# tlkvstepan/PracticalDeepStereo_NIPS2018

Hardware: AMD Instinct MI355X
Metric: stereo pairs/sec, 960x540 D=192, Matching+Regularization+SubpixelMap hot path (higher is better)
Workload: dtype f32; 1 GPU; configs[1]: 960x540 pair padded to 576x960, D=192 (48 matching planes, 96 cost planes), batch 1, eval mode, random-init weights seed 0; parallelism=single GPU, launch=eager, whole pairs round-robin over 3 HIP streams

## Files before the change

include/pds_hip.h:

```cpp
#ifndef PDS_HIP_H
#define PDS_HIP_H

#include <stddef.h>
#include <stdint.h>

#ifdef __cplusplus
extern "C" {
#endif

#define PDS_ABI_VERSION 6

typedef void* pds_stream_t;

int pds_abi_version(void);
const char* pds_last_error(void);

long long pds_nonfinite_statistics(int reset);

int pds_probe_begin(const char* kernel, int capacity);
int pds_probe_end(float* ms, int* workgroups, int capacity);

int pds_debug_chain_stamps(unsigned* ticks, int capacity);

typedef struct PdsConvBlockParams {
    const float* weight;
    const float* bias;
    const float* gamma;
    const float* beta;
} PdsConvBlockParams;

int pds_subpixel_map_fwd(const float* similarities, float* disparities,
                         int batch, int planes, int height, int width,
                         int half_support_window, int disparity_step,
                         pds_stream_t stream);

int pds_subpixel_map_confidence_fwd(const float* similarities, float* disparities, float* confidence,
                                    int batch, int planes, int height, int width,
                                    int half_support_window, int disparity_step,
                                    pds_stream_t stream);

int pds_shift_concat_fwd(const float* left, const float* right, float* out,
                         int batch, int channels, int h, int w,
                         int d_begin, int d_count, pds_stream_t stream);

typedef struct PdsMatchingParams {
    int features;
    int signature_features;
    int residual_blocks;
    PdsConvBlockParams first;
    const PdsConvBlockParams* blocks;
    PdsConvBlockParams last;
} PdsMatchingParams;

size_t pds_matching_workspace_bytes(const PdsMatchingParams* params, int batch, int h, int w,
                                    int d_count);
int pds_matching_fwd(const PdsMatchingParams* params,
                     const float* left, const float* right, float* signatures,
                     int batch, int h, int w, int d_begin, int d_count,
                     void* workspace, size_t workspace_bytes, int weights_resident,
                     pds_stream_t stream);

size_t pds_matching_operation_workspace_bytes(const PdsMatchingParams* params, int n, int h, int w);
int pds_matching_operation_fwd(const PdsMatchingParams* params,
                               const float* concatenated, float* signature,
                               int n, int h, int w,
                               void* workspace, size_t workspace_bytes, pds_stream_t stream);

typedef struct PdsRegularizationParams {
    int features;
    PdsConvBlockParams smoothing;
    PdsConvBlockParams contraction[4][2];
    PdsConvBlockParams expansion[4][2];
    PdsConvBlockParams upsample_half;
    PdsConvBlockParams upsample_full;
} PdsRegularizationParams;

size_t pds_regularization_workspace_bytes(const PdsRegularizationParams* params,
                                          int batch, int d, int h, int w);
int pds_regularization_fwd(const PdsRegularizationParams* params,
                           const float* signatures, const float* left_shortcut, float* cost,
                           int batch, int d, int h, int w,
                           void* workspace, size_t workspace_bytes, int weights_resident,
                           pds_stream_t stream);

int pds_regularization_subpixel_map_fwd(const PdsRegularizationParams* params,
                                        const float* signatures, const float* left_shortcut,
                                        float* disparities,
                                        int batch, int d, int h, int w,
                                        int half_support_window, int disparity_step,
                                        int crop_top, int crop_left,
                                        void* workspace, size_t workspace_bytes, int weights_resident,
                                        pds_stream_t stream);

int pds_regularization_subpixel_map_confidence_fwd(const PdsRegularizationParams* params,
                                                   const float* signatures, const float* left_shortcut,
                                                   float* disparities, float* confidence,
                                                   int batch, int d, int h, int w,
                                                   int half_support_window, int disparity_step,
                                                   int crop_top, int crop_left,
                                                   void* workspace, size_t workspace_bytes,
                                                   int weights_resident, pds_stream_t stream);

int pds_regularization_subpixel_map_mirrored_fwd(const PdsRegularizationParams* params,
                                                 const float* signatures, const float* left_shortcut,
                                                 float* disparities, float* confidence ,
                                                 int batch, int d, int h, int w,
                                                 int half_support_window, int disparity_step,
                                                 int crop_top, int crop_left,
                                                 void* workspace, size_t workspace_bytes,
                                                 int weights_resident, pds_stream_t stream);

size_t pds_contraction_block_workspace_bytes(int batch, int c, int d, int h, int w);
int pds_contraction_block_fwd(const PdsConvBlockParams* downsampling, const PdsConvBlockParams* smoothing,
                              const float* x, float* down, float* smooth,
                              int batch, int c, int d, int h, int w,
                              void* workspace, size_t workspace_bytes, pds_stream_t stream);

size_t pds_expansion_block_workspace_bytes(int batch, int c, int d, int h, int w);
int pds_expansion_block_fwd(const PdsConvBlockParams* upsampling, const PdsConvBlockParams* smoothing,
                            const float* x, const float* shortcut, float* out,
                            int batch, int c, int d, int h, int w,
                            void* workspace, size_t workspace_bytes, pds_stream_t stream);

size_t pds_conv_block_workspace_bytes(int n, int cin, int cout, int d, int h, int w, int kd, int stride,
                                      int per_plane);
int pds_conv_block_fwd(const PdsConvBlockParams* params, const float* x, float* raw, float* scale,
                       float* shift, int n, int cin, int cout, int d, int h, int w, int kd, int stride,
                       int per_plane, void* workspace, size_t workspace_bytes, pds_stream_t stream);
int pds_conv_block_chained_fwd(const PdsConvBlockParams* params, const float* x, const float* x_scale,
                               const float* x_shift, int x_per_plane, const float* x_bound, float* raw, float* scale,
                               float* shift, int n, int cin, int cout, int d, int h, int w, int kd, int stride,
                               int per_plane, void* workspace, size_t workspace_bytes, pds_stream_t stream);

size_t pds_regularization_bwd_workspace_bytes(const PdsRegularizationParams* params, int batch, int d, int h, int w);
int pds_regularization_bwd(const PdsRegularizationParams* params, const PdsRegularizationParams* grads,
                           const float* signatures, const float* left_shortcut, const float* grad_cost,
                           float* grad_signatures, float* grad_left_shortcut, int batch, int d, int h, int w,
                           void* fwd_workspace, size_t fwd_workspace_bytes, void* workspace, size_t workspace_bytes,
                           pds_stream_t stream);

size_t pds_matching_operation_bwd_workspace_bytes(const PdsMatchingParams* params, int n, int h, int w);
int pds_matching_operation_bwd(const PdsMatchingParams* params, const PdsMatchingParams* grads,
                               const float* concatenated, const float* grad_signature, float* grad_concatenated,
                               int n, int h, int w, void* fwd_workspace, size_t fwd_workspace_bytes,
                               void* workspace, size_t workspace_bytes, pds_stream_t stream);

size_t pds_matching_train_workspace_bytes(const PdsMatchingParams* params, int batch, int h, int w, int d_count);
int pds_matching_train_fwd(const PdsMatchingParams* params, const float* left, const float* right, float* signatures,
                           int batch, int h, int w, int d_begin, int d_count, void* workspace, size_t workspace_bytes,
                           pds_stream_t stream);
size_t pds_matching_bwd_workspace_bytes(const PdsMatchingParams* params, int batch, int h, int w, int d_count);
int pds_matching_bwd(const PdsMatchingParams* params, const PdsMatchingParams* grads, const float* left,
                     const float* right, const float* grad_signatures, float* grad_left, float* grad_right, int batch,
                     int h, int w, int d_begin, int d_count, void* fwd_workspace, size_t fwd_workspace_bytes,
                     void* workspace, size_t workspace_bytes, pds_stream_t stream);

typedef struct PdsEmbeddingParams {
    int input_features;
    int features;
    int shortcut_features;
    int residual_blocks;
    PdsConvBlockParams downsampling[2];
    const PdsConvBlockParams* blocks;
    PdsConvBlockParams shortcut;
} PdsEmbeddingParams;

size_t pds_embedding_workspace_bytes(const PdsEmbeddingParams* params, int batch, int h, int w, int pad_top,
                                     int pad_left);
int pds_embedding_fwd(const PdsEmbeddingParams* params, const float* image, float* descriptor, float* shortcut,
                      int batch, int h, int w, int pad_top, int pad_left, void* workspace, size_t workspace_bytes,
                      int weights_resident, pds_stream_t stream);
int pds_embedding_mirrored_fwd(const PdsEmbeddingParams* params, const float* image, float* descriptor,
                               float* shortcut, int batch, int h, int w, int pad_top, int pad_left, void* workspace,
                               size_t workspace_bytes, int weights_resident, pds_stream_t stream);
size_t pds_embedding_bwd_workspace_bytes(const PdsEmbeddingParams* params, int batch, int h, int w, int pad_top,
                                         int pad_left);
int pds_embedding_bwd(const PdsEmbeddingParams* params, const PdsEmbeddingParams* grads, const float* image,
                      const float* descriptor, float* grad_descriptor, const float* grad_shortcut, int batch, int h,
                      int w, int pad_top, int pad_left, void* fwd_workspace, size_t fwd_workspace_bytes, void* workspace,
                      size_t workspace_bytes, pds_stream_t stream);
size_t pds_embedding_image_bwd_workspace_bytes(const PdsEmbeddingParams* params, int batch, int h, int w, int pad_top,
                                               int pad_left);
int pds_embedding_image_bwd(const PdsEmbeddingParams* params, const PdsEmbeddingParams* grads, const float* image,
                            const float* descriptor, float* grad_descriptor, const float* grad_shortcut,
                            float* grad_image, int batch, int h, int w, int pad_top, int pad_left, void* fwd_workspace,
                            size_t fwd_workspace_bytes, void* workspace, size_t workspace_bytes, pds_stream_t stream);

size_t pds_contraction_block_bwd_workspace_bytes(int batch, int c, int d, int h, int w);
int pds_contraction_block_bwd(const PdsConvBlockParams* downsampling, const PdsConvBlockParams* smoothing,
                              const PdsConvBlockParams* grad_downsampling, const PdsConvBlockParams* grad_smoothing,
                              const float* x, const float* grad_down, const float* grad_smooth, float* grad_x,
                              int batch, int c, int d, int h, int w, void* fwd_workspace, size_t fwd_workspace_bytes,
                              void* workspace, size_t workspace_bytes, pds_stream_t stream);
size_t pds_expansion_block_bwd_workspace_bytes(int batch, int c, int d, int h, int w);
int pds_expansion_block_bwd(const PdsConvBlockParams* upsampling, const PdsConvBlockParams* smoothing,
                            const PdsConvBlockParams* grad_upsampling, const PdsConvBlockParams* grad_smoothing,
                            const float* x, const float* shortcut, const float* grad_out, float* grad_x,
                            float* grad_shortcut, int batch, int c, int d, int h, int w, void* fwd_workspace,
                            size_t fwd_workspace_bytes, void* workspace, size_t workspace_bytes, pds_stream_t stream);

int pds_shift_concat_bwd(const float* grad_out, float* grad_left, float* grad_right, int batch, int channels,
                         int h, int w, int d_begin, int d_count, pds_stream_t stream);

size_t pds_subpixel_cross_entropy_workspace_bytes(int n, int h, int w);
int pds_subpixel_cross_entropy_fwd(const float* similarities, const float* ground_truth, const float* weights,
                                   float* loss, float* lse, float* stats, int n, int planes, int h, int w,
                                   float diversity, int disparity_step, void* workspace, size_t workspace_bytes,
                                   pds_stream_t stream);
int pds_subpixel_cross_entropy_bwd(const float* similarities, const float* ground_truth, const float* weights,
                                   const float* lse, const float* stats, const float* grad_loss,
                                   float* grad_similarities, int n, int planes, int h, int w, float diversity,
                                   int disparity_step, pds_stream_t stream);
int pds_subpixel_cross_entropy_weights_bwd(const float* similarities, const float* ground_truth, const float* lse,
                                           const float* stats, const float* grad_loss, float* grad_weights, int n,
                                           int planes, int h, int w, float diversity, int disparity_step,
// ... 35 lines not shown
```

practicaldeepstereo_nips2018_amd/_lib.py:

```python
import ctypes
import os
import subprocess
import threading

import torch

_PKG_DIR = os.path.dirname(os.path.abspath(__file__))
_CSRC = os.path.join(_PKG_DIR, 'csrc')
LIB_PATH = os.environ.get('PDS_HIP_LIB') or os.path.join(_PKG_DIR, 'libpds_hip.so')
HEADER_PATH = os.path.join(os.path.dirname(_PKG_DIR), 'include', 'pds_hip.h')

_lock = threading.Lock()
_lib = None


class ConvBlockParams(ctypes.Structure):
    _fields_ = [('weight', ctypes.c_void_p), ('bias', ctypes.c_void_p),
                ('gamma', ctypes.c_void_p), ('beta', ctypes.c_void_p)]


class MatchingParams(ctypes.Structure):
    _fields_ = [('features', ctypes.c_int), ('signature_features', ctypes.c_int),
                ('residual_blocks', ctypes.c_int),
                ('first', ConvBlockParams),
# ... 30 lines not shown


BUILD_FLAGS = ['--offload-arch=gfx950', '-O3', '-std=c++17', '-fPIC']


def _source_digest():
    import hashlib
    h = hashlib.sha256(' '.join(BUILD_FLAGS).encode())
    deps = sources() + sorted(os.path.join(_CSRC, f) for f in os.listdir(_CSRC) if f.endswith('.hpp')) + [HEADER_PATH]
    for path in deps:
        h.update(os.path.basename(path).encode())
        with open(path, 'rb') as f:
            h.update(f.read())
    return h.hexdigest()


def build_library(force=False, verbose=False):
    from concurrent.futures import ThreadPoolExecutor
    if os.environ.get('PDS_HIP_LIB'):
        return LIB_PATH
    srcs = sources()
    stamp = LIB_PATH + '.sha256'
    digest = _source_digest()
    if not force and os.path.exists(LIB_PATH) and os.path.exists(stamp):
        with open(stamp) as f:
            if f.read().strip() == digest:
                return LIB_PATH
    objdir = os.path.join(os.path.dirname(_PKG_DIR), 'build', 'obj')
    os.makedirs(objdir, exist_ok=True)

    import hashlib
    headers = sorted(os.path.join(_CSRC, f) for f in os.listdir(_CSRC) if f.endswith('.hpp')) + [HEADER_PATH]
    base = hashlib.sha256(' '.join(BUILD_FLAGS).encode())
    for path in headers:
        with open(path, 'rb') as f:
            base.update(f.read())

    def compile_one(src):
        obj = os.path.join(objdir, os.path.basename(src)[:-4] + '.o')
        h = base.copy()
        with open(src, 'rb') as f:
            h.update(f.read())
        mark = obj + '.sha256'
        if not force and os.path.exists(obj) and os.path.exists(mark):
            with open(mark) as f:
                if f.read().strip() == h.hexdigest():
                    return obj
        cmd = ['hipcc'] + BUILD_FLAGS + ['-c', src, '-o', obj]
        if verbose:
            print(' '.join(cmd))
        subprocess.run(cmd, check=True)
        with open(mark, 'w') as f:
            f.write(h.hexdigest() + '\n')
        return obj

    with ThreadPoolExecutor(max_workers=min(8, os.cpu_count() or 1)) as pool:
        objs = list(pool.map(compile_one, srcs))
    cmd = ['hipcc', '--offload-arch=gfx950', '-shared', '-fPIC', '-o', LIB_PATH] + objs
    if verbose:
        print(' '.join(cmd))
    subprocess.run(cmd, check=True)
    with open(stamp, 'w') as f:
        f.write(digest + '\n')
    return LIB_PATH


_VP = ctypes.c_void_p
_I = ctypes.c_int
_SZ = ctypes.c_size_t

SIGNATURES = {
    'pds_abi_version': (_I, []),
    'pds_last_error': (ctypes.c_char_p, []),
    'pds_nonfinite_statistics': (ctypes.c_longlong, [_I]),
    'pds_probe_begin': (_I, [ctypes.c_char_p, _I]),
    'pds_probe_end': (_I, [_VP, _VP, _I]),
    'pds_debug_chain_stamps': (_I, [_VP, _I]),
    'pds_subpixel_map_fwd': (_I, [_VP, _VP, _I, _I, _I, _I, _I, _I, _VP]),
    'pds_subpixel_map_confidence_fwd': (_I, [_VP, _VP, _VP, _I, _I, _I, _I, _I, _I, _VP]),
    'pds_shift_concat_fwd': (_I, [_VP, _VP, _VP, _I, _I, _I, _I, _I, _I, _VP]),
    'pds_matching_workspace_bytes': (_SZ, [ctypes.POINTER(MatchingParams), _I, _I, _I, _I]),
    'pds_matching_fwd': (_I, [ctypes.POINTER(MatchingParams), _VP, _VP, _VP, _I, _I, _I, _I, _I,
                              _VP, _SZ, _I, _VP]),
    'pds_matching_train_workspace_bytes': (_SZ, [ctypes.POINTER(MatchingParams), _I, _I, _I, _I]),
    'pds_matching_train_fwd': (_I, [ctypes.POINTER(MatchingParams), _VP, _VP, _VP, _I, _I, _I, _I, _I, _VP, _SZ, _VP]),
    'pds_matching_bwd_workspace_bytes': (_SZ, [ctypes.POINTER(MatchingParams), _I, _I, _I, _I]),
    'pds_matching_bwd': (_I, [ctypes.POINTER(MatchingParams), ctypes.POINTER(MatchingParams), _VP, _VP, _VP, _VP, _VP,
                              _I, _I, _I, _I, _I, _VP, _SZ, _VP, _SZ, _VP]),
    'pds_matching_operation_workspace_bytes': (_SZ, [ctypes.POINTER(MatchingParams), _I, _I, _I]),
    'pds_matching_operation_fwd': (_I, [ctypes.POINTER(MatchingParams), _VP, _VP, _I, _I, _I,
                                        _VP, _SZ, _VP]),
    'pds_regularization_workspace_bytes': (_SZ, [ctypes.POINTER(RegularizationParams), _I, _I, _I, _I]),
    'pds_regularization_fwd': (_I, [ctypes.POINTER(RegularizationParams), _VP, _VP, _VP,
                                    _I, _I, _I, _I, _VP, _SZ, _I, _VP]),
    'pds_regularization_subpixel_map_fwd': (_I, [ctypes.POINTER(RegularizationParams), _VP, _VP, _VP,
                                                 _I, _I, _I, _I, _I, _I, _I, _I, _VP, _SZ, _I, _VP]),
    'pds_regularization_subpixel_map_confidence_fwd': (_I, [ctypes.POINTER(RegularizationParams), _VP, _VP, _VP,
                                                            _VP, _I, _I, _I, _I, _I, _I, _I, _I, _VP, _SZ, _I,
                                                            _VP]),
    'pds_regularization_subpixel_map_mirrored_fwd': (_I, [ctypes.POINTER(RegularizationParams), _VP, _VP, _VP,
                                                          _VP, _I, _I, _I, _I, _I, _I, _I, _I, _VP, _SZ, _I,
                                                          _VP]),
    'pds_conv_block_workspace_bytes': (_SZ, [_I] * 9),
    'pds_conv_block_fwd': (_I, [ctypes.POINTER(ConvBlockParams), _VP, _VP, _VP, _VP,
                                _I, _I, _I, _I, _I, _I, _I, _I, _I, _VP, _SZ, _VP]),
    'pds_conv_block_chained_fwd': (_I, [ctypes.POINTER(ConvBlockParams), _VP, _VP, _VP, _I, _VP, _VP, _VP, _VP,
                                        _I, _I, _I, _I, _I, _I, _I, _I, _I, _VP, _SZ, _VP]),
    'pds_regularization_bwd_workspace_bytes': (_SZ, [ctypes.POINTER(RegularizationParams), _I, _I, _I, _I]),
    'pds_regularization_bwd': (_I, [ctypes.POINTER(RegularizationParams), ctypes.POINTER(RegularizationParams),
                                    _VP, _VP, _VP, _VP, _VP, _I, _I, _I, _I, _VP, _SZ, _VP, _SZ, _VP]),
    'pds_matching_operation_bwd_workspace_bytes': (_SZ, [ctypes.POINTER(MatchingParams), _I, _I, _I]),
    'pds_matching_operation_bwd': (_I, [ctypes.POINTER(MatchingParams), ctypes.POINTER(MatchingParams),
                                        _VP, _VP, _VP, _I, _I, _I, _VP, _SZ, _VP, _SZ, _VP]),
    'pds_contraction_block_bwd_workspace_bytes': (_SZ, [_I, _I, _I, _I, _I]),
    'pds_contraction_block_bwd': (_I, [ctypes.POINTER(ConvBlockParams)] * 4 + [_VP, _VP, _VP, _VP, _I, _I, _I, _I, _I,
                                       _VP, _SZ, _VP, _SZ, _VP]),
    'pds_expansion_block_bwd_workspace_bytes': (_SZ, [_I, _I, _I, _I, _I]),
    'pds_expansion_block_bwd': (_I, [ctypes.POINTER(ConvBlockParams)] * 4 + [_VP, _VP, _VP, _VP, _VP, _I, _I, _I, _I,
                                     _I, _VP, _SZ, _VP, _SZ, _VP]),
    'pds_embedding_workspace_bytes': (_SZ, [ctypes.POINTER(EmbeddingParams), _I, _I, _I, _I, _I]),
    'pds_embedding_fwd': (_I, [ctypes.POINTER(EmbeddingParams), _VP, _VP, _VP, _I, _I, _I, _I, _I, _VP, _SZ, _I,
                               _VP]),
    'pds_embedding_mirrored_fwd': (_I, [ctypes.POINTER(EmbeddingParams), _VP, _VP, _VP, _I, _I, _I, _I, _I, _VP,
                                        _SZ, _I, _VP]),
    'pds_embedding_bwd_workspace_bytes': (_SZ, [ctypes.POINTER(EmbeddingParams), _I, _I, _I, _I, _I]),
    'pds_embedding_bwd': (_I, [ctypes.POINTER(EmbeddingParams)] * 2 + [_VP, _VP, _VP, _VP, _I, _I, _I, _I, _I,
                               _VP, _SZ, _VP, _SZ, _VP]),
    'pds_embedding_image_bwd_workspace_bytes': (_SZ, [ctypes.POINTER(EmbeddingParams), _I, _I, _I, _I, _I]),
    'pds_embedding_image_bwd': (_I, [ctypes.POINTER(EmbeddingParams)] * 2 + [_VP, _VP, _VP, _VP, _VP, _I, _I, _I, _I, _I,
                                     _VP, _SZ, _VP, _SZ, _VP]),
    'pds_disparity_errors_workspace_bytes': (_SZ, [_SZ]),
    'pds_disparity_errors_fwd': (_I, [_VP, _VP, _SZ, ctypes.c_float, _VP, _VP, _VP, _VP, _SZ, _VP]),
    'pds_left_right_check_fwd': (_I, [_VP, _VP, _VP, _VP, _VP, _VP, _I, _I, _I, ctypes.c_float, _VP]),
    'pds_rectify_maps_fwd': (_I, [_VP, _VP, _VP, _VP, _VP, _I, _I, _VP]),
    'pds_remap_fwd': (_I, [_VP, _I, _VP, _VP, _VP, _I, _I, _I, _I, _I, ctypes.c_float, _I, _VP]),
    'pds_reproject_fwd': (_I, [_VP, _VP, _VP, ctypes.c_float, _VP, _VP, _VP, _I, _I, _I, _VP]),
    'pds_speckle_filter_workspace_bytes': (_SZ, [_I, _I, _I]),
    'pds_speckle_filter_fwd': (_I, [_VP, _VP, _VP, _VP, _VP, _I, _I, _I, ctypes.c_float, _I, ctypes.c_float,
                                    _VP, _SZ, _VP]),
    'pds_median_filter_fwd': (_I, [_VP, _VP, _VP, _VP, _I, _I, _I, _I, _I, _I, ctypes.c_float, _VP]),
    'pds_subpixel_cross_entropy_workspace_bytes': (_SZ, [_I, _I, _I]),
    'pds_subpixel_cross_entropy_fwd': (_I, [_VP, _VP, _VP, _VP, _VP, _VP, _I, _I, _I, _I, ctypes.c_float, _I,
                                            _VP, _SZ, _VP]),
    'pds_subpixel_cross_entropy_bwd': (_I, [_VP, _VP, _VP, _VP, _VP, _VP, _VP, _I, _I, _I, _I, ctypes.c_float, _I,
                                            _VP]),
    'pds_subpixel_cross_entropy_weights_bwd': (_I, [_VP, _VP, _VP, _VP, _VP, _VP, _I, _I, _I, _I, ctypes.c_float, _I,
                                                    _VP]),
    'pds_shift_concat_bwd': (_I, [_VP, _VP, _VP, _I, _I, _I, _I, _I, _I, _VP]),
    'pds_contraction_block_workspace_bytes': (_SZ, [_I, _I, _I, _I, _I]),
    'pds_contraction_block_fwd': (_I, [ctypes.POINTER(ConvBlockParams), ctypes.POINTER(ConvBlockParams),
                                       _VP, _VP, _VP, _I, _I, _I, _I, _I, _VP, _SZ, _VP]),
    'pds_expansion_block_workspace_bytes': (_SZ, [_I, _I, _I, _I, _I]),
    'pds_expansion_block_fwd': (_I, [ctypes.POINTER(ConvBlockParams), ctypes.POINTER(ConvBlockParams),
                                     _VP, _VP, _VP, _I, _I, _I, _I, _I, _VP, _SZ, _VP]),
}


ABI_VERSION = 6


def load():
    global _lib
    with _lock:
        if _lib is None:
            if not os.path.exists(LIB_PATH):
                raise RuntimeError(
                    'libpds_hip.so is missing (%s). Build it with '
                    '`python -c "import __graft_entry__ as g; g.build()"`; there is no CPU fallback.'
                    % LIB_PATH)
            lib = ctypes.CDLL(LIB_PATH)
            lib.pds_abi_version.restype = ctypes.c_int
            lib.pds_abi_version.argtypes = []
            found = lib.pds_abi_version()
            if found != ABI_VERSION:
                raise RuntimeError(
                    '%s implements ABI version %d, this package binds version %d: rebuild it with '
                    '`python -c "import __graft_entry__ as g; g.build()"`' % (LIB_PATH, found, ABI_VERSION))
            for name, (res, args) in SIGNATURES.items():
                fn = getattr(lib, name)
                fn.restype = res
                fn.argtypes = args
            _lib = lib
    return _lib


def check(rc, what):
    if rc != 0:
        raise RuntimeError('%s failed (%d): %s' % (what, rc, load().pds_last_error().decode()))


def require_gpu_tensor(t, name, dims=None):
    if not isinstance(t, torch.Tensor):
        raise TypeError('%s must be a torch.Tensor' % name)
    if not t.is_cuda:
        raise RuntimeError('%s must live on an MI355X (cuda) device: the HIP path has no CPU fallback' % name)
    if t.dtype != torch.float32:
        raise TypeError('%s must be float32, got %s' % (name, t.dtype))
    if dims is not None and t.dim() != dims:
        raise ValueError('%s must have %d dimensions, got %d' % (name, dims, t.dim()))
    return t.contiguous()


def ptr(t):
    return ctypes.c_void_p(t.data_ptr())


def stream_handle(device):
    return ctypes.c_void_p(torch.cuda.current_stream(device).cuda_stream)


def conv_block_params(conv, norm=None, tensor_of=None):
    f = tensor_of if tensor_of is not None else (lambda t: t)
    p = ConvBlockParams()
    p.weight = f(conv.weight).data_ptr()
    p.bias = f(conv.bias).data_ptr()
    p.gamma = f(norm.weight).data_ptr() if norm is not None else None
    p.beta = f(norm.bias).data_ptr() if norm is not None else None
    return p


def gradient_buffers(module):
    grads = {id(p): torch.empty_like(p) for p in module.parameters()}
    return grads, (lambda p: grads[id(p)])


def parameter_signature(module):
    signature = []
    for p in module.parameters():
        if p.is_inference():
            return None
        signature.append((p.data_ptr(), p._version))
    return tuple(signature)


def resident_key(module, parameter_owner, geometry):
    if not getattr(module, '_weights_frozen', False):
        return None
    signature = parameter_signature(parameter_owner)
    if signature is None:
        return None
    return (geometry, signature)


class FrozenWeightsMixin(object):

    _weights_frozen = False

    def freeze_weights(self):
        self._weights_frozen = True
        return self

    def thaw_weights(self):
        self._weights_frozen = False
        self._workspace.invalidate()
        return self

    def invalidate_weights(self):
        self._workspace.invalidate()
        return self

    def _apply(self, fn, *args, **kwargs):
        result = super(FrozenWeightsMixin, self)._apply(fn, *args, **kwargs)
        self._workspace.invalidate()
        return result

    def _load_from_state_dict(self, *args, **kwargs):
        self._workspace.invalidate()
        return super(FrozenWeightsMixin, self)._load_from_state_dict(*args, **kwargs)

    def train(self, mode=True):
        if mode and self._weights_frozen:
            self.thaw_weights()
        return super(FrozenWeightsMixin, self).train(mode)


class Workspace(object):

    MAX_STREAMS = 8

    def __init__(self):
        self._buffers = {}
        self._keys = {}

    def _buffer(self, nbytes, device):
        slot = (device.index, torch.cuda.current_stream(device).cuda_stream)
        buf = self._buffers.pop(slot, None)
        if buf is None or buf.numel() < nbytes:
            buf = None
            self._keys.pop(slot, None)
            buf = torch.empty(max(int(nbytes), 256), dtype=torch.uint8, device=device)
        self._buffers[slot] = buf
        while len(self._buffers) > self.MAX_STREAMS:
            old = next(iter(self._buffers))
# ... 50 lines not shown
```

practicaldeepstereo_nips2018_amd/csrc/api.hip:

```cpp
#include <cmath>

#include "api_internal.hpp"

namespace pds {

static thread_local char g_error[512] = "";

int set_error(int code, const char* fmt, ...) {
    va_list ap;
    va_start(ap, fmt);
    vsnprintf(g_error, sizeof(g_error), fmt, ap);
    va_end(ap);
    return code;
}

int check_launch(const char* what) {
    const hipError_t e = hipGetLastError();
    if (e != hipSuccess) return set_error((int)e, "%s: %s", what, hipGetErrorString(e));
    static const bool debug_sync = getenv("PDS_DEBUG_SYNC") != nullptr;
    if (debug_sync) {
        fprintf(stderr, "[pds] %s ...", what);
        fflush(stderr);
        const hipError_t es = hipDeviceSynchronize();
        fprintf(stderr, " %s\n", es == hipSuccess ? "ok" : hipGetErrorString(es));
// ... 63 lines not shown
    L.type = type;
    L.kd = kd;
    L.stride = stride;
    L.a = a.id;
    L.b = b.p ? b.id : -1;
    L.out = o.id;
    L.in_g = in_g;
    L.out_g = o.g;
    L.P = P;
    L.norm = norm;
    c.tape->layers.push_back(L);
}

Geom conv_out_geom(const Geom& in, int cout, int kd, int stride) {
    Geom o = in;
    o.c = cout;
    if (stride == 2) {
        if (kd == 3) o.d = (in.d + 1) / 2;
        o.h = (in.h + 1) / 2;
        o.w = (in.w + 1) / 2;
    }
    return o;
}


DT conv_block(Ctx& c, const Src& a, const Src& b, const Geom& in, const PdsConvBlockParams& P, int cout, int kd, int stride,
              int per_plane, float* out_raw, bool allow_mfma, float* scale_out, float* shift_out, const ConvExtra* extra) {
    DT o;
    o.g = conv_out_geom(in, cout, kd, stride);
    o.per_plane = per_plane;
    o.raw = out_raw ? out_raw : c.get<float>(o.g.numel());
    const bool norm = P.gamma != nullptr;
    ConvLayer L;
    L.a = a;
    L.b = b;
    L.in = in;
    L.weight = (extra && extra->s2d_cin) ? extra->weight_used : P.weight;
    L.bias = P.bias;
    L.out = o.raw;
    L.out_g = o.g;
    L.kd = kd;
    L.stride = stride;
    L.lrelu = norm ? 1 : 0;
    L.stat_per_plane = per_plane;
    L.partials = nullptr;
    L.packed = nullptr;
    L.sink = c.sink;
    if (extra) {
        L.l0A = extra->l0A;
        L.l0G = extra->l0G;
        L.l0G2 = extra->l0G2;
        L.l0_cstride = extra->l0_cstride;
        L.l0_rs = extra->l0_rs;
        L.out_batch_channels = extra->out_batch_channels;
        L.d_begin = extra->d_begin;
        L.side_out = extra->side_out;
        L.plane_weight_sets = extra->plane_weight_sets;
        L.out_cb8 = extra->out_cb8 ? 1 : 0;
        L.l1B = extra->l1B;
        L.l1H = extra->l1H;
        L.l1_bstride = extra->l1_bstride;
        L.l1_hstride = extra->l1_hstride;
        L.l1_edge = extra->l1_edge;
        L.l1_P = extra->l1_P;
        L.l1_d0 = extra->l1_d0;
    }
    o.cb8 = L.out_cb8 != 0;
    int kind = 0;
    if (allow_mfma && !norm && !c.tape && conv2d_t8_supported(L)) kind = 8;
    else if (allow_mfma && !(extra && extra->matching_extras()) && conv2d_x3_supported(L)) kind = 9;
    else if (allow_mfma && conv2d_mfma_supported(L)) kind = conv2d_wino_eligible(L) ? 4 : 2;
    else if (allow_mfma && conv3d_t8_supported(L)) kind = 6;
    else if (allow_mfma && conv3d_ks_supported(L)) kind = 7;
    else if (allow_mfma && conv3d_nx_supported(L)) kind = 10;
    else if (allow_mfma && conv3d_mfma_supported(L)) kind = 3;
    if (kind == 2)
        L.packed = c.get<float>(conv2d_mfma_packed_floats(in.c, cout) * (L.plane_weight_sets > 0 ? L.plane_weight_sets : 1));
    if (kind == 4)
        L.packed = c.get<float>(conv2d_wino_packed_floats(in.c, cout) * (L.plane_weight_sets > 0 ? L.plane_weight_sets : 1));
    if (kind == 3) L.packed = c.get<float>(conv3d_mfma_packed_floats(o.g, in.c, stride));
    if (kind == 7) L.packed = c.get<float>(conv3d_ks_packed_floats(in.c, cout, 27));
    if (kind == 10) L.packed = c.get<float>(conv3d_nx_packed_floats(in.c, cout));
    if (kind == 9) L.packed = c.get<float>(conv2d_x3_packed_floats(in.c));
    if ((a.cb8 || b.cb8 || L.out_cb8) && !(kind == 9 && !b.p && conv2d_x3_cb8_ok(L, a.cb8 != 0, L.out_cb8 != 0))) {
        c.run(set_error(-1, "conv_block: a channel-blocked tensor reached a kernel that does not take it"));
        return o;
    }
    if (L.l1B && kind != 9) {
        c.run(set_error(-1, "conv_block: the on-the-fly layer-1 source needs conv2d_x3"));
        return o;
    }
    if (L.out_batch_channels && kind != 4 && kind != 9) {
        c.run(set_error(-1, "conv_block: a channel-slice output needs the Winograd kernel"));
        return o;
    }
    if (extra && extra->matching_extras() && kind != 2 && kind != 4 && kind != 8) {
        c.run(set_error(-1, "conv_block: fused Matching extras need the conv2d MFMA kernel"));
        return o;
    }
    auto launch = [&]() {
        return kind == 2 ? launch_conv2d_mfma(L, c.s)
                         : kind == 4 ? launch_conv2d_wino(L, c.s)
                                     : kind == 3 ? launch_conv3d_mfma(L, c.s)
                                                 : kind == 6 ? launch_conv3d_t8(L, c.s)
                                                             : kind == 7 ? launch_conv3d_ks(L, c.s)
                                                             : kind == 10 ? launch_conv3d_nx(L, c.s)
                                                                         : kind == 8 ? launch_conv2d_t8(L, c.s)
                                                                                     : kind == 9 ? launch_conv2d_x3(L, c.s) : launch_conv_direct(L, c.s);
    };
    const bool collecting = c.sink && c.sink->phase == kPackCollect && c.base != nullptr;
    if (collecting && kind != 0 && kind != 6 && kind != 8) c.run(launch());
    if (norm) {
        const int tiles = kind == 2 ? conv2d_mfma_tiles(o.g)
                                    : kind == 4 ? conv2d_wino_tiles(o.g)
                                    : kind == 9 ? conv2d_x3_tiles(L)
                                    : kind == 3 ? conv3d_mfma_tiles(o.g, in.c, stride)
                                    : kind == 6 ? conv3d_t8_records(o.g)
                                    : kind == 7 ? conv3d_ks_tiles(o.g)
                                    : kind == 10 ? conv3d_nx_tiles(o.g) : conv_direct_tiles_for(o.g, stride);
        const bool volume_records = kind == 3 || kind == 6 || kind == 7 || kind == 10;
        const size_t records = (size_t)o.g.n * o.g.c * (volume_records ? 1 : o.g.d) * tiles;
        L.partials = c.get<double>(records * 2);
        const int groups = o.g.n * o.g.c * (per_plane ? o.g.d : 1);
        o.normed = true;
        o.scale = scale_out ? scale_out : c.get<float>(groups);
        o.shift = shift_out ? shift_out : c.get<float>(groups);
        o.mean = c.get<float>(groups);
        o.rstd = c.get<float>(groups);
        o.bound = c.get<float>(1);
        o.bound_n = 1;
        o.bounded = true;
        if (!c.plan) {
            const int per_group = volume_records ? tiles : tiles * (per_plane ? 1 : o.g.d);
            const double count = (double)o.g.h * o.g.w * (per_plane ? 1 : o.g.d);
            bool chained = false;
            if (c.chain && kind == 7 && !per_plane) {
                const KsChainFold fold{P.gamma, P.beta, o.scale, o.shift, o.mean, o.rstd, o.bound, groups, per_group, o.g.c, count};
                c.run(conv3d_ks_chain_add(*c.chain, L, fold, &chained));
            }
            if (!chained) {
                c.flush_chain();
                c.run(launch());
                c.run(launch_in_finalize(L.partials, groups, per_group, count, P.gamma, P.beta, o.g.c,
                                         per_plane ? o.g.d : 1, o.scale, o.shift, o.mean, o.rstd, c.s, o.bound));
            }
        }
    } else if (!c.plan) {
        c.flush_chain();
        c.run(launch());
    }
    tape_layer(c, 0, kd, stride, a, b, in, o, &P, norm);
    if (c.tape && extra && extra->s2d_cin) {
        c.tape->layers.back().weight_used = extra->weight_used;
        c.tape->layers.back().s2d_cin = extra->s2d_cin;
    }
    return o;
}

DT deconv_block(Ctx& c, const Src& a, const Src& b, const Geom& in, const PdsConvBlockParams& P, int cout, int kd,
                float* out_raw) {
    DT o;
    o.g = in;
    o.g.c = cout;
    o.g.d = (kd == 4) ? in.d * 2 : in.d;
    o.g.h = in.h * 2;
    o.g.w = in.w * 2;
// ... 98 lines not shown
    for (int i = 0; i < n; ++i) {
        if (hipEventSynchronize(g_probe_stop[i]) != hipSuccess) return set_error(-1, "probe: hipEventSynchronize failed");
        float t = 0.f;
        if (hipEventElapsedTime(&t, g_probe_start[i], g_probe_stop[i]) != hipSuccess)
            return set_error(-1, "probe: hipEventElapsedTime failed");
        if (ms) ms[i] = t;
        if (workgroups) workgroups[i] = g_probe_wgs[i];
    }
    return n;
}
const char* pds_last_error(void) { return g_error; }

int pds_debug_chain_stamps(unsigned* ticks, int capacity) {
    PDS_REQUIRE(ticks && capacity > 0, "chain stamps: bad arguments");
    return ks_chain_debug_stamps(ticks, capacity);
}

int pds_subpixel_map_fwd(const float* similarities, float* disparities, int batch, int planes, int height,
                         int width, int half_support_window, int disparity_step, pds_stream_t stream) {
    PDS_REQUIRE(similarities && disparities, "subpixel_map: null pointer");
    PDS_REQUIRE(batch > 0 && planes > 0 && height > 0 && width > 0, "subpixel_map: bad shape");
    PDS_REQUIRE(disparity_step >= 1 && half_support_window >= 1 && half_support_window % disparity_step == 0,
                "subpixel_map: bad window/step");
    const int hi = half_support_window / disparity_step;
    const int lo = -((half_support_window + disparity_step - 1) / disparity_step);
    return launch_subpixel_map(similarities, disparities, batch, planes, height, width, lo, hi, disparity_step,
                               (hipStream_t)stream);
}

int pds_subpixel_map_confidence_fwd(const float* similarities, float* disparities, float* confidence, int batch,
                                    int planes, int height, int width, int half_support_window, int disparity_step,
                                    pds_stream_t stream) {
    PDS_REQUIRE(similarities && disparities && confidence, "subpixel_map_confidence: null pointer");
    PDS_REQUIRE(batch > 0 && planes > 0 && height > 0 && width > 0, "subpixel_map_confidence: bad shape");
    PDS_REQUIRE(disparity_step >= 1 && half_support_window >= 1 && half_support_window % disparity_step == 0,
                "subpixel_map_confidence: bad window/step");
    const int hi = half_support_window / disparity_step;
    const int lo = -((half_support_window + disparity_step - 1) / disparity_step);
    return launch_subpixel_map(similarities, disparities, batch, planes, height, width, lo, hi, disparity_step,
                               (hipStream_t)stream, confidence);
}

int pds_shift_concat_fwd(const float* left, const float* right, float* out, int batch, int channels, int h, int w,
                         int d_begin, int d_count, pds_stream_t stream) {
    PDS_REQUIRE(left && right && out, "shift_concat: null pointer");
    PDS_REQUIRE(batch > 0 && channels > 0 && h > 0 && w > 0 && d_begin >= 0 && d_count > 0,
                "shift_concat: bad shape");
    return launch_shift_concat(left, right, out, batch, channels, h, w, d_begin, d_count, (hipStream_t)stream);
}

size_t pds_conv_block_workspace_bytes(int n, int cin, int cout, int d, int h, int w, int kd, int stride,
                                      int per_plane) {
    PdsConvBlockParams dummy{nullptr, nullptr, (const float*)1, (const float*)1};
    size_t need = 0;
    for (int bounded = 0; bounded < 2; ++bounded) {
        Ctx c{nullptr, 0, true, nullptr};
        Src src = plain_src(nullptr);
        src.normed = 1;
        src.bounded = bounded;
        conv_block(c, src, no_src(), Geom{n, cin, d, h, w}, dummy, cout, kd, stride, per_plane, (float*)1, true,
                   (float*)1, (float*)1);
        if (c.off > need) need = c.off;
    }
    return need + 256;
}

int pds_conv_block_fwd(const PdsConvBlockParams* params, const float* x, float* raw, float* scale, float* shift,
                       int n, int cin, int cout, int d, int h, int w, int kd, int stride, int per_plane,
                       void* workspace, size_t workspace_bytes, pds_stream_t stream) {
    PDS_REQUIRE(params && x && raw && workspace, "conv_block: null pointer");
    PDS_REQUIRE(params->weight && params->bias, "conv_block: null weight/bias");
    PDS_REQUIRE(n > 0 && cin > 0 && cout > 0 && d > 0 && h > 0 && w > 0, "conv_block: bad shape");
    PDS_REQUIRE((kd == 1 || kd == 3) && (stride == 1 || stride == 2) && !(kd == 1 && stride == 2),
                "conv_block: unsupported kd=%d stride=%d", kd, stride);
    if (params->gamma) PDS_REQUIRE(params->beta && scale && shift, "conv_block: null InstanceNorm outputs");
    const size_t need = pds_conv_block_workspace_bytes(n, cin, cout, d, h, w, kd, stride, per_plane);
    PDS_REQUIRE(workspace_bytes >= need, "conv_block: workspace too small (%zu < %zu)", workspace_bytes, need);
    Ctx c{(char*)workspace, 0, false, (hipStream_t)stream};
    conv_block(c, plain_src(x), no_src(), Geom{n, cin, d, h, w}, *params, cout, kd, stride, per_plane, raw, true,
               scale, shift);
    return c.err;
}

int pds_conv_block_chained_fwd(const PdsConvBlockParams* params, const float* x, const float* x_scale,
                               const float* x_shift, int x_per_plane, const float* x_bound, float* raw, float* scale,
                               float* shift, int n, int cin, int cout, int d, int h, int w, int kd, int stride,
                               int per_plane, void* workspace, size_t workspace_bytes, pds_stream_t stream) {
    PDS_REQUIRE(params && x && x_scale && x_shift && raw && workspace, "conv_block_chained: null pointer");
    PDS_REQUIRE(params->weight && params->bias, "conv_block_chained: null weight/bias");
    PDS_REQUIRE(n > 0 && cin > 0 && cout > 0 && d > 0 && h > 0 && w > 0, "conv_block_chained: bad shape");
    PDS_REQUIRE((kd == 1 || kd == 3) && (stride == 1 || stride == 2) && !(kd == 1 && stride == 2),
                "conv_block_chained: unsupported kd=%d stride=%d", kd, stride);
    if (params->gamma) PDS_REQUIRE(params->beta && scale && shift, "conv_block_chained: null InstanceNorm outputs");
    const size_t need = pds_conv_block_workspace_bytes(n, cin, cout, d, h, w, kd, stride, per_plane);
    PDS_REQUIRE(workspace_bytes >= need, "conv_block_chained: workspace too small (%zu < %zu)", workspace_bytes, need);
    Ctx c{(char*)workspace, 0, false, (hipStream_t)stream};
    Src src{x, x_scale, x_shift, x_per_plane ? 1 : 0, 0};
    src.normed = 1;
    if (x_bound) {
        src.bound = x_bound;
        src.bound_n = 1;
        src.bounded = 1;
    }
    conv_block(c, src, no_src(), Geom{n, cin, d, h, w}, *params, cout, kd, stride, per_plane, raw, true, scale, shift);
    return c.err;
}

size_t pds_disparity_errors_workspace_bytes(size_t count) {
    return disparity_errors_partial_doubles(count) * sizeof(double) + 256;
}

int pds_disparity_errors_fwd(const float* estimated, const float* ground_truth, size_t count, float n,
                             float* pixelwise_absolute_error, float* pixelwise_n_pixels_error, double* stats,
                             void* workspace, size_t workspace_bytes, pds_stream_t stream) {
    PDS_REQUIRE(estimated && ground_truth && stats && workspace, "disparity_errors: null pointer");
    PDS_REQUIRE(count > 0, "disparity_errors: empty input");
    PDS_REQUIRE(workspace_bytes >= pds_disparity_errors_workspace_bytes(count), "disparity_errors: workspace too small");
    return launch_disparity_errors(estimated, ground_truth, count, n, pixelwise_absolute_error,
                                   pixelwise_n_pixels_error, stats, reinterpret_cast<double*>(workspace),
                                   (hipStream_t)stream);
}

int pds_left_right_check_fwd(const float* left_disparity, const float* right_disparity, unsigned char* left_valid,
                             unsigned char* right_valid, float* left_filled, float* right_filled, int batch, int h,
                             int w, float max_difference, pds_stream_t stream) {
    PDS_REQUIRE(left_disparity && right_disparity && left_valid && right_valid, "left_right_check: null pointer");
    PDS_REQUIRE(batch > 0 && h > 0 && w > 0 && w < (1 << 24) && (size_t)batch * h <= 0x7fffffffu,
                "left_right_check: bad shape (%d, %d, %d)", batch, h, w);
    PDS_REQUIRE(max_difference >= 0.f && max_difference <= 3.402823466e+38f,
                "left_right_check: max_difference must be finite and >= 0 (got %g)", (double)max_difference);
    PDS_REQUIRE(left_filled != left_disparity && left_filled != right_disparity && right_filled != left_disparity &&
                    right_filled != right_disparity && (!left_filled || left_filled != right_filled),
                "left_right_check: a filled output aliases an input");
    return launch_left_right_check(left_disparity, right_disparity, left_valid, right_valid, left_filled, right_filled,
                                   batch * h, w, max_difference, (hipStream_t)stream);
}

static size_t speckle_checked_bytes(int batch, int h, int w) {
    if (!(batch > 0 && h > 0 && w > 0)) {
        set_error(-1, "speckle_filter: bad shape (%d, %d, %d)", batch, h, w);
        return 0;
    }
    if ((size_t)h * w > 0x7fffffffu) {
        set_error(-1, "speckle_filter: an image of %d x %d pixels does not fit 32-bit labels", h, w);
        return 0;
    }
    if ((size_t)batch * h * w > speckle_max_pixels()) {
        set_error(-1, "speckle_filter: batch * h * w = %zu does not fit 32-bit indices (at most %zu)",
                  (size_t)batch * h * w, speckle_max_pixels());
        return 0;
    }
    return speckle_workspace_bytes(batch, h, w);
}

size_t pds_speckle_filter_workspace_bytes(int batch, int h, int w) { return speckle_checked_bytes(batch, h, w); }

int pds_speckle_filter_fwd(const float* disparity, const unsigned char* valid, unsigned char* keep, float* filtered,
                           int* sizes, int batch, int h, int w, float max_difference, int max_size, float fill_value,
                           void* workspace, size_t workspace_bytes, pds_stream_t stream) {
    PDS_REQUIRE(disparity && keep && workspace, "speckle_filter: null pointer");
    const size_t need = speckle_checked_bytes(batch, h, w);
    if (need == 0) return -1;
    PDS_REQUIRE(max_difference >= 0.f && max_difference <= 3.402823466e+38f,
                "speckle_filter: max_difference must be finite and >= 0 (got %g)", (double)max_difference);
    PDS_REQUIRE(max_size >= 0, "speckle_filter: max_size must be >= 0 (got %d)", max_size);
    PDS_REQUIRE(workspace_bytes >= need, "speckle_filter: workspace too small (%zu < %zu)", workspace_bytes, need);
// ... 144 lines not shown
```

practicaldeepstereo_nips2018_amd/csrc/api_internal.hpp:

```cpp
#pragma once
#include <cstdlib>
#include <cstring>
#include <vector>

#include "common.hpp"

namespace pds {

int launch_conv2d_mfma(const ConvLayer& L, hipStream_t s);
bool conv2d_mfma_supported(const ConvLayer& L);
int conv2d_mfma_tiles(const Geom& out_g);
size_t conv2d_mfma_packed_floats(int cin, int cout);
int launch_conv2d_wino(const ConvLayer& L, hipStream_t s);
bool conv2d_wino_eligible(const ConvLayer& L);
int conv2d_wino_tiles(const Geom& out_g);
size_t conv2d_wino_packed_floats(int cin, int cout);
int launch_conv2d_x3(const ConvLayer& L, hipStream_t s);
bool conv2d_x3_supported(const ConvLayer& L);
bool conv2d_x3_cb8_ok(const ConvLayer& L, bool in_cb8, bool out_cb8);
int conv2d_x3_tiles(const ConvLayer& L);
size_t conv2d_x3_packed_floats(int cin);
int launch_conv2d_t8(const ConvLayer& L, hipStream_t s);
bool conv2d_t8_supported(const ConvLayer& L);
int launch_conv3d_mfma(const ConvLayer& L, hipStream_t s);
// ... 100 lines not shown
    }
    void run(int rc) {
        if (!err && rc) err = rc;
    }
    bool before_packing() const {
        if (sink) return base != nullptr && sink->phase == kPackCollect;
        return !plan;
    }
};

template <class Pipeline>
static int run_with_batched_packing(void* workspace, hipStream_t stream, Pipeline&& pipeline,
                                    bool weights_resident = false) {
    PackJob table[64];
    PackSink sink;
    sink.jobs = table;
    sink.capacity = 64;
    if (!weights_resident) {
        sink.phase = kPackCollect;
        Ctx collect{(char*)workspace, 0, true, stream};
        collect.sink = &sink;
        pipeline(collect);
        if (collect.err) return collect.err;
        if (sink.count > 0)
            if (int rc = launch_multi_pack(table, sink.count, stream)) return rc;
    }
    sink.phase = kPackDone;
    Ctx run{(char*)workspace, 0, false, stream};
    run.sink = &sink;
    pipeline(run);
    return run.err;
}

struct DT {
    float* raw = nullptr;
    float* scale = nullptr;
    float* shift = nullptr;
    float* mean = nullptr;
    float* rstd = nullptr;
    Geom g{0, 0, 0, 0, 0};
    int per_plane = 0;
    int id = -1;
    bool normed = false;
    float* bound = nullptr;
    int bound_n = 0;
    bool bounded = false;
    bool cb8 = false;
    Src src() const {
        Src s{raw, scale, shift, per_plane, 0};
        s.cb8 = cb8 ? 1 : 0;
        s.id = id;
        s.normed = normed ? 1 : 0;
        s.bound = bound;
        s.bound_n = bound_n;
        s.bounded = bounded ? 1 : 0;
        return s;
    }
};


void carve_amax(Ctx& c, DT& t, int records);
Src external_src(Ctx& c, const float* p, const Geom& g, int bcast_d = 0, bool needs_grad = true);
void tape_layer(Ctx& c, int type, int kd, int stride, const Src& a, const Src& b, const Geom& in_g, DT& o,
                const PdsConvBlockParams* P, bool norm);
Geom conv_out_geom(const Geom& in, int cout, int kd, int stride);

struct ConvExtra {
    const float* l0A = nullptr;
    const float* l0G = nullptr;
    const float* l0G2 = nullptr;
    size_t l0_cstride = 0;
    int l0_rs = 0;
    int out_batch_channels = 0;
    int d_begin = 0;
    float* side_out = nullptr;
    int plane_weight_sets = 0;
    const float* weight_used = nullptr;
    int s2d_cin = 0;
    bool out_cb8 = false;
    const float* l1B = nullptr;
    const float* l1H = nullptr;
    unsigned l1_bstride = 0, l1_hstride = 0, l1_edge = 0;
    int l1_P = 0, l1_d0 = 0;
    bool matching_extras() const { return l0A || side_out || plane_weight_sets > 0; }
};


DT conv_block(Ctx& c, const Src& a, const Src& b, const Geom& in, const PdsConvBlockParams& P, int cout, int kd, int stride,
              int per_plane, float* out_raw = nullptr, bool allow_mfma = true, float* scale_out = nullptr,
              float* shift_out = nullptr, const ConvExtra* extra = nullptr);
DT deconv_block(Ctx& c, const Src& a, const Src& b, const Geom& in, const PdsConvBlockParams& P, int cout, int kd,
                float* out_raw = nullptr);
int check_block(const PdsConvBlockParams& b, bool norm, const char* name);

struct GradMap {
    const char* params_base;
    const char* grads_base;
    size_t struct_bytes;
    const PdsConvBlockParams* blocks_params = nullptr;
    const PdsConvBlockParams* blocks_grads = nullptr;
    int blocks_count = 0;
    const PdsConvBlockParams* find(const PdsConvBlockParams* p) const {
        if (blocks_params && p >= blocks_params && p < blocks_params + blocks_count) return blocks_grads + (p - blocks_params);
        const char* q = reinterpret_cast<const char*>(p);
        if (q >= params_base && q < params_base + struct_bytes)
            return reinterpret_cast<const PdsConvBlockParams*>(grads_base + (q - params_base));
        return nullptr;
    }
};


extern thread_local size_t g_backward_arena_bytes;
struct ArenaLimit {
    explicit ArenaLimit(size_t bytes) { g_backward_arena_bytes = bytes; }
    ~ArenaLimit() { g_backward_arena_bytes = ~(size_t)0; }
};

void backward_walk(Ctx& c, const Tape& T, const GradMap& M, std::vector<float*>& dhat, std::vector<char>& written);

}
```

practicaldeepstereo_nips2018_amd/csrc/api_matching.hip:

```cpp
#include "api_internal.hpp"

namespace pds {

static void operation_tail(Ctx& c, const PdsMatchingParams& P, const Src& x0, const Geom& g, float* signature) {
    const int F = P.features;
    Src cur = x0;
    DT t2;
    for (int r = 0; r < P.residual_blocks; ++r) {
        DT t1 = conv_block(c, cur, no_src(), g, P.blocks[2 * r], F, 1, 1, 1);
        t2 = conv_block(c, t1.src(), no_src(), g, P.blocks[2 * r + 1], F, 1, 1, 1);
        if (r + 1 < P.residual_blocks) {
            DT nxt;
            nxt.raw = c.get<float>(g.numel());
            nxt.g = g;
            carve_amax(c, nxt, materialize_records(g));
            if (!c.plan) c.run(launch_materialize(t2.src(), cur, g, nxt.raw, c.s, nxt.bound));
            tape_layer(c, 2, 0, 0, t2.src(), cur, g, nxt, nullptr, false);
            cur = nxt.src();
        }
    }
    if (P.residual_blocks > 0)
        conv_block(c, t2.src(), cur, g, P.last, P.signature_features, 1, 1, 1, signature);
    else
        conv_block(c, cur, no_src(), g, P.last, P.signature_features, 1, 1, 1, signature);
}

static bool fused_matching_supported(const PdsMatchingParams& P, int batch, int h, int w, int d_count) {
    ConvLayer L{};
    L.a = plain_src(nullptr);
    L.b = no_src();
    L.in = Geom{batch, P.features, d_count, h, w};
    L.out_g = L.in;
    L.kd = 1;
    L.stride = 1;
    ConvLayer T = L;
    T.out_g.c = P.signature_features;
    return conv2d_mfma_supported(L) && conv2d_mfma_supported(T);
}

struct MatchingL0 {
    const float* w3 = nullptr;
};

static void matching_pipeline(Ctx& c, const PdsMatchingParams& P, const float* left, const float* right,
                              float* signatures, int batch, int h, int w, int d_begin, int d_count, bool train = false,
                              MatchingL0* l0_out = nullptr) {
    const int F = P.features;
    const size_t wn = (size_t)F * F * 9;
    float* w3 = c.get<float>(3 * wn);
    float* bias3 = c.get<float>(3 * F);
    if (l0_out) l0_out->w3 = w3;
    const Geom g{batch, F, d_count, h, w};
    const bool fused = [&]() {
        static const bool enabled = []() {
            const char* e = debug_switch("PDS_MATCHING_FUSED");
            return !(e && e[0] == '0');
        }();
        return enabled && fused_matching_supported(P, batch, h, w, d_count);
    }();
    const bool columns = [&]() {
        static const bool enabled = []() {
            const char* e = debug_switch("PDS_MATCHING_COLUMNS");
            return !(e && e[0] == '0');
        }();
        return enabled && fused && !train && P.residual_blocks >= 1 && F % 8 == 0;
    }();
    const int l0_planes = columns ? 2 : 3;
    const int l0_pad = columns ? 2 : 1;
    const int l0_rs = w + l0_pad;
    const Geom g3{batch, F, l0_planes, h, l0_rs};
    float* x3 = c.get<float>(g3.numel());
    float* wcol0 = columns ? c.get<float>(9 * (size_t)F * F) : nullptr;
    float* wcol1 = columns ? c.get<float>(9 * (size_t)F * F) : nullptr;
    if (c.before_packing()) {
        c.run(launch_split_first_weights(P.first.weight, P.first.bias, w3, w3 + wn, w3 + 2 * wn, bias3, F, F, c.s));
        if (columns) {
            c.run(launch_column_weights(P.first.weight, 2 * F, F, F, F, wcol0, c.s));
            c.run(launch_column_weights(P.blocks[0].weight, F, 0, F, F, wcol1, c.s));
        }
    }
    if (!c.plan) c.run(launch_l0_stack_inputs(left, right, x3, (size_t)batch * F, h, w, l0_planes, l0_pad, c.s));
    float* y3;
    if (fused) {
        PdsConvBlockParams p3{w3, bias3, nullptr, nullptr};
        ConvExtra e3;
        e3.plane_weight_sets = l0_planes;
        Tape* tape = c.tape;
        c.tape = nullptr;
        y3 = conv_block(c, plain_src(x3), no_src(), g3, p3, F, 1, 1, 1, nullptr, true, nullptr, nullptr, &e3).raw;
        c.tape = tape;
    } else {
        y3 = c.get<float>(g3.numel());
        float* tmp_in = c.get<float>((size_t)batch * F * h * (w + 1));
        float* tmp_out = c.get<float>((size_t)batch * F * h * (w + 1));
        const Geom g1{batch, F, 1, h, w + 1};
        Tape* tape = c.tape;
        c.tape = nullptr;
        for (int p = 0; p < 3; ++p) {
            if (!c.plan) c.run(launch_pad_left1(p == 0 ? left : right, tmp_in, (size_t)batch * F * h, w, c.s));
            PdsConvBlockParams pp{w3 + p * wn, bias3 + p * F, nullptr, nullptr};
            conv_block(c, plain_src(tmp_in), no_src(), g1, pp, F, 1, 1, 1, tmp_out);
            if (!c.plan)
                c.run((int)hipMemcpy2DAsync(y3 + (size_t)p * h * (w + 1), (size_t)3 * h * (w + 1) * sizeof(float), tmp_out,
                                        (size_t)h * (w + 1) * sizeof(float), (size_t)h * (w + 1) * sizeof(float),
                                        (size_t)batch * F, hipMemcpyDeviceToDevice, c.s));
        }
        c.tape = tape;
    }
    const size_t l0_cstride = (size_t)l0_planes * h * l0_rs;
    const float* l0A = y3 + l0_pad;
    const float* l0G = y3 + (size_t)h * l0_rs + (l0_pad - 1);
    const float* l0G2 = y3 + (size_t)2 * h * l0_rs + (l0_pad - 1);
    float* g2buf = nullptr;
    if (columns) {
        g2buf = c.get<float>(g3.numel());
        if (!c.plan)
            c.run(launch_l0_column_fix(y3 + (size_t)h * l0_rs, right, wcol0, g2buf + (size_t)h * l0_rs, y3, l0_pad,
                                       l0_cstride, l0_rs, l0_pad, batch, F, F, h, w, d_begin, d_count, c.s));
        l0G2 = g2buf + (size_t)h * l0_rs + (l0_pad - 1);
    }
    if (!fused || train) {
        DT x0;
        x0.g = g;
        x0.raw = c.get<float>(g.numel());
        carve_amax(c, x0, l0_combine_records(batch, F, d_count));
        if (!c.plan)
            c.run(launch_l0_combine(l0A, l0G, l0G2, l0_cstride, x0.raw, batch, F, h, w, d_begin, d_count, c.s, x0.bound));
        Src x0s = x0.src();
        if (c.tape) {
            TapeTensor t;
            t.raw = x0.raw;
            t.g = g;
            t.bound = x0.bound;
            t.bound_n = x0.bound_n;
            t.bounded = true;
            x0s.id = c.tape->add(t);
        }
        operation_tail(c, P, x0s, g, signatures);
        return;
    }
    ConvExtra l0;
    l0.l0A = l0A;
    l0.l0G = l0G;
    l0.l0G2 = l0G2;
    l0.l0_cstride = l0_cstride;
    l0.l0_rs = l0_rs;
    l0.d_begin = d_begin;
    const Src none = no_src();
    if (P.residual_blocks == 0) {
        conv_block(c, none, none, g, P.last, P.signature_features, 1, 1, 1, signatures, true, nullptr, nullptr, &l0);
        return;
    }
    const int cb8_level = [&]() {
        static const int level = []() {
            const char* e = debug_switch("PDS_MATCHING_CB8");
            return e ? atoi(e) : 2;
        }();
        if (!(F == 64 && h % 16 == 0 && w % 16 == 0)) return 0;
        ConvLayer probe;
        probe.a = plain_src(nullptr);
        probe.a.bounded = 1;
        probe.b = no_src();
        probe.in = g;
        probe.out_g = g;
        probe.kd = 1;
        probe.stride = 1;
        return conv2d_x3_cb8_ok(probe, true, true) ? level : 0;
    }();
    DT t1;
    ConvExtra fly;
    bool on_the_fly = false;
    {
        DT y4;
        const float* corr = nullptr;
        const float* corr0 = nullptr;
        if (columns) {
            float* w2 = c.get<float>(2 * wn);
            float* bias2 = c.get<float>(2 * F);
            const Geom g2{batch, F, 2, h, w + 2};
            float* cr = c.get<float>((size_t)batch * F * h * d_count * 2);
            float* cr0 = c.get<float>((size_t)batch * F * h);
            if (c.before_packing())
                c.run(launch_l1_weights2(P.blocks[0].weight, P.blocks[0].bias, w2, bias2, F, F, c.s));
            if (!c.plan)
                c.run(launch_l1_column_terms(y3 + (size_t)h * l0_rs, g2buf + (size_t)h * l0_rs, wcol1, cr, cr0,
                                             l0_cstride, l0_rs, l0_pad, batch, F, F, h, w, d_begin, d_count, c.s));
            float* x2 = y3;
            PdsConvBlockParams p2{w2, bias2, nullptr, nullptr};
            ConvExtra e2;
            e2.plane_weight_sets = 2;
            y4 = conv_block(c, plain_src(x2), none, g2, p2, F, 1, 1, 1, nullptr, true, nullptr, nullptr, &e2);
            corr = cr;
            corr0 = cr0;
        } else {
            const size_t wn4 = (size_t)kL1Planes * F * 2 * F * 9;
            float* w4 = c.get<float>(wn4);
            float* bias4 = c.get<float>(kL1Planes * F);
            const Geom g4{batch, 2 * F, kL1Planes, h, w + 2};
            float* x4 = c.get<float>(g4.numel());
            if (c.before_packing())
                c.run(launch_l1_weights(P.blocks[0].weight, P.blocks[0].bias, w4, bias4, F, F, c.s));
            if (!c.plan) c.run(launch_l1_stack_inputs(y3, x4, batch, F, h, w, c.s));
            PdsConvBlockParams p4{w4, bias4, nullptr, nullptr};
            ConvExtra e4;
            e4.plane_weight_sets = kL1Planes;
            y4 = conv_block(c, plain_src(x4), none, g4, p4, F, 1, 1, 1, nullptr, true, nullptr, nullptr, &e4);
        }
        t1.g = g;
        t1.per_plane = 1;
        t1.raw = c.get<float>(g.numel());
        const int tiles = l1_combine_tiles(h, w);
        double* partials = c.get<double>((size_t)batch * F * d_count * tiles * 2);
        const int groups = batch * F * d_count;
        t1.normed = true;
        t1.scale = c.get<float>(groups);
        t1.shift = c.get<float>(groups);
        t1.mean = c.get<float>(groups);
        t1.rstd = c.get<float>(groups);
        t1.bound = c.get<float>(1);
        t1.bound_n = 1;
        t1.bounded = true;
        if (columns && cb8_level >= 2) {
            const int pad = d_begin + d_count;
            fly.l1_bstride = (unsigned)(l1_blocked_b_floats(h, w) * sizeof(float));
            fly.l1_hstride = (unsigned)(l1_blocked_h_floats(h, w, pad, d_count) * sizeof(float));
            fly.l1_edge = (unsigned)(l1_blocked_edge_offset_floats(h, w, pad) * sizeof(float));
            fly.l1_P = pad;
            fly.l1_d0 = d_begin;
            float* Bc = c.get<float>((size_t)batch * (F / 8) * l1_blocked_b_floats(h, w));
            float* Hx = c.get<float>((size_t)batch * (F / 8) * l1_blocked_h_floats(h, w, pad, d_count));
            fly.l1B = Bc;
            fly.l1H = Hx;
            on_the_fly = true;
            if (!c.plan)
                c.run(launch_l1_blocked(y4.raw, corr, corr0, Bc, Hx, batch, F, h, w, pad, d_begin, d_count, c.s));
        }
        if (!c.plan) {
            c.run(launch_l1_combine(y4.raw, corr, corr0, on_the_fly ? nullptr : t1.raw, partials, batch, F, h, w, d_begin,
                                    d_count, c.s));
            c.run(launch_in_finalize(partials, groups, tiles, (double)h * w, P.blocks[0].gamma, P.blocks[0].beta, F,
                                     d_count, t1.scale, t1.shift, t1.mean, t1.rstd, c.s, t1.bound));
        }
    }
    DT t2 = on_the_fly ? conv_block(c, t1.src(), none, g, P.blocks[1], F, 1, 1, 1, nullptr, true, nullptr, nullptr, &fly)
                       : conv_block(c, t1.src(), none, g, P.blocks[1], F, 1, 1, 1);
    if (P.residual_blocks == 1) {
        conv_block(c, t2.src(), none, g, P.last, P.signature_features, 1, 1, 1, signatures, true, nullptr, nullptr,
                   &l0);
        return;
    }
    DT cur;
    cur.g = g;
    cur.raw = t1.raw;
    carve_amax(c, cur, materialize_l0_records(g));
    if (!c.plan)
        c.run(launch_materialize_l0(t2.src(), g, l0A, l0G, l0G2, l0_cstride, l0_rs, d_begin, cur.raw, c.s, cur.bound));
    float* spare_a = t2.raw;
    float* spare_b = c.get<float>(g.numel());
    for (int r = 1; r < P.residual_blocks; ++r) {
        ConvExtra blocked;
        blocked.out_cb8 = cb8_level >= 1;
        t1 = conv_block(c, cur.src(), none, g, P.blocks[2 * r], F, 1, 1, 1, spare_a, true, nullptr, nullptr, &blocked);
        t2 = conv_block(c, t1.src(), none, g, P.blocks[2 * r + 1], F, 1, 1, 1, spare_b);
        if (r + 1 < P.residual_blocks) {
            DT nxt;
            nxt.g = g;
            nxt.raw = spare_a;
            carve_amax(c, nxt, materialize_records(g));
            if (!c.plan) c.run(launch_materialize(t2.src(), cur.src(), g, nxt.raw, c.s, nxt.bound));
            spare_a = cur.raw;
            cur = nxt;
        }
    }
    conv_block(c, t2.src(), cur.src(), g, P.last, P.signature_features, 1, 1, 1, signatures);
}

static void operation_pipeline(Ctx& c, const PdsMatchingParams& P, const float* concatenated, float* signature,
                               int n, int h, int w) {
    const Geom gin{n, 2 * P.features, 1, h, w};
    DT x0 = conv_block(c, external_src(c, concatenated, gin), no_src(), gin, P.first, P.features, 1, 1, 1);
    operation_tail(c, P, x0.src(), x0.g, signature);
}

}

using namespace pds;

extern "C" {

static int check_matching_params(const PdsMatchingParams* P) {
    PDS_REQUIRE(P, "matching: null params");
    PDS_REQUIRE(P->features > 0 && P->signature_features > 0 && P->residual_blocks >= 0, "matching: bad params");
    PDS_REQUIRE(P->first.weight && P->first.bias && P->last.weight && P->last.bias, "matching: null weights");
    for (int i = 0; i < 2 * P->residual_blocks; ++i)
        PDS_REQUIRE(P->blocks && P->blocks[i].weight && P->blocks[i].bias && P->blocks[i].gamma && P->blocks[i].beta,
                    "matching: null residual-block weights");
    return 0;
}

size_t pds_matching_workspace_bytes(const PdsMatchingParams* params, int batch, int h, int w, int d_count) {
    if (check_matching_params(params)) return 0;
    Ctx c{nullptr, 0, true, nullptr};
    matching_pipeline(c, *params, nullptr, nullptr, nullptr, batch, h, w, 0, d_count);
    return c.off;
}

int pds_matching_fwd(const PdsMatchingParams* params, const float* left, const float* right, float* signatures,
                     int batch, int h, int w, int d_begin, int d_count, void* workspace, size_t workspace_bytes,
                     int weights_resident, pds_stream_t stream) {
    if (int rc = check_matching_params(params)) return rc;
    PDS_REQUIRE(left && right && signatures && workspace, "matching: null pointer");
    PDS_REQUIRE(batch > 0 && h > 0 && w > 0 && d_begin >= 0 && d_count > 0, "matching: bad shape");
    const size_t need = pds_matching_workspace_bytes(params, batch, h, w, d_count);
    PDS_REQUIRE(workspace_bytes >= need, "matching: workspace too small (%zu < %zu)", workspace_bytes, need);
    return run_with_batched_packing(workspace, (hipStream_t)stream, [&](Ctx& c) {
        matching_pipeline(c, *params, left, right, signatures, batch, h, w, d_begin, d_count);
    }, weights_resident != 0);
}

static int matching_backward(bool plan, size_t* bytes, const PdsMatchingParams* params, const PdsMatchingParams* grads,
                             const float* left, const float* right, const float* grad_signatures, float* grad_left,
                             float* grad_right, int batch, int h, int w, int d_begin, int d_count, void* fwd_workspace,
                             void* workspace, hipStream_t stream);

size_t pds_matching_train_workspace_bytes(const PdsMatchingParams* params, int batch, int h, int w, int d_count) {
    if (check_matching_params(params)) return 0;
    Ctx c{nullptr, 0, true, nullptr};
    matching_pipeline(c, *params, nullptr, nullptr, nullptr, batch, h, w, 0, d_count, true);
    return c.off;
}

int pds_matching_train_fwd(const PdsMatchingParams* params, const float* left, const float* right, float* signatures,
                           int batch, int h, int w, int d_begin, int d_count, void* workspace, size_t workspace_bytes,
                           pds_stream_t stream) {
    if (int rc = check_matching_params(params)) return rc;
    PDS_REQUIRE(left && right && signatures && workspace, "matching_train: null pointer");
    PDS_REQUIRE(batch > 0 && h > 0 && w > 0 && d_begin >= 0 && d_count > 0, "matching_train: bad shape");
    PDS_REQUIRE(params->residual_blocks >= 0, "matching_train: bad block count");
    const size_t need = pds_matching_train_workspace_bytes(params, batch, h, w, d_count);
    PDS_REQUIRE(workspace_bytes >= need, "matching_train: workspace too small (%zu < %zu)", workspace_bytes, need);
    return run_with_batched_packing(workspace, (hipStream_t)stream, [&](Ctx& c) {
        matching_pipeline(c, *params, left, right, signatures, batch, h, w, d_begin, d_count, true);
    });
}

size_t pds_matching_bwd_workspace_bytes(const PdsMatchingParams* params, int batch, int h, int w, int d_count) {
    if (check_matching_params(params)) return 0;
    size_t bytes = 0;
    if (matching_backward(true, &bytes, params, params, nullptr, nullptr, nullptr, nullptr, nullptr, batch, h, w, 0,
                          d_count, nullptr, nullptr, nullptr))
        return 0;
    return bytes + 256;
}

int pds_matching_bwd(const PdsMatchingParams* params, const PdsMatchingParams* grads, const float* left,
                     const float* right, const float* grad_signatures, float* grad_left, float* grad_right, int batch,
                     int h, int w, int d_begin, int d_count, void* fwd_workspace, size_t fwd_workspace_bytes,
                     void* workspace, size_t workspace_bytes, pds_stream_t stream) {
    if (int rc = check_matching_params(params)) return rc;
    if (int rc = check_matching_params(grads)) return rc;
    PDS_REQUIRE(left && right && grad_signatures && grad_left && grad_right && fwd_workspace && workspace,
                "matching_bwd: null pointer");
    PDS_REQUIRE(batch > 0 && h > 0 && w > 0 && d_begin >= 0 && d_count > 0, "matching_bwd: bad shape");
    PDS_REQUIRE(fwd_workspace_bytes >= pds_matching_train_workspace_bytes(params, batch, h, w, d_count),
                "matching_bwd: forward workspace too small");
    const size_t need = pds_matching_bwd_workspace_bytes(params, batch, h, w, d_count);
    PDS_REQUIRE(workspace_bytes >= need, "matching_bwd: workspace too small (%zu < %zu)", workspace_bytes, need);
    ArenaLimit limit(workspace_bytes);
    return matching_backward(false, nullptr, params, grads, left, right, grad_signatures, grad_left, grad_right, batch, h,
                             w, d_begin, d_count, fwd_workspace, workspace, (hipStream_t)stream);
}

size_t pds_matching_operation_workspace_bytes(const PdsMatchingParams* params, int n, int h, int w) {
    if (check_matching_params(params)) return 0;
    Ctx c{nullptr, 0, true, nullptr};
    operation_pipeline(c, *params, nullptr, nullptr, n, h, w);
    return c.off;
}

int pds_matching_operation_fwd(const PdsMatchingParams* params, const float* concatenated, float* signature, int n,
                               int h, int w, void* workspace, size_t workspace_bytes, pds_stream_t stream) {
    if (int rc = check_matching_params(params)) return rc;
    PDS_REQUIRE(concatenated && signature && workspace, "matching_operation: null pointer");
    PDS_REQUIRE(n > 0 && h > 0 && w > 0, "matching_operation: bad shape");
    const size_t need = pds_matching_operation_workspace_bytes(params, n, h, w);
    PDS_REQUIRE(workspace_bytes >= need, "matching_operation: workspace too small (%zu < %zu)", workspace_bytes,
                need);
    return run_with_batched_packing(workspace, (hipStream_t)stream, [&](Ctx& c) {
        operation_pipeline(c, *params, concatenated, signature, n, h, w);
    });
}

static int operation_backward(bool plan, size_t* bytes, const PdsMatchingParams* params, const PdsMatchingParams* grads,
                              const float* concatenated, const float* grad_signature, float* grad_concatenated, int n,
                              int h, int w, void* fwd_workspace, void* workspace, hipStream_t stream) {
    Tape tape;
    Ctx re{plan ? nullptr : (char*)fwd_workspace, 0, true, stream};
    re.tape = &tape;
    operation_pipeline(re, *params, concatenated, const_cast<float*>(grad_signature) , n, h, w);
// ... 118 lines not shown
```

practicaldeepstereo_nips2018_amd/csrc/api_regularization.hip:

```cpp
#include "api_internal.hpp"

namespace pds {

static DT regularization_trunk(Ctx& c, const PdsRegularizationParams& P, const float* ms, const float* left,
                               int batch, int d, int h, int w) {
    const int F = P.features;
    const Geom g0{batch, F, d, h, w};
    const Src ms_src = external_src(c, ms, g0);
    Src shortcut = external_src(c, left, g0, 1);
    KsChain chain;
    c.chain_sync = c.get<unsigned>(kKsChainStateWords);
    c.chain = (!c.plan && conv3d_ks_chain_enabled()) ? &chain : nullptr;
    DT out = conv_block(c, ms_src, no_src(), g0, P.smoothing, F, 3, 1, 0);
    DT pushed[4];
    for (int i = 0; i < 4; ++i) {
        pushed[i] = out;
        const int cin = out.g.c;
        DT down = conv_block(c, out.src(), shortcut, out.g, P.contraction[i][0], 2 * cin, 3, 2, 0);
        DT smooth = conv_block(c, down.src(), no_src(), down.g, P.contraction[i][1], 2 * cin, 3, 1, 0);
        shortcut = down.src();
        out = smooth;
    }
    for (int i = 0; i < 4; ++i) {
        const int cin = out.g.c;
        DT up = deconv_block(c, out.src(), no_src(), out.g, P.expansion[i][0], cin / 2, 4);
        out = conv_block(c, up.src(), pushed[3 - i].src(), up.g, P.expansion[i][1], cin / 2, 3, 1, 0);
    }
    DT half = deconv_block(c, out.src(), no_src(), out.g, P.upsample_half, F / 2, 4);
    c.flush_chain();
    c.chain = nullptr;
    return half;
}

bool upsample_full_valu_supported(int cin);
int launch_upsample_full(const float* in, const float* scale, const float* shift, const float* w, const float* bias,
                         float* cost, int batch, int cin, int d, int hi_, int wi, hipStream_t s);

static void regularization_pipeline(Ctx& c, const PdsRegularizationParams& P, const float* ms, const float* left,
                                    float* cost, int batch, int d, int h, int w) {
    DT half = regularization_trunk(c, P, ms, left, batch, d, h, w);
    if (upsample_full_valu_supported(half.g.c)) {
        float* w_pairs = c.get<float>((size_t)half.g.c * 48);
        if (c.before_packing()) c.run(launch_upsample_weight_pairs(P.upsample_full.weight, w_pairs, half.g.c, c.s));
        if (!c.plan)
            c.run(launch_upsample_full(half.raw, half.scale, half.shift, w_pairs, P.upsample_full.bias,
                                       cost, batch, half.g.c, half.g.d, half.g.h, half.g.w, c.s));
        DT full;
        full.raw = cost;
        full.g = Geom{batch, 1, half.g.d, 2 * half.g.h, 2 * half.g.w};
        tape_layer(c, 1, 3, 1, half.src(), no_src(), half.g, full, &P.upsample_full, false);
        return;
    }
    deconv_block(c, half.src(), no_src(), half.g, P.upsample_full, 1, 3, cost);
}


static void contraction_pipeline(Ctx& c, const PdsConvBlockParams* pp, const float* x, float* down_out,
                                 float* smooth_out, const Geom& g, int* id_down_out = nullptr,
                                 int* id_smooth_out = nullptr) {
    const Src xs = external_src(c, x, g);
    DT down = conv_block(c, xs, no_src(), g, pp[0], 2 * g.c, 3, 2, 0);
    DT smooth = conv_block(c, down.src(), no_src(), down.g, pp[1], 2 * g.c, 3, 1, 0);
    if (!c.plan) {
        c.run(launch_materialize(down.src(), no_src(), down.g, down_out, c.s));
        c.run(launch_materialize(smooth.src(), no_src(), smooth.g, smooth_out, c.s));
    }
    DT od, os;
    od.raw = down_out;
    od.g = down.g;
    os.raw = smooth_out;
    os.g = smooth.g;
    tape_layer(c, 2, 0, 0, down.src(), no_src(), down.g, od, nullptr, false);
    tape_layer(c, 2, 0, 0, smooth.src(), no_src(), smooth.g, os, nullptr, false);
    if (id_down_out) *id_down_out = od.id;
    if (id_smooth_out) *id_smooth_out = os.id;
}

static void expansion_pipeline(Ctx& c, const PdsConvBlockParams* pp, const float* x, const float* shortcut,
                               float* out, const Geom& g) {
    const Src xs = external_src(c, x, g);
    const Geom gs{g.n, g.c / 2, 2 * g.d, 2 * g.h, 2 * g.w};
    const Src ss = external_src(c, shortcut, gs);
    DT up = deconv_block(c, xs, no_src(), g, pp[0], g.c / 2, 4);
    DT sm = conv_block(c, up.src(), ss, up.g, pp[1], g.c / 2, 3, 1, 0);
    if (!c.plan) c.run(launch_materialize(sm.src(), no_src(), sm.g, out, c.s));
    DT o;
    o.raw = out;
    o.g = sm.g;
    tape_layer(c, 2, 0, 0, sm.src(), no_src(), sm.g, o, nullptr, false);
}

}

using namespace pds;

extern "C" {

static int check_regularization(const PdsRegularizationParams* P, int batch, int d, int h, int w) {
    PDS_REQUIRE(P, "regularization: null params");
    PDS_REQUIRE(P->features >= 2 && P->features % 2 == 0, "regularization: features must be even");
    PDS_REQUIRE(batch > 0 && d > 0 && h > 0 && w > 0, "regularization: bad shape");
    PDS_REQUIRE(d % 16 == 0 && h % 16 == 0 && w % 16 == 0,
                "regularization: D, h, w must be multiples of 16 (got %d, %d, %d)", d, h, w);
    PDS_REQUIRE((d / 16) * (h / 16) * (w / 16) > 1,
                "regularization: InstanceNorm needs more than one element at 1/16 scale");
    if (int rc = check_block(P->smoothing, true, "regularization._smoothing")) return rc;
    for (int i = 0; i < 4; ++i)
        for (int j = 0; j < 2; ++j) {
            if (int rc = check_block(P->contraction[i][j], true, "regularization._contraction_blocks")) return rc;
            if (int rc = check_block(P->expansion[i][j], true, "regularization._expansion_blocks")) return rc;
        }
    if (int rc = check_block(P->upsample_half, true, "regularization._upsample_to_halfsize")) return rc;
    return check_block(P->upsample_full, false, "regularization._upsample_to_fullsize");
}

size_t pds_regularization_workspace_bytes(const PdsRegularizationParams* params, int batch, int d, int h, int w) {
    if (check_regularization(params, batch, d, h, w)) return 0;
    Ctx c{nullptr, 0, true, nullptr};
    regularization_pipeline(c, *params, nullptr, nullptr, nullptr, batch, d, h, w);
    c.get<float>((size_t)batch * 2 * d * 4 * h * 4 * w);
    return c.off;
}

int pds_regularization_fwd(const PdsRegularizationParams* params, const float* signatures,
                           const float* left_shortcut, float* cost, int batch, int d, int h, int w, void* workspace,
                           size_t workspace_bytes, int weights_resident, pds_stream_t stream) {
    if (int rc = check_regularization(params, batch, d, h, w)) return rc;
    PDS_REQUIRE(signatures && left_shortcut && cost && workspace, "regularization: null pointer");
    const size_t need = pds_regularization_workspace_bytes(params, batch, d, h, w);
    PDS_REQUIRE(workspace_bytes >= need, "regularization: workspace too small (%zu < %zu)", workspace_bytes, need);
    return run_with_batched_packing(workspace, (hipStream_t)stream, [&](Ctx& c) {
        regularization_pipeline(c, *params, signatures, left_shortcut, cost, batch, d, h, w);
    }, weights_resident != 0);
}

static int regularization_estimator(const PdsRegularizationParams* params, const float* signatures,
                                    const float* left_shortcut, float* disparities, float* confidence, int batch, int d,
                                    int h, int w, int half_support_window, int disparity_step, int crop_top,
                                    int crop_left, void* workspace, size_t workspace_bytes, int weights_resident,
                                    pds_stream_t stream, const char* what, bool mirror = false) {
    if (int rc = check_regularization(params, batch, d, h, w)) return rc;
    PDS_REQUIRE(signatures && left_shortcut && disparities && workspace, "%s: null pointer", what);
    PDS_REQUIRE(disparity_step >= 1 && half_support_window >= 1 && half_support_window % disparity_step == 0,
                "%s: bad window/step", what);
    PDS_REQUIRE(crop_top >= 0 && crop_top < 4 * h && crop_left >= 0 && crop_left < 4 * w,
                "%s: bad crop (%d, %d)", what, crop_top, crop_left);
    const size_t need = pds_regularization_workspace_bytes(params, batch, d, h, w);
    PDS_REQUIRE(workspace_bytes >= need, "%s: workspace too small (%zu < %zu)", what, workspace_bytes, need);
    Ctx c{(char*)workspace, 0, false, (hipStream_t)stream};
    const int hi = half_support_window / disparity_step;
    const int lo = -((half_support_window + disparity_step - 1) / disparity_step);
    if (upsample_estimator_supported(params->features / 2, lo, hi)) {
        DT half;
        float* w_pairs = nullptr;
        if (int rc = run_with_batched_packing(workspace, (hipStream_t)stream, [&](Ctx& cc) {
                half = regularization_trunk(cc, *params, signatures, left_shortcut, batch, d, h, w);
                w_pairs = cc.get<float>((size_t)half.g.c * 48);
                if (cc.before_packing())
                    cc.run(launch_upsample_weight_pairs(params->upsample_full.weight, w_pairs, half.g.c, cc.s));
            }, weights_resident != 0))
            return rc;
        return launch_upsample_estimator(half.raw, half.scale, half.shift, w_pairs,
                                         params->upsample_full.bias, disparities, batch, half.g.c, half.g.d, half.g.h,
                                         half.g.w, lo, hi, disparity_step, crop_top, crop_left, (hipStream_t)stream,
                                         confidence, mirror);
    }
    PDS_REQUIRE(crop_top == 0 && crop_left == 0,
                "%s: the crop is only folded into the fused kernel (4 features, window <= 4 taps)", what);
    PDS_REQUIRE(!mirror, "%s: the mirror is only folded into the fused kernel (4 features, window <= 4 taps)", what);
    float* cost = c.get<float>((size_t)batch * 2 * d * 4 * h * 4 * w);
    if (int rc = run_with_batched_packing((char*)workspace + c.off, (hipStream_t)stream, [&](Ctx& cc) {
            regularization_pipeline(cc, *params, signatures, left_shortcut, cost, batch, d, h, w);
        }, weights_resident != 0))
        return rc;
    if (confidence)
        return pds_subpixel_map_confidence_fwd(cost, disparities, confidence, batch, 2 * d, 4 * h, 4 * w,
                                               half_support_window, disparity_step, stream);
    return pds_subpixel_map_fwd(cost, disparities, batch, 2 * d, 4 * h, 4 * w, half_support_window, disparity_step,
                                stream);
}

int pds_regularization_subpixel_map_fwd(const PdsRegularizationParams* params, const float* signatures,
                                        const float* left_shortcut, float* disparities, int batch, int d, int h,
                                        int w, int half_support_window, int disparity_step, int crop_top,
                                        int crop_left, void* workspace, size_t workspace_bytes, int weights_resident,
                                        pds_stream_t stream) {
    return regularization_estimator(params, signatures, left_shortcut, disparities, nullptr, batch, d, h, w,
                                    half_support_window, disparity_step, crop_top, crop_left, workspace,
                                    workspace_bytes, weights_resident, stream, "regularization_subpixel_map");
}

int pds_regularization_subpixel_map_confidence_fwd(const PdsRegularizationParams* params, const float* signatures,
                                                   const float* left_shortcut, float* disparities, float* confidence,
                                                   int batch, int d, int h, int w, int half_support_window,
                                                   int disparity_step, int crop_top, int crop_left, void* workspace,
                                                   size_t workspace_bytes, int weights_resident, pds_stream_t stream) {
    PDS_REQUIRE(confidence, "regularization_subpixel_map_confidence: null pointer");
    return regularization_estimator(params, signatures, left_shortcut, disparities, confidence, batch, d, h, w,
                                    half_support_window, disparity_step, crop_top, crop_left, workspace,
                                    workspace_bytes, weights_resident, stream, "regularization_subpixel_map_confidence");
}

int pds_regularization_subpixel_map_mirrored_fwd(const PdsRegularizationParams* params, const float* signatures,
                                                 const float* left_shortcut, float* disparities, float* confidence,
                                                 int batch, int d, int h, int w, int half_support_window,
                                                 int disparity_step, int crop_top, int crop_left, void* workspace,
                                                 size_t workspace_bytes, int weights_resident, pds_stream_t stream) {
    return regularization_estimator(params, signatures, left_shortcut, disparities, confidence, batch, d, h, w,
                                    half_support_window, disparity_step, crop_top, crop_left, workspace,
                                    workspace_bytes, weights_resident, stream, "regularization_subpixel_map_mirrored",
                                    true);
}


#define PDS_MARK reinterpret_cast<const float*>(8)
static const PdsConvBlockParams kDummyBlocks[2] = {{PDS_MARK, PDS_MARK, PDS_MARK, PDS_MARK},
                                                   {PDS_MARK, PDS_MARK, PDS_MARK, PDS_MARK}};

size_t pds_contraction_block_workspace_bytes(int batch, int c_, int d, int h, int w) {
    Ctx c{nullptr, 0, true, nullptr};
    contraction_pipeline(c, kDummyBlocks, nullptr, nullptr, nullptr, Geom{batch, c_, d, h, w});
    return c.off + 256;
}

int pds_contraction_block_fwd(const PdsConvBlockParams* downsampling, const PdsConvBlockParams* smoothing,
                              const float* x, float* down_out, float* smooth_out, int batch, int c_, int d, int h,
                              int w, void* workspace, size_t workspace_bytes, pds_stream_t stream) {
    PDS_REQUIRE(downsampling && smoothing && x && down_out && smooth_out && workspace, "contraction: null pointer");
    PDS_REQUIRE(batch > 0 && c_ > 0 && d > 0 && h > 0 && w > 0, "contraction: bad shape");
    if (int rc = check_block(*downsampling, true, "contraction._downsampling_2x")) return rc;
    if (int rc = check_block(*smoothing, true, "contraction._smoothing")) return rc;
    const size_t need = pds_contraction_block_workspace_bytes(batch, c_, d, h, w);
    PDS_REQUIRE(workspace_bytes >= need, "contraction: workspace too small (%zu < %zu)", workspace_bytes, need);
    const PdsConvBlockParams pp[2] = {*downsampling, *smoothing};
    Ctx c{(char*)workspace, 0, false, (hipStream_t)stream};
    contraction_pipeline(c, pp, x, down_out, smooth_out, Geom{batch, c_, d, h, w});
    return c.err;
}

size_t pds_expansion_block_workspace_bytes(int batch, int c_, int d, int h, int w) {
    Ctx c{nullptr, 0, true, nullptr};
    expansion_pipeline(c, kDummyBlocks, nullptr, nullptr, nullptr, Geom{batch, c_, d, h, w});
    return c.off + 256;
}

int pds_expansion_block_fwd(const PdsConvBlockParams* upsampling, const PdsConvBlockParams* smoothing, const float* x,
                            const float* shortcut, float* out, int batch, int c_, int d, int h, int w,
                            void* workspace, size_t workspace_bytes, pds_stream_t stream) {
    PDS_REQUIRE(upsampling && smoothing && x && shortcut && out && workspace, "expansion: null pointer");
    PDS_REQUIRE(batch > 0 && c_ >= 2 && c_ % 2 == 0 && d > 0 && h > 0 && w > 0, "expansion: bad shape");
    if (int rc = check_block(*upsampling, true, "expansion._upsampling_2x")) return rc;
    if (int rc = check_block(*smoothing, true, "expansion._smoothing")) return rc;
    const size_t need = pds_expansion_block_workspace_bytes(batch, c_, d, h, w);
    PDS_REQUIRE(workspace_bytes >= need, "expansion: workspace too small (%zu < %zu)", workspace_bytes, need);
    const PdsConvBlockParams pp[2] = {*upsampling, *smoothing};
    Ctx c{(char*)workspace, 0, false, (hipStream_t)stream};
    expansion_pipeline(c, pp, x, shortcut, out, Geom{batch, c_, d, h, w});
    return c.err;
}

static size_t regularization_fwd_bytes(const PdsRegularizationParams* params, int batch, int d, int h, int w) {
    Ctx c{nullptr, 0, true, nullptr};
    regularization_pipeline(c, *params, nullptr, nullptr, nullptr, batch, d, h, w);
    return c.off;
}

static int regularization_backward(bool plan, size_t* bytes, const PdsRegularizationParams* params,
                                   const PdsRegularizationParams* grads, const float* signatures,
                                   const float* left_shortcut, const float* grad_cost, float* grad_signatures,
                                   float* grad_left_shortcut, int batch, int d, int h, int w, void* fwd_workspace,
                                   void* workspace, hipStream_t stream) {
    Tape tape;
    Ctx re{plan ? nullptr : (char*)fwd_workspace, 0, true, stream};
    re.tape = &tape;
    regularization_pipeline(re, *params, signatures, left_shortcut, const_cast<float*>(grad_cost) ,
                            batch, d, h, w);
    if (re.err) return re.err;
    std::vector<float*> dhat(tape.tensors.size(), nullptr);
    std::vector<char> written(tape.tensors.size(), 0);
    dhat[0] = grad_signatures;
    dhat[1] = grad_left_shortcut;
    dhat[tape.tensors.size() - 1] = const_cast<float*>(grad_cost);
    written[tape.tensors.size() - 1] = 1;
    GradMap M{reinterpret_cast<const char*>(params), reinterpret_cast<const char*>(grads), sizeof(PdsRegularizationParams)};
    Ctx c{plan ? nullptr : (char*)workspace, 0, plan, stream};
    if (!plan) c.limit = g_backward_arena_bytes;
    if (plan) {
        dhat[0] = dhat[1] = dhat[tape.tensors.size() - 1] = reinterpret_cast<float*>(8);
    }
    backward_walk(c, tape, M, dhat, written);
    if (bytes) *bytes = c.off;
    return c.err;
}

size_t pds_regularization_bwd_workspace_bytes(const PdsRegularizationParams* params, int batch, int d, int h, int w) {
    if (check_regularization(params, batch, d, h, w)) return 0;
// ... 119 lines not shown
```

practicaldeepstereo_nips2018_amd/csrc/common.hpp:

```cpp
#pragma once
#include <hip/hip_runtime.h>
#include <atomic>
#include <mutex>
#include <cstdarg>
#include <cstddef>
#include <cstdint>
#include <cstdio>
#include <cstdlib>

#include "../../include/pds_hip.h"

namespace pds {

inline const char* debug_switch(const char* name) {
    static const bool armed = []() {
        const char* e = std::getenv("PDS_DEBUG_SWITCHES");
        return e && e[0] == '1';
    }();
    return armed ? std::getenv(name) : nullptr;
}
inline bool debug_switch_off(const char* name) {
    const char* e = debug_switch(name);
    return e && e[0] == '0';
}
// ... 38 lines not shown
        return m;
    }
};

#define PDS_REQUIRE(cond, ...)                       \
    do {                                             \
        if (!(cond)) return pds::set_error(-1, __VA_ARGS__); \
    } while (0)

struct Src {
    const float* p;
    const float* scale;
    const float* shift;
    int per_plane;
    int bcast_d;
    int id = -1;
    int normed = 0;
    const float* bound = nullptr;
    int bound_n = 0;
    int bounded = 0;
    int cb8 = 0;
};

inline Src plain_src(const float* p) { return Src{p, nullptr, nullptr, 0, 0}; }
inline Src no_src() { return Src{nullptr, nullptr, nullptr, 0, 0}; }

struct Geom {
    int n, c, d, h, w;
    __host__ __device__ size_t plane() const { return (size_t)h * w; }
    __host__ __device__ size_t volume() const { return (size_t)d * h * w; }
    __host__ __device__ size_t numel() const { return (size_t)n * c * d * h * w; }
};

struct PackJob {
    const float* src = nullptr;
    float* dst = nullptr;
    unsigned* mask = nullptr;
    int cout = 0, cin = 0, mblocks = 0, kc = 4, taps = 9;
    int mode = 0;
    int total = 0;
};
int launch_multi_pack(const PackJob* jobs, int count, hipStream_t s);

enum PackPhase { kPackInline = 0, kPackCollect = 1, kPackDone = 2 };
struct PackSink {
    PackPhase phase = kPackInline;
    PackJob* jobs = nullptr;
    int count = 0, capacity = 0;
    bool push(const PackJob& j) {
        if (count >= capacity) return false;
        jobs[count++] = j;
        return true;
    }
};

struct ConvLayer {
    Src a, b;
    Geom in;
    const float* weight;
    const float* bias;
    float* out;
    Geom out_g;
    int kd;
    int stride;
    int lrelu;
    int stat_per_plane;
    double* partials;
    float* packed;
    const float* l0A = nullptr;
    const float* l0G = nullptr;
    const float* l0G2 = nullptr;
    size_t l0_cstride = 0;
    int l0_rs = 0;
    int out_batch_channels = 0;
    int d_begin = 0;
    float* side_out = nullptr;
    int plane_weight_sets = 0;
    PackSink* sink = nullptr;
    int out_cb8 = 0;
    const float* l1B = nullptr;
    const float* l1H = nullptr;
    unsigned l1_bstride = 0, l1_hstride = 0, l1_edge = 0;
    int l1_P = 0, l1_d0 = 0;
};

int launch_conv_direct(const ConvLayer& L, hipStream_t s);
int conv_direct_tiles_for(const Geom& out_g, int stride);

struct DeconvLayer {
    Src a, b;
    Geom in;
    const float* weight;
    const float* bias;
    float* out;
    Geom out_g;
    int kd;
    int lrelu;
    double* partials;
    float* packed;
    PackSink* sink = nullptr;
};
int launch_deconv_direct(const DeconvLayer& L, hipStream_t s);
int deconv_direct_tiles(const Geom& out_g);

struct KsChainFold {
    const float* gamma;
    const float* beta;
    float* scale;
    float* shift;
    float* mean;
    float* rstd;
    float* bound;
    int groups, per_group, channels;
    double count;
};
struct KsChain {
    int count = 0;
    struct alignas(8) Slot {
        unsigned char bytes[384];
    } storage[12];
};
constexpr int kKsChainSyncWords = 64;
constexpr int kKsChainStateWords = 2048;
bool conv3d_ks_chain_enabled();
int conv3d_ks_chain_add(KsChain& chain, const ConvLayer& L, const KsChainFold& fold, bool* taken);
int deconv3d_ks_chain_add(KsChain& chain, const DeconvLayer& L, const KsChainFold& fold, bool* taken);
int conv3d_ks_chain_launch(KsChain& chain, unsigned* sync_words, hipStream_t s);

int launch_in_finalize(const double* partials, int groups, int per_group, double count,
                       const float* gamma, const float* beta, int channels, int groups_per_channel_block,
                       float* scale, float* shift, float* mean, float* rstd, hipStream_t s, float* bound = nullptr);

size_t in_bwd_scratch_doubles(const Geom& g);
int launch_in_bwd(const float* g, const float* t, const Geom& geom, int per_plane, const float* mean,
                  const float* rstd, const float* gamma, double* scratch, float* m1, float* m2, float* dz,
                  float* dgamma, float* dbeta, float* dbias, int accumulate_params, hipStream_t s,
                  float* dz_amax = nullptr);
constexpr int kDzAmaxSlots = 1024;
int channel_sum_splits(const Geom& g);
int launch_channel_sum(const float* dz, const Geom& g, float* db, int accumulate, double* scratch, hipStream_t s,
                       float* amax = nullptr);
int launch_flip_weights(const float* w, float* wf, int cout, int cin, int taps, hipStream_t s);
int launch_bwd_data(int transposed, int kd, int stride, const float* dz, const float* w, float* dx, const Geom& in,
                    const Geom& out, hipStream_t s);
size_t bwd_weight_scratch_doubles(int transposed, int kd, const Geom& in, const Geom& out);
int launch_bwd_weight(int transposed, int kd, int stride, const Src& a, const Src& b, const float* dz, float* dw,
                      const Geom& in, const Geom& out, int accumulate, double* scratch, hipStream_t s);
bool wgrad_up_full_mfma_supported(int transposed, int kd, const Src& b, const Geom& in, const Geom& out);
size_t wgrad_up_full_mfma_scratch_floats(const Geom& in);
int launch_wgrad_up_full_mfma(const Src& a, const float* dz, float* dw, const Geom& in, int accumulate, float* scratch,
                              hipStream_t s);
bool wgrad3d_s2_mfma_supported(int transposed, int kd, int stride, const Geom& in, const Geom& out);
size_t wgrad3d_s2_mfma_scratch_floats(int transposed, const Geom& in, const Geom& out);
int launch_wgrad3d_s2_mfma(int transposed, const Src& a, const Src& b, const float* dz, float* dw, const Geom& in,
                           const Geom& out, int accumulate, float* scratch, hipStream_t s);
bool wgrad3d_mfma_supported(int transposed, int kd, int stride, const Geom& in, const Geom& out);
size_t wgrad3d_mfma_scratch_floats(const Geom& in, const Geom& out);
int launch_wgrad3d_mfma(const Src& a, const Src& b, const float* dz, float* dw, const Geom& in, const Geom& out,
                        int accumulate, float* scratch, hipStream_t s);
bool wgrad2d_mfma_supported(int transposed, int kd, int stride, const Src& b, const Geom& in, const Geom& out);
size_t wgrad2d_mfma_scratch_floats(const Geom& in, const Geom& out);
int launch_wgrad2d_mfma(const Src& a, const Src& b, const Src& dz, float* dw, const Geom& in, const Geom& out,
                        int accumulate, float* scratch, hipStream_t s);
bool wgrad2d_x3_supported(const Src& a, const Src& b, const Src& dz, const Geom& in, const Geom& out);
int launch_wgrad2d_x3(const Src& a, const Src& b, const Src& dz, float* partial, int workgroups, const Geom& in,
                      const Geom& out, hipStream_t s);
int launch_wgrad_reduce_f32(const float* partial, size_t wcount, int parts, float* dw, int accumulate, hipStream_t s);
int launch_grad_add(float* dst, const float* src, size_t count, int accumulate, hipStream_t s);
int launch_grad_reduce_d(float* dst, const float* src, const Geom& g, int accumulate, hipStream_t s);
int launch_shift_concat_bwd(const float* g, float* dleft, float* dright, int batch, int channels, int h, int w,
                            int d_begin, int d_count, hipStream_t s);

int launch_materialize(const Src& a, const Src& b, const Geom& g, float* out, hipStream_t s, float* amax = nullptr);
int materialize_records(const Geom& g);
int launch_materialize_l0(const Src& a, const Geom& g, const float* A, const float* G, const float* G2,
                          size_t l0_cstride, int l0_rs, int d_begin, float* out, hipStream_t s, float* amax = nullptr);
int materialize_l0_records(const Geom& g);

int launch_left_right_check(const float* dl, const float* dr, unsigned char* lv, unsigned char* rv, float* lf,
                            float* rf, int rows, int w, float max_difference, hipStream_t s);

size_t speckle_workspace_bytes(int batch, int h, int w);
size_t speckle_max_pixels();
int launch_speckle_filter(const float* disparity, const unsigned char* valid, unsigned char* keep, float* filtered,
                          int* sizes, int batch, int h, int w, float max_difference, int max_size, float fill,
                          void* workspace, hipStream_t s);

int launch_median_filter(const float* disparity, const unsigned char* valid, float* filtered, unsigned char* ok,
                         int batch, int h, int w, int kernel_size, int fill_holes, int min_valid, float fill,
                         hipStream_t s);

struct RectifyMapsArgs {
    double inverse_projection[9];
    double camera[5];
    double distortion[5];
};
struct ReprojectArgs {
    float matrix[16];
    float min_confidence;
    int first;
};
int launch_rectify_maps(const RectifyMapsArgs& a, float* map_x, float* map_y, int h, int w, hipStream_t s);
int launch_remap(const void* image, int layout, const float* map_x, const float* map_y, float* out, int batch, int h_in,
                 int w_in, int h_out, int w_out, float border, int reverse_channels, hipStream_t s);
int launch_reproject(const ReprojectArgs& a, const float* disparity, const unsigned char* valid, const float* confidence,
                     float* points, float* depth, int total, int h, int w, hipStream_t s);

int launch_subpixel_map(const float* sim, float* disp, int batch, int planes, int height, int width,
                        int taps_lo, int taps_hi, int step, hipStream_t s, float* conf = nullptr);

template <bool NEG_INF>
__device__ __forceinline__ float softmax_mass_update(float S, float v, float best) {
    const float d = v - best;
    const float e = __builtin_amdgcn_exp2f(-fabsf(d) * 1.44269504088896341f);
    if constexpr (NEG_INF) return d > 0.f ? fmaf(S, e, 1.f) : (d == d ? S + e : S);
    return d > 0.f ? fmaf(S, e, 1.f) : S + e;
}

int launch_shift_concat(const float* left, const float* right, float* out, int batch, int channels,
                        int h, int w, int d_begin, int d_count, hipStream_t s);

int launch_l0_combine(const float* A, const float* G, const float* G2, size_t cstride, float* x0, int batch,
                      int channels, int h, int w, int d_begin, int d_count, hipStream_t s, float* amax = nullptr);
int l0_combine_records(int batch, int channels, int d_count);
int launch_l0_combine_bwd(const float* g, float* gy_a, float* gy_gs, float* gy_g, float* gy_g2, int batch,
                          int channels, int h, int w, int d_begin, int d_count, hipStream_t s);
int launch_first_weight_grads(const float* dwl, const float* dws, const float* dwg, float* dw0, int cout, int cin_half,
                              hipStream_t s);
int launch_crop_left1_add(const float* a, const float* b, float* out, size_t rows, int w, hipStream_t s);
int launch_l0_stack_inputs(const float* left, const float* right, float* out, size_t bc_count, int h, int w,
                           int planes, int pad, hipStream_t s);

constexpr int kL1Planes = 5;
int launch_l1_stack_inputs(const float* y3, float* x4, int batch, int channels, int h, int w, hipStream_t s);
int launch_l1_weights(const float* w1, const float* b1, float* w4, float* bias4, int cout, int channels, hipStream_t s);
int l1_combine_tiles(int h, int w);
int launch_l1_combine(const float* y4, const float* corr, const float* corr0, float* t1, double* partials,
                      int batch, int channels, int h, int w, int d_begin, int d_count, hipStream_t s);
int launch_column_weights(const float* wt, int cin_total, int cin_off, int channels, int cout, float* out,
                          hipStream_t s);
int launch_l0_column_fix(const float* G, const float* R, const float* wcol, float* G2, float* A, int zero_cols,
                         size_t cstride, int rs, int co, int batch, int channels, int cout, int h, int w, int d_begin,
                         int d_count, hipStream_t s);
int launch_l1_column_terms(const float* G, const float* G2, const float* wcol, float* corr, float* corr0,
                           size_t cstride, int rs, int co, int batch, int channels, int cout, int h, int w, int d_begin,
                           int d_count, hipStream_t s);
int launch_l1_weights2(const float* w1, const float* b1, float* w2, float* bias2, int cout, int channels,
                       hipStream_t s);
__host__ __device__ size_t l1_blocked_b_floats(int h, int w);
__host__ __device__ size_t l1_blocked_h_floats(int h, int w, int pad, int d_count);
__host__ __device__ size_t l1_blocked_edge_offset_floats(int h, int w, int pad);
int launch_l1_blocked(const float* y4, const float* corr, const float* corr0, float* Bc, float* Hx, int batch, int channels,
                      int h, int w, int pad, int d_begin, int d_count, hipStream_t s);

int launch_pad_left1(const float* in, float* out, size_t rows, int w, hipStream_t s);
int launch_split_first_weights(const float* w0, const float* b0, float* wl, float* wr, float* wr2, float* bias3,
                               int cout, int cin_half, hipStream_t s);

int image_stats_chunks(int h, int w);
int launch_image_stats(const float* img, int nc, int h, int w, double* partials, hipStream_t s);
// ... 158 lines not shown
```

practicaldeepstereo_nips2018_amd/csrc/conv2d_t8.hip:

```cpp
#include <atomic>
#include <type_traits>

#include "common.hpp"

namespace pds {

namespace {

constexpr int C2_THREADS = 256;
constexpr int C2_CIN = 64, C2_COUT = 8, C2_KC = 4, C2_CHUNKS = C2_CIN / C2_KC;
constexpr int C2_TY = 16, C2_NB = 2, C2_TX = 16 * C2_NB, C2_RP = C2_TY / 8;
constexpr int C2_YT = C2_TY + 2, C2_XT = C2_TX + 2, C2_RS = 36;
constexpr int C2_PART = C2_YT * C2_RS * 8;
constexpr int C2_BUF = 2 * C2_PART;
constexpr int C2_AFRAGS = C2_CHUNKS * 3 * 2;
constexpr int C2_ABYTES = C2_AFRAGS * 64 * 8;
constexpr int C2_NPOS = C2_YT * C2_XT;
constexpr int C2_POS = (C2_NPOS + C2_THREADS - 1) / C2_THREADS;
static_assert(C2_RS >= C2_XT, "LDS row");
typedef float f32x4 __attribute__((ext_vector_type(4)));
typedef _Float16 f16x4 __attribute__((ext_vector_type(4)));

struct C2Args {
    Src a, b;
    const float* __restrict__ w;
    const float* __restrict__ bias;
    float* __restrict__ out;
    int N, D, H, W;
    int lrelu;
    int tiles_x, tiles_y, tiles;
};

__device__ __forceinline__ void c2_split(const float (&v)[4], f16x4& hi, f16x4& lo) {
    pds_u32x2 h, l;
    split_quad_f16(v, h, l);
    hi = __builtin_bit_cast(f16x4, h);
    lo = __builtin_bit_cast(f16x4, l);
}

struct C2Scales {
    float ws, as, unscale;
};
__device__ __forceinline__ float c2_uniform(float v) {
    return __builtin_bit_cast(float, __builtin_amdgcn_readfirstlane(__builtin_bit_cast(int, v)));
}
__device__ __forceinline__ C2Scales c2_scales(const C2Args& A, bool two, float* red) {
    float m[3] = {0.f, 0.f, 0.f};
    for (int i = threadIdx.x; i < C2_COUT * C2_CIN * 9; i += blockDim.x) m[0] = fmaxf(m[0], fabsf(A.w[i]));
    for (int i = threadIdx.x; i < A.a.bound_n; i += blockDim.x) {
        const float v = fabsf(A.a.bound[i]);
        m[1] = fmaxf(m[1], v == v ? v : __builtin_inff());
    }
    if (two)
        for (int i = threadIdx.x; i < A.b.bound_n; i += blockDim.x) {
            const float v = fabsf(A.b.bound[i]);
            m[2] = fmaxf(m[2], v == v ? v : __builtin_inff());
        }
    const int wave = threadIdx.x >> 6, waves = (blockDim.x + 63) >> 6;
#pragma unroll
    for (int k = 0; k < 3; ++k) {
        m[k] = wave_max(m[k]);
        if ((threadIdx.x & 63) == 0) red[wave * 3 + k] = m[k];
    }
    __syncthreads();
    float r[3] = {0.f, 0.f, 0.f};
    for (int w = 0; w < waves; ++w)
#pragma unroll
        for (int k = 0; k < 3; ++k) r[k] = fmaxf(r[k], red[w * 3 + k]);
    __syncthreads();
    C2Scales S;
    S.ws = c2_uniform(pow2_scale(r[0], kHalfTarget));
    S.as = c2_uniform(pow2_scale(r[1] + r[2], kHalfTarget));
    S.unscale = c2_uniform((1.f / S.ws) * (1.f / S.as));
    return S;
}

}

template <bool TWO, bool NA, bool NB2>
__global__ __launch_bounds__(C2_THREADS, 2) void conv2d_t8_kernel(const C2Args A) {
    extern __shared__ __attribute__((aligned(16))) unsigned char lds[];
    unsigned char* abuf = lds;
    unsigned char* ibuf = lds + C2_ABYTES;

    const int tid = threadIdx.x;
    const int lane = tid & 63;
    const int wave = __builtin_amdgcn_readfirstlane(tid >> 6);
    const int n16 = lane & 15, q = lane >> 4;
    const size_t plane = (size_t)A.H * A.W;
    const size_t cstride = (size_t)A.D * plane;
    const int cbytes = (int)(cstride * sizeof(float));
    const __amdgpu_buffer_rsrc_t ra = __builtin_amdgcn_make_buffer_rsrc(
        const_cast<float*>(A.a.p), 0, (int)((size_t)A.N * C2_CIN * cstride * sizeof(float)), 0x00020000);
    const __amdgpu_buffer_rsrc_t rb = __builtin_amdgcn_make_buffer_rsrc(
        const_cast<float*>(TWO ? A.b.p : A.a.p), 0, (int)((size_t)A.N * C2_CIN * cstride * sizeof(float)), 0x00020000);
    const __amdgpu_buffer_rsrc_t ro = __builtin_amdgcn_make_buffer_rsrc(
        A.out, 0, (int)((size_t)A.N * C2_COUT * cstride * sizeof(float)), 0x00020000);

    const C2Scales SC = c2_scales(A, TWO, reinterpret_cast<float*>(ibuf));
    for (int e = tid; e < C2_CHUNKS * 3 * 64; e += C2_THREADS) {
        const int l = e & 63, f = e >> 6;
        const int m = l & 15, oc = m >> 1, py = m & 1, yi = l >> 4, dy = yi - py;
        const int chunk = f / 3, dx = f % 3;
        float wv[4];
#pragma unroll
        for (int i = 0; i < 4; ++i)
            wv[i] = (dy >= 0 && dy <= 2)
                        ? A.w[((size_t)oc * C2_CIN + chunk * C2_KC + i) * 9 + dy * 3 + dx] * SC.ws
                        : 0.f;
        f16x4 hi, lo;
        c2_split(wv, hi, lo);
        *reinterpret_cast<f16x4*>(abuf + ((size_t)(f * 2 + 0) * 64 + l) * 8) = hi;
        *reinterpret_cast<f16x4*>(abuf + ((size_t)(f * 2 + 1) * 64 + l) * 8) = lo;
    }
// ... 55 lines not shown
        const int c0 = (g % C2_CHUNKS) * C2_KC;
        const int soff = __builtin_amdgcn_readfirstlane(sbase + c0 * cbytes);
#pragma unroll
        for (int k = 0; k < C2_POS; ++k) {
#pragma unroll
            for (int ch = 0; ch < C2_KC; ++ch) {
                va[SET][k][ch] =
                    __builtin_bit_cast(float, __builtin_amdgcn_raw_buffer_load_b32(ra, goff[k], soff + ch * cbytes, 0));
                if (TWO)
                    vb[SET][k][ch] = __builtin_bit_cast(
                        float, __builtin_amdgcn_raw_buffer_load_b32(rb, goff[k], soff + ch * cbytes, 0));
            }
            inside_regs[SET][k] = inside[k];
        }
#pragma unroll
        for (int ch = 0; ch < C2_KC; ++ch) {
            if (NA) {
                const int gi = __builtin_amdgcn_readfirstlane(gidx + (c0 + ch) * stride_a);
                vs[SET][ch] = A.a.scale[gi];
                vh[SET][ch] = A.a.shift[gi];
            }
            if (TWO && NB2) {
                const int gi = __builtin_amdgcn_readfirstlane(gch + (c0 + ch) * stride_b);
                vs2[SET][ch] = A.b.scale[gi];
                vh2[SET][ch] = A.b.shift[gi];
            }
        }
    };
    auto stash = [&](unsigned char* buf, auto set_c) {
        constexpr int SET = decltype(set_c)::value;
        float cs[C2_KC], cs2[C2_KC], chs[C2_KC];
#pragma unroll
        for (int ch = 0; ch < C2_KC; ++ch) {
            cs[ch] = NA ? vs[SET][ch] * SC.as : SC.as;
            cs2[ch] = (TWO && NB2) ? vs2[SET][ch] * SC.as : SC.as;
            chs[ch] = ((NA ? vh[SET][ch] : 0.f) + ((TWO && NB2) ? vh2[SET][ch] : 0.f)) * SC.as;
        }
#pragma unroll
        for (int k = 0; k < C2_POS; ++k) {
            float v[4];
#pragma unroll
            for (int ch = 0; ch < C2_KC; ++ch) {
                float t = cs[ch] * va[SET][k][ch];
                if (TWO) t = fmaf(cs2[ch], vb[SET][k][ch], t);
                if (NA || (TWO && NB2)) t = fmaf(chs[ch], inside_regs[SET][k], t);
                v[ch] = t;
            }
            f16x4 hi, lo;
            c2_split(v, hi, lo);
            *reinterpret_cast<f16x4*>(buf + lo_off[k]) = hi;
            *reinterpret_cast<f16x4*>(buf + C2_PART + lo_off[k]) = lo;
        }
    };

    const float bscale = SC.ws * SC.as;
    const float bias0 = (A.bias ? A.bias[2 * q] : 0.f) * bscale, bias1 = (A.bias ? A.bias[2 * q + 1] : 0.f) * bscale;
    const int b_base = ((2 * C2_RP * wave + q) * C2_RS + n16) * 8;
    const unsigned out_lane = (unsigned)((size_t)(2 * q) * cstride + n16) * 4u;
    const unsigned out_c1 = (unsigned)cstride * 4u;

    using S0 = std::integral_constant<int, 0>;
    using S1 = std::integral_constant<int, 1>;
    using S2 = std::integral_constant<int, 2>;
    using S3 = std::integral_constant<int, 3>;
    int fetched_tile = -1;
    auto fetch_chunk = [&](int g, auto set_c) {
        const int gf = min(g, total_chunks - 1);
        if (gf / C2_CHUNKS != fetched_tile) {
            fetched_tile = gf / C2_CHUNKS;
            prepare(fetched_tile, goff, inside, sbase, gidx, gch);
        }
        fetch(gf, set_c);
    };
    if (total_chunks > 0) {
        fetch_chunk(0, S0());
        stash(ibuf, S0());
        fetch_chunk(1, S1());
        fetch_chunk(2, S2());
        fetch_chunk(3, S3());
    }
    __syncthreads();

    f32x4 acc[C2_RP][C2_NB];
    TilePos Pcur = tile_pos(0);
    auto step = [&](int g, auto set_stash, auto set_fetch) {
        const int c = g % C2_CHUNKS;
        if (c == 0) {
            Pcur = tile_pos(g / C2_CHUNKS);
#pragma unroll
            for (int p = 0; p < C2_RP; ++p)
#pragma unroll
                for (int j = 0; j < C2_NB; ++j) acc[p][j] = f32x4{bias0, bias0, bias1, bias1};
        }
        const int gf = min(g + DEPTH, total_chunks - 1);
        const bool new_tile = gf / C2_CHUNKS != fetched_tile;
        if (new_tile) prepare(gf / C2_CHUNKS, goff_n, inside_n, sbase_n, gidx_n, gch_n);
        fetched_tile = gf / C2_CHUNKS;

        const unsigned char* buf = ibuf + (g & 1) * C2_BUF + b_base;
        stash(ibuf + ((g + 1) & 1) * C2_BUF, set_stash);
#pragma unroll
        for (int k = 0; k < C2_POS; ++k) {
            inside[k] = new_tile ? inside_n[k] : inside[k];
            goff[k] = new_tile ? goff_n[k] : goff[k];
        }
        sbase = new_tile ? sbase_n : sbase;
        gidx = new_tile ? gidx_n : gidx;
        gch = new_tile ? gch_n : gch;
        fetch(gf, set_fetch);
        const unsigned char* af = abuf + ((size_t)c * 3 * 2 * 64 + lane) * 8;
#pragma unroll
        for (int dx = 0; dx < 3; ++dx) {
            const f16x4 a_hi = *reinterpret_cast<const f16x4*>(af + (dx * 2 + 0) * 512);
            const f16x4 a_lo = *reinterpret_cast<const f16x4*>(af + (dx * 2 + 1) * 512);
#pragma unroll
            for (int p = 0; p < C2_RP; ++p)
#pragma unroll
                for (int j = 0; j < C2_NB; ++j) {
                    const unsigned char* bp = buf + ((2 * p) * C2_RS + 16 * j + dx) * 8;
                    const f16x4 b_hi = *reinterpret_cast<const f16x4*>(bp);
                    const f16x4 b_lo = *reinterpret_cast<const f16x4*>(bp + C2_PART);
                    acc[p][j] = __builtin_amdgcn_mfma_f32_16x16x16f16(a_hi, b_lo, acc[p][j], 0, 0, 0);
                    acc[p][j] = __builtin_amdgcn_mfma_f32_16x16x16f16(a_lo, b_hi, acc[p][j], 0, 0, 0);
                    acc[p][j] = __builtin_amdgcn_mfma_f32_16x16x16f16(a_hi, b_hi, acc[p][j], 0, 0, 0);
                }
        }
#pragma unroll
        for (int i = 0; i < 3 * C2_RP * C2_NB * 3; ++i) {
            __builtin_amdgcn_sched_group_barrier(0x008, 1, 0);
            __builtin_amdgcn_sched_group_barrier(0x100, 1, 0);
            __builtin_amdgcn_sched_group_barrier(0x002, 4, 0);
            __builtin_amdgcn_sched_group_barrier(0x200, 1, 0);
            __builtin_amdgcn_sched_group_barrier(0x020, 1, 0);
        }
        if (c == C2_CHUNKS - 1) {
            const int out_base = (int)((size_t)Pcur.nb * C2_COUT * cstride * sizeof(float));
#pragma unroll
            for (int p = 0; p < C2_RP; ++p)
#pragma unroll
                for (int r = 0; r < 4; ++r) {
                    const int h = r >> 1, y = Pcur.y0 + 2 * (C2_RP * wave + p) + (r & 1);
                    const int row_bytes = __builtin_amdgcn_readfirstlane(
                        out_base + (int)(((size_t)Pcur.d * A.H + min(y, A.H - 1)) * A.W + Pcur.x0) * (int)sizeof(float));
#pragma unroll
                    for (int j = 0; j < C2_NB; ++j) {
                        float t = acc[p][j][r] * SC.unscale;
                        if (A.lrelu) t = fmaxf(t, t * kLeakySlope);
                        const bool ok = y < A.H && Pcur.x0 + 16 * j + n16 < A.W;
                        __builtin_amdgcn_raw_buffer_store_b32(__builtin_bit_cast(int, t), ro,
                                                              ok ? out_lane + (h ? out_c1 : 0u) + 64u * j : ~0u, row_bytes, 0);
                    }
                }
        }
        __syncthreads();
    };
    for (int g = 0; g < total_chunks; g += 4) {
        step(g, S1(), S0());
        step(g + 1, S2(), S1());
        step(g + 2, S3(), S2());
        step(g + 3, S0(), S3());
    }
}

constexpr int C2W_THREADS = 512;
constexpr int C2W_MAXW = 352;
typedef unsigned u32x4 __attribute__((ext_vector_type(4)));

template <bool TWO, int NBH, int C2W_TY, int C2W_ITEMS>
__global__ __launch_bounds__(C2W_THREADS, 2) void conv2d_t8w_kernel(const C2Args A) {
    constexpr int C2W_YT = C2W_TY + 2;
    extern __shared__ __attribute__((aligned(16))) unsigned char lds[];
    unsigned char* abuf = lds;
    unsigned char* ibuf = lds + C2_ABYTES;
    const int RSW = A.W + 4, QW = A.W >> 2;
    const int part_bytes = C2W_YT * RSW * 8, buf_bytes = 2 * part_bytes;

    const int tid = threadIdx.x;
    const int lane = tid & 63;
    const int wave = __builtin_amdgcn_readfirstlane(tid >> 6);
    const int pair = wave & 3, half = wave >> 2;
    const int n16 = lane & 15, q = lane >> 4;
    const size_t plane = (size_t)A.H * A.W;
    const size_t cstride = (size_t)A.D * plane;
    const int cbytes = (int)(cstride * sizeof(float));
    const __amdgpu_buffer_rsrc_t ra = __builtin_amdgcn_make_buffer_rsrc(
        const_cast<float*>(A.a.p), 0, (int)((size_t)A.N * C2_CIN * cstride * sizeof(float)), 0x00020000);
    const __amdgpu_buffer_rsrc_t rb = __builtin_amdgcn_make_buffer_rsrc(
        const_cast<float*>(TWO ? A.b.p : A.a.p), 0, (int)((size_t)A.N * C2_CIN * cstride * sizeof(float)), 0x00020000);
    const __amdgpu_buffer_rsrc_t ro = __builtin_amdgcn_make_buffer_rsrc(
        A.out, 0, (int)((size_t)A.N * C2_COUT * cstride * sizeof(float)), 0x00020000);

    const C2Scales SC = c2_scales(A, TWO, reinterpret_cast<float*>(ibuf));
    for (int e = tid; e < C2_CHUNKS * 3 * 64; e += C2W_THREADS) {
        const int l = e & 63, f = e >> 6;
        const int m = l & 15, oc = m >> 1, py = m & 1, yi = l >> 4, dy = yi - py;
        const int chunk = f / 3, dx = f % 3;
        float wv[4];
#pragma unroll
        for (int i = 0; i < 4; ++i)
            wv[i] = (dy >= 0 && dy <= 2)
                        ? A.w[((size_t)oc * C2_CIN + chunk * C2_KC + i) * 9 + dy * 3 + dx] * SC.ws
                        : 0.f;
        f16x4 hi, lo;
        c2_split(wv, hi, lo);
        *reinterpret_cast<f16x4*>(abuf + ((size_t)(f * 2 + 0) * 64 + l) * 8) = hi;
        *reinterpret_cast<f16x4*>(abuf + ((size_t)(f * 2 + 1) * 64 + l) * 8) = lo;
    }
    for (int e = tid; e < 2 * 2 * C2W_YT * 2; e += C2W_THREADS) {
        const int side = e & 1, row = e >> 1;
        *reinterpret_cast<unsigned long long*>(ibuf + ((size_t)row * RSW + (side ? A.W + 2 : 1)) * 8) = 0ull;
    }

    const int xcd = blockIdx.x & 7, slot = blockIdx.x >> 3, per_xcd = gridDim.x >> 3;
    const int t_end = (int)(((long long)(xcd + 1) * A.tiles) >> 3);
    const int t_first = (int)(((long long)xcd * A.tiles) >> 3) + slot;
    const int my_tiles = t_first < t_end ? (t_end - t_first + per_xcd - 1) / per_xcd : 0;
    const int total_chunks = my_tiles * C2_CHUNKS;

    int item_row[C2W_ITEMS], item_col[C2W_ITEMS], lo_off[C2W_ITEMS], lo_step[C2W_ITEMS];
    bool item_ok[C2W_ITEMS];
#pragma unroll
    for (int k = 0; k < C2W_ITEMS; ++k) {
        item_ok[k] = tid + C2W_THREADS * k < C2W_YT * QW;
        const int it = min(tid + C2W_THREADS * k, C2W_YT * QW - 1);
        item_row[k] = it / QW;
        item_col[k] = 4 * (it % QW);
        lo_off[k] = item_ok[k] ? (item_row[k] * RSW + 2 + item_col[k]) * 8 : 0;
        lo_step[k] = item_ok[k] ? 16 : 0;
    }

    struct TilePos {
        int nb, d, y0;
    };
    auto tile_pos = [&](int local) {
        const int t = t_first + min(local, my_tiles - 1) * per_xcd;
        TilePos p;
        p.y0 = (t % A.tiles_y) * C2W_TY;
        const int r = t / A.tiles_y;
        p.d = r % A.D;
        p.nb = r / A.D;
        return p;
    };

    unsigned goff[C2W_ITEMS], goff_n[C2W_ITEMS];
// ... 24 lines not shown
#pragma unroll
        for (int k = 0; k < C2W_ITEMS; ++k) {
#pragma unroll
            for (int ch = 0; ch < C2_KC; ++ch) {
                va[SET][k][ch] = __builtin_bit_cast(
                    f32x4, __builtin_amdgcn_raw_buffer_load_b128(ra, goff[k], soff + ch * cbytes, 0));
                if (TWO)
                    vb[SET][k][ch] = __builtin_bit_cast(
                        f32x4, __builtin_amdgcn_raw_buffer_load_b128(rb, goff[k], soff + ch * cbytes, 0));
            }
            inside_regs[SET][k] = inside[k];
        }
#pragma unroll
        for (int ch = 0; ch < C2_KC; ++ch) {
            const int gi = __builtin_amdgcn_readfirstlane(gidx + (c0 + ch) * stride_a);
            vs[SET][ch] = A.a.scale[gi];
            vh[SET][ch] = A.a.shift[gi];
        }
    };
    typedef _Float16 f16x8 __attribute__((ext_vector_type(8)));
    auto stash = [&](unsigned char* buf, auto set_c) {
        constexpr int SET = decltype(set_c)::value;
        float cs[C2_KC], chs[C2_KC];
#pragma unroll
        for (int ch = 0; ch < C2_KC; ++ch) {
            cs[ch] = vs[SET][ch] * SC.as;
            chs[ch] = vh[SET][ch] * SC.as;
        }
#pragma unroll
        for (int k = 0; k < C2W_ITEMS; ++k)
#pragma unroll
            for (int pp = 0; pp < 2; ++pp) {
                f16x8 hi2, lo2;
#pragma unroll
                for (int e = 0; e < 2; ++e) {
                    const int px = 2 * pp + e;
                    float v[4];
#pragma unroll
                    for (int ch = 0; ch < C2_KC; ++ch) {
                        float t = cs[ch] * va[SET][k][ch][px];
                        if (TWO) t = fmaf(SC.as, vb[SET][k][ch][px], t);
                        v[ch] = fmaf(chs[ch], inside_regs[SET][k], t);
                    }
                    f16x4 hi, lo;
                    c2_split(v, hi, lo);
#pragma unroll
                    for (int i = 0; i < 4; ++i) {
                        hi2[4 * e + i] = hi[i];
                        lo2[4 * e + i] = lo[i];
                    }
                }
                *reinterpret_cast<f16x8*>(buf + lo_off[k] + pp * lo_step[k]) = hi2;
                *reinterpret_cast<f16x8*>(buf + part_bytes + lo_off[k] + pp * lo_step[k]) = lo2;
            }
    };

    const float bscale = SC.ws * SC.as;
    const float bias0 = (A.bias ? A.bias[2 * q] : 0.f) * bscale, bias1 = (A.bias ? A.bias[2 * q + 1] : 0.f) * bscale;
    const int b_base = ((2 * pair + q) * RSW + 16 * half * NBH + n16 + 1) * 8;
    const unsigned out_lane = (unsigned)((size_t)(2 * q) * cstride + 16 * half * NBH + n16) * 4u;
    const unsigned out_c1 = (unsigned)cstride * 4u;

    using S0 = std::integral_constant<int, 0>;
    using S1 = std::integral_constant<int, 1>;
    int fetched_tile = -1;
    auto fetch_chunk = [&](int g, auto set_c) {
        const int gf = min(g, total_chunks - 1);
        if (gf / C2_CHUNKS != fetched_tile) {
            fetched_tile = gf / C2_CHUNKS;
            prepare(fetched_tile, goff, inside, sbase, gidx);
        }
        fetch(gf, set_c);
    };
    __syncthreads();
    if (total_chunks > 0) {
        fetch_chunk(0, S0());
        stash(ibuf, S0());
        fetch_chunk(1, S1());
        fetch_chunk(2, S0());
    }
    __syncthreads();

    f32x4 acc[NBH];
    TilePos Pcur = tile_pos(0);
#ifdef PDS_C2W_TIMING
    long long tmw[5] = {0, 0, 0, 0, 0};
#endif
    auto step = [&](int g, auto set_c) {
        const int c = g % C2_CHUNKS;
        if (c == 0) {
            Pcur = tile_pos(g / C2_CHUNKS);
#pragma unroll
            for (int j = 0; j < NBH; ++j) acc[j] = f32x4{bias0, bias0, bias1, bias1};
        }
        const int gf = min(g + 3, total_chunks - 1);
        const bool new_tile = gf / C2_CHUNKS != fetched_tile;
        if (new_tile) prepare(gf / C2_CHUNKS, goff_n, inside_n, sbase_n, gidx_n);
        fetched_tile = gf / C2_CHUNKS;

        const unsigned char* buf = ibuf + (g & 1) * buf_bytes + b_base;
#ifdef PDS_C2W_TIMING
        const long long tt0 = __builtin_readcyclecounter();
#endif
        stash(ibuf + ((g + 1) & 1) * buf_bytes, set_c);
#ifdef PDS_C2W_TIMING
        asm volatile("s_waitcnt lgkmcnt(0)" ::: "memory");
        const long long tt1 = __builtin_readcyclecounter();
#endif
#pragma unroll
        for (int k = 0; k < C2W_ITEMS; ++k) {
            inside[k] = new_tile ? inside_n[k] : inside[k];
            goff[k] = new_tile ? goff_n[k] : goff[k];
        }
        sbase = new_tile ? sbase_n : sbase;
        gidx = new_tile ? gidx_n : gidx;
        fetch(gf, set_c);
#ifdef PDS_C2W_TIMING
        const long long tt2 = __builtin_readcyclecounter();
#endif
        const unsigned char* af = abuf + ((size_t)c * 3 * 2 * 64 + lane) * 8;
#pragma unroll
        for (int dx = 0; dx < 3; ++dx) {
            const f16x4 a_hi = *reinterpret_cast<const f16x4*>(af + (dx * 2 + 0) * 512);
            const f16x4 a_lo = *reinterpret_cast<const f16x4*>(af + (dx * 2 + 1) * 512);
#pragma unroll
            for (int j = 0; j < NBH; ++j) {
                const unsigned char* bp = buf + (16 * j + dx) * 8;
                const f16x4 b_hi = *reinterpret_cast<const f16x4*>(bp);
                const f16x4 b_lo = *reinterpret_cast<const f16x4*>(bp + part_bytes);
                acc[j] = __builtin_amdgcn_mfma_f32_16x16x16f16(a_hi, b_lo, acc[j], 0, 0, 0);
                acc[j] = __builtin_amdgcn_mfma_f32_16x16x16f16(a_lo, b_hi, acc[j], 0, 0, 0);
                acc[j] = __builtin_amdgcn_mfma_f32_16x16x16f16(a_hi, b_hi, acc[j], 0, 0, 0);
            }
        }
#ifndef PDS_C2W_TIMING
#pragma unroll
        for (int i = 0; i < 3 * NBH * 3; ++i) {
            __builtin_amdgcn_sched_group_barrier(0x008, 1, 0);
            __builtin_amdgcn_sched_group_barrier(0x100, 1, 0);
            __builtin_amdgcn_sched_group_barrier(0x002, 4, 0);
            __builtin_amdgcn_sched_group_barrier(0x200, 1, 0);
            __builtin_amdgcn_sched_group_barrier(0x020, 1, 0);
        }
#else
        const long long tt3 = __builtin_readcyclecounter();
        tmw[0] += tt1 - tt0; tmw[1] += tt2 - tt1; tmw[2] += tt3 - tt2;
#endif
        if (c == C2_CHUNKS - 1) {
            const int out_base = (int)((size_t)Pcur.nb * C2_COUT * cstride * sizeof(float));
#pragma unroll
            for (int r = 0; r < 4; ++r) {
                const int h = r >> 1, y = Pcur.y0 + 2 * pair + (r & 1);
                const int row_bytes = __builtin_amdgcn_readfirstlane(
                    out_base + (int)(((size_t)Pcur.d * A.H + min(y, A.H - 1)) * A.W) * (int)sizeof(float));
#pragma unroll
                for (int j = 0; j < NBH; ++j) {
                    float t = acc[j][r] * SC.unscale;
                    if (A.lrelu) t = fmaxf(t, t * kLeakySlope);
                    const bool ok = 2 * pair < C2W_TY && y < A.H && 16 * (half * NBH + j) + n16 < A.W;
                    __builtin_amdgcn_raw_buffer_store_b32(__builtin_bit_cast(int, t), ro,
                                                          ok ? out_lane + (h ? out_c1 : 0u) + 64u * j : ~0u, row_bytes, 0);
                }
            }
        }
#ifdef PDS_C2W_TIMING
        const long long tt4 = __builtin_readcyclecounter();
#endif
        __syncthreads();
#ifdef PDS_C2W_TIMING
        tmw[3] += __builtin_readcyclecounter() - tt4;
        tmw[4] += 1;
#endif
    };
#ifdef PDS_C2W_TIMING
    const long long t_all = __builtin_readcyclecounter();
#endif
    for (int g = 0; g < total_chunks; g += 2) {
        step(g, S1());
        step(g + 1, S0());
    }
#ifdef PDS_C2W_TIMING
    if (lane == 0 && (blockIdx.x % 61) == 0 && (wave == 0 || wave == 5))
        printf("[t8w] wg %d wave %d: total %lld | stash(+wait) %lld fetch-issue %lld mfma %lld barrier %lld over %lld chunks (%d tiles)\n",
               (int)blockIdx.x, wave, (long long)__builtin_readcyclecounter() - t_all, tmw[0], tmw[1], tmw[2], tmw[3], tmw[4], my_tiles);
#endif
}

namespace {

bool c2t8_enabled() {
    static const bool on = []() {
        const char* e = debug_switch("PDS_CONV2D_T8");
        return !(e && e[0] == '0');
    }();
    return on;
}

template <bool TWO, bool NA, bool NB2>
int launch_c2t8(const C2Args& A, hipStream_t s) {
    constexpr size_t lds_bytes = (size_t)C2_ABYTES + 2 * C2_BUF;
    static std::atomic<unsigned> attr_done{0};
    if (DeviceOnce once{attr_done}) {
        (void)hipFuncSetAttribute(reinterpret_cast<const void*>(&conv2d_t8_kernel<TWO, NA, NB2>),
                                  hipFuncAttributeMaxDynamicSharedMemorySize, (int)(160 * 1024));
    }
    int wgs = 512;
    if (wgs > A.tiles) wgs = (A.tiles + 7) / 8 * 8;
    hipLaunchKernelGGL((conv2d_t8_kernel<TWO, NA, NB2>), dim3(wgs), dim3(C2_THREADS), lds_bytes, s, A);
    return check_launch("conv2d_t8");
}

}

bool c2t8_wide(const ConvLayer& L) {
    static const bool on = []() {
        const char* e = debug_switch("PDS_CONV2D_T8W");
        return !(e && e[0] == '0');
    }();
    if (!on) return false;
    if (!L.a.scale || (L.b.p && L.b.scale)) return false;
    return (L.in.w & 3) == 0 && L.in.w >= 64 && L.in.w <= C2W_MAXW && L.in.h >= 8;
}

template <bool TWO, int NBH, int TY, int ITEMS>
int launch_c2t8w(C2Args& A, hipStream_t s) {
    A.tiles_x = 1;
    A.tiles_y = (A.H + TY - 1) / TY;
    A.tiles = A.N * A.D * A.tiles_y;
    const size_t lds_bytes = (size_t)C2_ABYTES + 2 * 2 * (size_t)(TY + 2) * (A.W + 4) * 8 + 2 * (size_t)(A.W + 4) * 8 + 256;
    static std::atomic<unsigned> attr_done{0};
    static int cus[32] = {0};
    int dev = 0;
    (void)hipGetDevice(&dev);
    if (DeviceOnce once{attr_done}) {
        (void)hipFuncSetAttribute(reinterpret_cast<const void*>(&conv2d_t8w_kernel<TWO, NBH, TY, ITEMS>),
                                  hipFuncAttributeMaxDynamicSharedMemorySize, (int)(160 * 1024));
        int n = 0;
        (void)hipDeviceGetAttribute(&n, hipDeviceAttributeMultiprocessorCount, dev);
        cus[dev & 31] = n > 0 ? n : 256;
    }
    int wgs = cus[dev & 31] / 8 * 8;
    if (wgs > A.tiles) wgs = (A.tiles + 7) / 8 * 8;
    const int probe = probe_before("conv2d_t8w", s);
    hipLaunchKernelGGL((conv2d_t8w_kernel<TWO, NBH, TY, ITEMS>), dim3(wgs), dim3(C2W_THREADS), lds_bytes, s, A);
    probe_after(probe, A.tiles, s);
    return check_launch("conv2d_t8w");
}

int c2t8w_rows(int w) {
    static const int forced = []() {
        const char* e = debug_switch("PDS_CONV2D_T8W_ROWS");
        return e ? atoi(e) : 0;
    }();
    if (forced == 8 || forced == 6) return forced;
    return 8 * (w >> 2) <= C2W_THREADS ? 6 : 8;
}

bool conv2d_t8_supported(const ConvLayer& L) {
    if (!c2t8_enabled()) return false;
    if (L.kd != 1 || L.stride != 1 || L.in.c != C2_CIN || L.out_g.c != C2_COUT) return false;
    if (L.l0A || L.side_out || L.plane_weight_sets > 0) return false;
    if (!L.a.bounded) return false;
    if (L.b.p && !L.b.bounded) return false;
    if (L.b.p && L.b.bcast_d) return false;
    if ((size_t)L.in.n * C2_CIN * L.in.d * L.in.h * L.in.w >= ((size_t)1 << 29)) return false;
    const long tiles = (long)L.in.n * L.in.d * ((L.in.h + C2_TY - 1) / C2_TY) * ((L.in.w + C2_TX - 1) / C2_TX);
    return tiles < (1L << 30);
}

int launch_conv2d_t8(const ConvLayer& L, hipStream_t s) {
    C2Args A;
    A.a = L.a;
    A.b = L.b;
    A.w = L.weight;
    A.bias = L.bias;
    A.out = L.out;
    A.N = L.in.n;
    A.D = L.in.d;
    A.H = L.in.h;
    A.W = L.in.w;
    A.lrelu = L.lrelu;
    A.tiles_x = (A.W + C2_TX - 1) / C2_TX;
    A.tiles_y = (A.H + C2_TY - 1) / C2_TY;
    A.tiles = A.N * A.D * A.tiles_y * A.tiles_x;
    if (!A.a.bound || A.a.bound_n <= 0 || (L.b.p && (!A.b.bound || A.b.bound_n <= 0)))
        return set_error(-1, "conv2d_t8: a source without a range bound");
    if (c2t8_wide(L)) {
        const int blocks = (A.W + 15) / 16, nbh = (blocks + 1) / 2;
        const int rows = c2t8w_rows(A.W), items = ((rows + 2) * (A.W >> 2) + C2W_THREADS - 1) / C2W_THREADS;
        if (nbh <= 8 && rows == 6 && items == 1)
            return L.b.p ? launch_c2t8w<true, 8, 6, 1>(A, s) : launch_c2t8w<false, 8, 6, 1>(A, s);
        if (nbh <= 8) return L.b.p ? launch_c2t8w<true, 8, 8, 2>(A, s) : launch_c2t8w<false, 8, 8, 2>(A, s);
        return L.b.p ? launch_c2t8w<true, 11, 8, 2>(A, s) : launch_c2t8w<false, 11, 8, 2>(A, s);
    }
    const bool na = L.a.scale != nullptr, nb2 = L.b.p && L.b.scale;
    if (L.b.p) {
        if (na) return nb2 ? launch_c2t8<true, true, true>(A, s) : launch_c2t8<true, true, false>(A, s);
        return nb2 ? launch_c2t8<true, false, true>(A, s) : launch_c2t8<true, false, false>(A, s);
    }
    return na ? launch_c2t8<false, true, false>(A, s) : launch_c2t8<false, false, false>(A, s);
}

}
```

practicaldeepstereo_nips2018_amd/csrc/conv3d_t8x.hip:

```cpp
#include "persistent3d.hpp"

namespace pds {

namespace {

template <int NB, int P>
struct TXCfg {
    static constexpr int XT = 16 * NB + 2, YT = 6;
    static constexpr int YX = YT * XT;
    static constexpr int PART = T8_C * YX * 8;
    static constexpr int BUF = P * PART;
    static constexpr int SLOTS_HALF = 4 * YX;
    static constexpr int SPT = (SLOTS_HALF + P3D_THREADS - 1) / P3D_THREADS;
    static constexpr int PRODUCTS = P == 3 ? 6 : 3;
};

template <int P>
__device__ __forceinline__ void tx_split(const float (&v)[4], u32x2 (&part)[P]) {
    if constexpr (P == 2) {
        pds_u32x2 h, l;
        split_quad_f16(v, h, l);
        part[0] = __builtin_bit_cast(u32x2, h);
        part[1] = __builtin_bit_cast(u32x2, l);
    } else {
// ... 174 lines not shown
        walk.next(px, py, pz);
        prepare(px, py, pz);
        unsigned char* nxt = lds + (cur ^ 1) * C::BUF;
        const unsigned char* bp = lds + cur * C::BUF + b_base;

        f32x4 acc[NB];
#pragma unroll
        for (int j = 0; j < NB; ++j) acc[j] = f32x4{0.f, 0.f, 0.f, 0.f};
#pragma unroll
        for (int g = 0; g < 2; ++g) {
            fetch_half(g);
#pragma unroll
            for (int dy = 0; dy < 3; ++dy) {
#pragma unroll
                for (int dx = 0; dx < 3; ++dx) {
                    u32x2 bf[NB][P];
#pragma unroll
                    for (int j = 0; j < NB; ++j)
#pragma unroll
                        for (int p = 0; p < P; ++p)
                            bf[j][p] = *reinterpret_cast<const u32x2*>(
                                bp + p * C::PART + ((g * 4 * C::YT + dy) * C::XT + dx + 16 * j) * 8);
#pragma unroll
                    for (int c = 0; c < C::PRODUCTS; ++c) {
                        const int pa = P == 3 ? (c == 0 ? 0 : c == 1 ? 2 : c == 2 ? 1 : c == 3 ? 0 : c == 4 ? 1 : 0) : (c == 1 ? 1 : 0);
                        const int pb = P == 3 ? (c == 0 ? 2 : c == 1 ? 0 : c == 2 ? 1 : c == 3 ? 1 : c == 4 ? 0 : 0) : (c == 0 ? 1 : 0);
#pragma unroll
                        for (int j = 0; j < NB; ++j) acc[j] = tx_mma<P>(af[g][dy * 3 + dx][pa], bf[j][pb], acc[j]);
                    }
                }
            }
            stash_half(g, nxt);
        }

        {
            const int y = y0 + wave;
#pragma unroll
            for (int r = 0; r < 4; ++r) {
                const int h = r >> 1, z = z0 + (r & 1);
                const bool rowok = EXACT || (z < A.D && y < A.H);
                const int row_bytes = EXACT ? ((z * A.H + y) * A.W + x0) * (int)sizeof(float)
                                            : ((min(z, A.D - 1) * A.H + min(y, A.H - 1)) * A.W + x0) * (int)sizeof(float);
#pragma unroll
                for (int j = 0; j < NB; ++j) {
                    float t = fmaf(acc[j][r], unscale, h ? bias1 : bias0);
                    if (A.lrelu) t = fmaxf(t, t * kLeakySlope);
                    const bool ok = EXACT || (rowok && x0 + 16 * j + n16 < A.W);
                    const unsigned off = out_lane + (h ? out_c1 : 0u) + 64u * j;
                    __builtin_amdgcn_raw_buffer_store_b32(__builtin_bit_cast(int, t), ro, ok ? off : ~0u, row_bytes, 0);
                    t = ok ? t : 0.f;
                    ssum[h] += t;
                    ssq[h] = fmaf(t, t, ssq[h]);
                }
            }
        }
        __syncthreads();
        cur ^= 1;
    }

    if (A.partials) {
        double* red = reinterpret_cast<double*>(lds);
        red[tid * 4 + 0] = (double)ssum[0];
        red[tid * 4 + 1] = (double)ssq[0];
        red[tid * 4 + 2] = (double)ssum[1];
        red[tid * 4 + 3] = (double)ssq[1];
        __syncthreads();
        if (tid < T8_C * 2) {
            const int oc = tid >> 1, k = tid & 1, qq = oc >> 1, hh = oc & 1;
            double sum = 0.0;
            for (int wv = 0; wv < 4; ++wv)
                for (int n = 0; n < 16; ++n) sum += red[(wv * 64 + qq * 16 + n) * 4 + hh * 2 + k];
            A.partials[(((size_t)nb * T8_C + oc) * A.records + blockIdx.x) * 2 + k] = sum;
        }
    }
}

namespace {

template <int NB, int P, int SRC, bool EXACT>
int launch_t8x(const T8Args& A, int batch, hipStream_t s) {
    using C = TXCfg<NB, P>;
    constexpr size_t lds_bytes = (size_t)2 * C::BUF + 4 * T8_C * sizeof(float);
    static_assert(lds_bytes <= 160 * 1024, "LDS");
    return launch_persistent<&conv3d_t8x_kernel<NB, P, SRC, EXACT>>(EXACT ? "conv3d_t8x<exact>" : "conv3d_t8x<guarded>",
                                                                    "conv3d_t8x", A, A.records, batch, lds_bytes, s);
}

}

bool conv3d_t8x_enabled() {
    static const bool on = !debug_switch_off("PDS_CONV3D_T8X");
    return on;
}

int launch_conv3d_t8x(const ConvLayer& L, const T8Plan& plan, hipStream_t s) {
    const T8Args A = t8_args(L, plan);
    const int nb = plan.nb, src = plan.src;
    const bool exact = plan.exact, fp16 = plan.certified;
    if (!fp16 && src == 2) return set_error(-1, "conv3d_t8x: two sources need range certificates");
#define PDS_T8X_CASE(NB_, SRC_)                                                                                  \
    if (nb == NB_ && src == SRC_) {                                                                              \
        if (fp16) return exact ? launch_t8x<NB_, 2, SRC_, true>(A, L.in.n, s) : launch_t8x<NB_, 2, SRC_, false>(A, L.in.n, s); \
        if constexpr (SRC_ != 2)                                                                                 \
            return exact ? launch_t8x<NB_, 3, SRC_, true>(A, L.in.n, s) : launch_t8x<NB_, 3, SRC_, false>(A, L.in.n, s);       \
    }
    PDS_T8X_CASE(2, 0)
    PDS_T8X_CASE(2, 1)
    PDS_T8X_CASE(2, 2)
    PDS_T8X_CASE(3, 0)
    PDS_T8X_CASE(3, 1)
    PDS_T8X_CASE(3, 2)
#undef PDS_T8X_CASE
    return set_error(-1, "conv3d_t8x: no configuration");
}

}
```

practicaldeepstereo_nips2018_amd/csrc/misc.hip:

```cpp
#include "common.hpp"

namespace pds {

__global__ __launch_bounds__(256) void shift_concat_kernel(const float* __restrict__ left,
                                                           const float* __restrict__ right,
                                                           float* __restrict__ out, int batch, int C, int h,
                                                           int w, int d_begin, int d_count) {
    const size_t row_count = (size_t)d_count * batch * 2 * C * h;
    for (size_t row = blockIdx.x; row < row_count; row += gridDim.x) {
        size_t r = row;
        const int y = (int)(r % h);
        r /= h;
        const int c2 = (int)(r % (2 * C));
        r /= (2 * C);
        const int b = (int)(r % batch);
        const int d = d_begin + (int)(r / batch);
        float* dst = out + row * w;
        if (c2 < C) {
            const float* src = left + (((size_t)b * C + c2) * h + y) * w;
            for (int x = threadIdx.x; x < w; x += 256) dst[x] = src[x];
        } else {
            const float* src = right + (((size_t)b * C + (c2 - C)) * h + y) * w;
            for (int x = threadIdx.x; x < w; x += 256) dst[x] = (x >= d) ? src[x - d] : 0.f;
        }
// ... 653 lines not shown
    const float* Bp = y4 + ((size_t)(n * C + g * 8) * 2) * plane;
    const float* Hp = Bp + plane;
    float v[8];
    float* dst;
    if (item < nb) {
#pragma unroll
        for (int c = 0; c < 8; ++c) v[c] = Bp[(size_t)c * 2 * plane + item];
        dst = Bc + (size_t)ng * l1_blocked_b_floats(h, w) + (size_t)item * 8;
    } else if (item < nb + nh) {
        const int i = item - nb, y = i / HW, j = i % HW;
#pragma unroll
        for (int c = 0; c < 8; ++c) v[c] = j >= pad ? Hp[(size_t)c * 2 * plane + (size_t)y * W2 + (j - pad)] : 0.f;
        dst = Hx + (size_t)ng * l1_blocked_h_floats(h, w, pad, d_count) + (size_t)i * 8;
    } else {
        const int i = item - nb - nh, slot = i & 1, y = (i >> 1) % h, dl = (i >> 1) / h, d = d_begin + dl;
#pragma unroll
        for (int c = 0; c < 8; ++c) {
            const size_t nc = (size_t)n * C + g * 8 + c;
            const float* hrow = Hp + (size_t)c * 2 * plane + (size_t)y * W2;
            float t = 0.f;
            if (d == 0) {
                if (slot == 0) t = hrow[2] + corr0[nc * h + y];
            } else {
                const int u = w - 2 + slot - d;
                t = (u >= -2 ? hrow[u + 2] : 0.f) + corr[((nc * h + y) * d_count + dl) * 2 + slot];
            }
            v[c] = t;
        }
        dst = Hx + (size_t)ng * l1_blocked_h_floats(h, w, pad, d_count) + l1_blocked_edge_offset_floats(h, w, pad) +
              (size_t)i * 8;
    }
    typedef float f32x4 __attribute__((ext_vector_type(4)));
    reinterpret_cast<f32x4*>(dst)[0] = f32x4{v[0], v[1], v[2], v[3]};
    reinterpret_cast<f32x4*>(dst)[1] = f32x4{v[4], v[5], v[6], v[7]};
}

int launch_l1_blocked(const float* y4, const float* corr, const float* corr0, float* Bc, float* Hx, int batch, int channels,
                      int h, int w, int pad, int d_begin, int d_count, hipStream_t s) {
    const int items = h * (w + 2) + h * (pad + w + 2) + d_count * h * 2;
    hipLaunchKernelGGL(l1_blocked_kernel, dim3((items + 255) / 256, batch * (channels / 8)), dim3(256), 0, s, y4, corr, corr0,
                       Bc, Hx, channels, h, w, pad, d_begin, d_count);
    return check_launch("l1_blocked");
}

int launch_l1_stack_inputs(const float* y3, float* x4, int batch, int channels, int h, int w, hipStream_t s) {
    const size_t total = (size_t)batch * 2 * channels * kL1Planes * h * (w + 2);
    unsigned bx = (unsigned)((total + 255) / 256);
    if (bx > 8192) bx = 8192;
    hipLaunchKernelGGL(l1_stack_inputs_kernel, dim3(bx), dim3(256), 0, s, y3, x4, batch, channels, h, w);
    return check_launch("l1_stack_inputs");
}

int launch_l1_weights(const float* w1, const float* b1, float* w4, float* bias4, int cout, int channels,
                      hipStream_t s) {
    const int total = kL1Planes * cout * 2 * channels * 9;
    hipLaunchKernelGGL(l1_weights_kernel, dim3((total + 255) / 256), dim3(256), 0, s, w1, b1, w4, bias4, cout,
                       channels);
    return check_launch("l1_weights");
}

int l1_combine_tiles(int h, int w) {
    const size_t quads = (size_t)h * ((w + 3) / 4);
    return (int)((quads + 255) / 256);
}

int launch_l1_combine(const float* y4, const float* corr, const float* corr0, float* t1, double* partials,
                      int batch, int channels, int h, int w, int d_begin, int d_count, hipStream_t s) {
    for (int first = 0; first < d_count; first += kL1MaxPlanes) {
        const int n = d_count - first < kL1MaxPlanes ? d_count - first : kL1MaxPlanes;
        const dim3 grid(l1_combine_tiles(h, w), batch * channels);
        if (corr && !t1)
            hipLaunchKernelGGL((l1_combine_kernel<true, false>), grid, dim3(256), 0, s, y4, corr, corr0, t1, partials,
                               channels, h, w, d_begin, first, n, d_count);
        else if (corr)
            hipLaunchKernelGGL(l1_combine_kernel<true>, grid, dim3(256), 0, s, y4, corr, corr0, t1, partials, channels, h,
                               w, d_begin, first, n, d_count);
        else
            hipLaunchKernelGGL(l1_combine_kernel<false>, grid, dim3(256), 0, s, y4, corr, corr0, t1, partials, channels,
                               h, w, d_begin, first, n, d_count);
    }
    return check_launch("l1_combine");
}

}
```

practicaldeepstereo_nips2018_amd/matching.py:

```python
import ctypes

import torch
from torch import nn

from practicaldeepstereo_nips2018_amd import _lib
from practicaldeepstereo_nips2018_amd import network_blocks


class MatchingOperation(nn.Module):

    def __init__(self,
                 number_of_concatenated_descriptor_features=128,
                 number_of_features=64,
                 number_of_compact_matching_signature_features=8,
                 number_of_residual_blocks=2):
        super(MatchingOperation, self).__init__()
        if number_of_concatenated_descriptor_features % 2 != 0:
            raise ValueError('"number_of_concatenated_descriptor_features" should be even.')
        self._number_of_residual_blocks = number_of_residual_blocks
        layers = [network_blocks.convolution_3x3(number_of_concatenated_descriptor_features,
                                                 number_of_features)]
        for _ in range(number_of_residual_blocks):
            layers.append(network_blocks.ResidualBlock(number_of_features))
        layers.append(network_blocks.convolution_3x3(
# ... 79 lines not shown
        params, keep = module.native_params()
        grads, tensor_of = _lib.gradient_buffers(module)
        grad_params, keep_grads = module.native_params(tensor_of)
        grad_x = torch.empty_like(x)
        nbytes = lib.pds_matching_operation_bwd_workspace_bytes(ctypes.byref(params), n, h, w)
        ws = torch.empty(max(int(nbytes), 256), dtype=torch.uint8, device=x.device)
        fws = _lib.saved_workspace(ctx, 'matching')
        with torch.cuda.device(x.device):
            _lib.check(lib.pds_matching_operation_bwd(
                ctypes.byref(params), ctypes.byref(grad_params), _lib.ptr(x), _lib.ptr(grad_out),
                _lib.ptr(grad_x), n, h, w, _lib.ptr(fws), fws.numel(), _lib.ptr(ws), ws.numel(),
                _lib.stream_handle(x.device)), 'pds_matching_operation_bwd')
        del keep, keep_grads
        ctx.forward_workspace = None
        return (None, grad_x) + tuple(grads[id(p)] for p in module.parameters())


class _ShiftConcatFunction(torch.autograd.Function):

    @staticmethod
    def forward(ctx, left, right, begin, count):
        lib = _lib.load()
        batch, channels, h, w = left.shape
        out = torch.empty((count, batch, 2 * channels, h, w), dtype=torch.float32, device=left.device)
        with torch.cuda.device(left.device):
            _lib.check(lib.pds_shift_concat_fwd(
                _lib.ptr(left), _lib.ptr(right), _lib.ptr(out), batch, channels, h, w,
                begin, count, _lib.stream_handle(left.device)), 'pds_shift_concat_fwd')
        ctx.geometry = (batch, channels, h, w, begin, count)
        return out

    @staticmethod
    def backward(ctx, grad_out):
        lib = _lib.load()
        batch, channels, h, w, begin, count = ctx.geometry
        grad_out = grad_out.contiguous()
        grad_left = torch.empty((batch, channels, h, w), dtype=torch.float32, device=grad_out.device)
        grad_right = torch.empty_like(grad_left)
        with torch.cuda.device(grad_out.device):
            _lib.check(lib.pds_shift_concat_bwd(
                _lib.ptr(grad_out), _lib.ptr(grad_left), _lib.ptr(grad_right), batch, channels, h, w,
                begin, count, _lib.stream_handle(grad_out.device)), 'pds_shift_concat_bwd')
        return grad_left, grad_right, None, None


class Matching(_lib.FrozenWeightsMixin, nn.Module):

    def __init__(self, maximum_disparity, operation):
        super(Matching, self).__init__()
        self._maximum_disparity = maximum_disparity
        self._operation = operation
        self._workspace = _lib.Workspace()
        self._disparity_shard = None

    def set_maximum_disparity(self, maximum_disparity):
        self._maximum_disparity = maximum_disparity

    def set_disparity_shard(self, shard):
        self._disparity_shard = shard

    def _plane_range(self):
        if self._disparity_shard is None:
            return 0, self._maximum_disparity + 1
        begin, count = self._disparity_shard
        if begin < 0 or count < 1 or begin + count > self._maximum_disparity + 1:
            raise ValueError('disparity shard (%d, %d) outside [0, %d]' %
                             (begin, count, self._maximum_disparity))
        return begin, count

    def forward(self, left_embedding, right_embedding):
        left = _lib.require_gpu_tensor(left_embedding, 'left_embedding', 4)
        right = _lib.require_gpu_tensor(right_embedding, 'right_embedding', 4)
        if left.shape != right.shape:
            raise ValueError('left and right embeddings differ in shape: %s vs %s' %
                             (tuple(left.shape), tuple(right.shape)))
        begin, count = self._plane_range()
        operation = self._operation
        needs_grad = torch.is_grad_enabled() and (
            left.requires_grad or right.requires_grad or
            (isinstance(operation, nn.Module) and any(p.requires_grad for p in operation.parameters())))
        if (isinstance(operation, MatchingOperation) and operation.supports_fused_matching()
                and left.size(1) == operation.number_of_descriptor_features):
            if not needs_grad:
                return _FusedMatchingFunction.apply(self, left, right, begin, count,
                                                    *operation.parameters())
            _lib.warn_eval_with_grad(self)
            if operation.supports_native_training():
                return _TrainMatchingFunction.apply(self, left, right, begin, count, *operation.parameters())
        return self._forward_generic(left, right, begin, count)

    def _forward_generic(self, left, right, begin, count):
        concatenated = _ShiftConcatFunction.apply(left, right, begin, count)
        return torch.stack([self._operation(plane) for plane in concatenated.unbind(0)], dim=2)


class _TrainMatchingFunction(torch.autograd.Function):

    @staticmethod
    def forward(ctx, module, left, right, begin, count, *unused_parameters):
        lib = _lib.load()
        operation = module._operation
        left, right = left.contiguous(), right.contiguous()
        batch, _, h, w = left.shape
        params, keep = operation.native_params()
        out = torch.empty((batch, operation.number_of_signature_features, count, h, w),
                          dtype=torch.float32, device=left.device)
        nbytes = _lib.planned_bytes(lib.pds_matching_train_workspace_bytes(ctypes.byref(params), batch, h, w, count),
                                    'pds_matching_train_workspace_bytes')
        ws = torch.empty(nbytes, dtype=torch.uint8, device=left.device)
        with torch.cuda.device(left.device):
            _lib.check(lib.pds_matching_train_fwd(
                ctypes.byref(params), _lib.ptr(left), _lib.ptr(right), _lib.ptr(out), batch, h, w, begin, count,
                _lib.ptr(ws), ws.numel(), _lib.stream_handle(left.device)), 'pds_matching_train_fwd')
        del keep
        ctx.module = module
        ctx.geometry = (begin, count)
        ctx.forward_workspace = ws
        ctx.save_for_backward(left, right)
        return out

    @staticmethod
    def backward(ctx, grad_out):
        lib = _lib.load()
        operation = ctx.module._operation
        left, right = ctx.saved_tensors
        begin, count = ctx.geometry
        batch, _, h, w = left.shape
        grad_out = grad_out.contiguous()
        params, keep = operation.native_params()
        grads, tensor_of = _lib.gradient_buffers(operation)
        grad_params, keep_grads = operation.native_params(tensor_of)
        grad_left, grad_right = torch.empty_like(left), torch.empty_like(right)
        nbytes = _lib.planned_bytes(lib.pds_matching_bwd_workspace_bytes(ctypes.byref(params), batch, h, w, count),
                                    'pds_matching_bwd_workspace_bytes')
        ws = torch.empty(nbytes, dtype=torch.uint8, device=left.device)
        fws = _lib.saved_workspace(ctx, 'matching')
        with torch.cuda.device(left.device):
            _lib.check(lib.pds_matching_bwd(
                ctypes.byref(params), ctypes.byref(grad_params), _lib.ptr(left), _lib.ptr(right), _lib.ptr(grad_out),
                _lib.ptr(grad_left), _lib.ptr(grad_right), batch, h, w, begin, count, _lib.ptr(fws), fws.numel(),
                _lib.ptr(ws), ws.numel(), _lib.stream_handle(left.device)), 'pds_matching_bwd')
        del keep, keep_grads
        ctx.forward_workspace = None
        return (None, grad_left, grad_right, None, None) + tuple(grads[id(p)] for p in operation.parameters())


class _FusedMatchingFunction(torch.autograd.Function):
    @staticmethod
    def forward(ctx, module, left, right, begin, count, *unused_parameters):
        lib = _lib.load()
        operation = module._operation
        batch, _, h, w = left.shape
        params, keep = operation.native_params()
        out = torch.empty((batch, operation.number_of_signature_features, count, h, w),
                          dtype=torch.float32, device=left.device)
        nbytes = lib.pds_matching_workspace_bytes(ctypes.byref(params), batch, h, w, count)
        ws, resident, token = module._workspace.get_resident(
            nbytes, left.device, _lib.resident_key(module, operation, (batch, h, w, count)))
        with torch.cuda.device(left.device):
            _lib.check(lib.pds_matching_fwd(
                ctypes.byref(params), _lib.ptr(left), _lib.ptr(right), _lib.ptr(out),
                batch, h, w, begin, count, _lib.ptr(ws), ws.numel(), int(resident),
                _lib.stream_handle(left.device)), 'pds_matching_fwd')
        module._workspace.commit(token)
        del keep
        return out

    @staticmethod
    def backward(ctx, *grads):
        _lib.not_differentiable('Matching (fused inference path)')
```

practicaldeepstereo_nips2018_amd/regularization.py:

```python
import ctypes

import torch
from torch import nn

from practicaldeepstereo_nips2018_amd import _lib
from practicaldeepstereo_nips2018_amd import network_blocks


def _block_params(block, tensor_of=None):
    return _lib.conv_block_params(block.conv, block.norm, tensor_of)


class ContractionBlock3d(nn.Module):

    def __init__(self, number_of_features):
        super(ContractionBlock3d, self).__init__()
        self._downsampling_2x = network_blocks.convolutional_block_3x3x3_stride_2(
            number_of_features, 2 * number_of_features)
        self._smoothing = network_blocks.convolutional_block_3x3x3(
            2 * number_of_features, 2 * number_of_features)
        self._workspace = _lib.Workspace()

    def forward(self, block_input):
        x = _lib.require_gpu_tensor(block_input, 'block_input', 5)
# ... 94 lines not shown
            _lib.check(lib.pds_expansion_block_fwd(
                ctypes.byref(pu), ctypes.byref(ps), _lib.ptr(x), _lib.ptr(shortcut), _lib.ptr(out),
                batch, c, d, h, w, _lib.ptr(ws), ws.numel(), _lib.stream_handle(x.device)),
                'pds_expansion_block_fwd')
        if training:
            ctx.module = module
            ctx.forward_workspace = ws
            ctx.save_for_backward(x, shortcut)
        return out

    @staticmethod
    def backward(ctx, grad_out):
        lib = _lib.load()
        module = ctx.module
        x, shortcut = ctx.saved_tensors
        batch, c, d, h, w = x.shape
        grad_out = grad_out.contiguous()
        grads, tensor_of = _lib.gradient_buffers(module)
        pu, ps = _block_params(module._upsampling_2x), _block_params(module._smoothing)
        gu, gs = _block_params(module._upsampling_2x, tensor_of), _block_params(module._smoothing, tensor_of)
        grad_x, grad_shortcut = torch.empty_like(x), torch.empty_like(shortcut)
        ws = torch.empty(max(int(lib.pds_expansion_block_bwd_workspace_bytes(batch, c, d, h, w)), 256),
                         dtype=torch.uint8, device=x.device)
        fws = _lib.saved_workspace(ctx, 'regularization')
        with torch.cuda.device(x.device):
            _lib.check(lib.pds_expansion_block_bwd(
                ctypes.byref(pu), ctypes.byref(ps), ctypes.byref(gu), ctypes.byref(gs), _lib.ptr(x),
                _lib.ptr(shortcut), _lib.ptr(grad_out), _lib.ptr(grad_x), _lib.ptr(grad_shortcut),
                batch, c, d, h, w, _lib.ptr(fws), fws.numel(), _lib.ptr(ws), ws.numel(),
                _lib.stream_handle(x.device)), 'pds_expansion_block_bwd')
        ctx.forward_workspace = None
        return (None, grad_x, grad_shortcut) + tuple(grads[id(p)] for p in module.parameters())


class Regularization(_lib.FrozenWeightsMixin, nn.Module):

    def __init__(self, number_of_features=8):
        super(Regularization, self).__init__()
        self._smoothing = network_blocks.convolutional_block_3x3x3(
            number_of_features, number_of_features)
        self._contraction_blocks = nn.ModuleList(
            [ContractionBlock3d(number_of_features * scale) for scale in (1, 2, 4, 8)])
        self._expansion_blocks = nn.ModuleList(
            [ExpansionBlock3d(number_of_features * scale) for scale in (16, 8, 4, 2)])
        self._upsample_to_halfsize = network_blocks.transposed_convolutional_block_4x4x4_stride_2(
            number_of_features, number_of_features // 2)
        self._upsample_to_fullsize = network_blocks.transposed_convolution_3x4x4_stride_122(
            number_of_features // 2, 1)
        self._workspace = _lib.Workspace()

    @property
    def number_of_features(self):
        return self._smoothing.conv.in_channels

    def native_params(self, tensor_of=None):
        params = _lib.RegularizationParams()
        params.features = self.number_of_features
        params.smoothing = _block_params(self._smoothing, tensor_of)
        for level in range(4):
            contraction, expansion = self._contraction_blocks[level], self._expansion_blocks[level]
            params.contraction[level][0] = _block_params(contraction._downsampling_2x, tensor_of)
            params.contraction[level][1] = _block_params(contraction._smoothing, tensor_of)
            params.expansion[level][0] = _block_params(expansion._upsampling_2x, tensor_of)
            params.expansion[level][1] = _block_params(expansion._smoothing, tensor_of)
        params.upsample_half = _block_params(self._upsample_to_halfsize, tensor_of)
        params.upsample_full = _lib.conv_block_params(self._upsample_to_fullsize, None, tensor_of)
        return params

    def can_fold_crop(self, estimator):
        taps = -(-estimator._half_support_window // estimator._disparity_step)
        return self.number_of_features == 8 and 1 <= taps <= 4

    def _check_inputs(self, matching_signatures, shortcut_from_left_image):
        ms = _lib.require_gpu_tensor(matching_signatures, 'matching_signatures', 5)
        shortcut = _lib.require_gpu_tensor(shortcut_from_left_image, 'shortcut_from_left_image', 4)
        batch, c, d, h, w = ms.shape
        if c != self.number_of_features:
            raise ValueError('expected %d matching signature features, got %d' % (self.number_of_features, c))
        if tuple(shortcut.shape) != (batch, c, h, w):
            raise ValueError('shortcut of shape %s does not match signatures %s' %
                             (tuple(shortcut.shape), tuple(ms.shape)))
        return ms, shortcut

    def forward(self, matching_signatures, shortcut_from_left_image):
        ms, shortcut = self._check_inputs(matching_signatures, shortcut_from_left_image)
        return _RegularizationFunction.apply(self, ms, shortcut, None, *self.parameters())

    def forward_with_estimator(self, matching_signatures, shortcut_from_left_image, estimator, crop=(0, 0),
                               with_confidence=False, mirror=False):
        ms, shortcut = self._check_inputs(matching_signatures, shortcut_from_left_image)
        fold_mirror = bool(mirror) and self.can_fold_crop(estimator)
        window = (estimator._half_support_window, estimator._disparity_step, int(crop[0]), int(crop[1]),
                  bool(with_confidence), fold_mirror)
        out = _RegularizationFunction.apply(self, ms, shortcut, window, *self.parameters())
        if mirror and not fold_mirror:
            out = tuple(torch.flip(o, [-1]) for o in out) if with_confidence else torch.flip(out, [-1])
        return tuple(out) if with_confidence else out


class _RegularizationFunction(torch.autograd.Function):

    @staticmethod
    def forward(ctx, module, ms, shortcut, estimator_window, *unused_parameters):
        lib = _lib.load()
        batch, _, d, h, w = ms.shape
        params = module.native_params()
        nbytes = lib.pds_regularization_workspace_bytes(ctypes.byref(params), batch, d, h, w)
        if nbytes == 0:
            raise ValueError(lib.pds_last_error().decode())
        training = any(ctx.needs_input_grad) and estimator_window is None
        confidence = None
        if estimator_window is None:
            out = torch.empty((batch, 2 * d, 4 * h, 4 * w), dtype=torch.float32, device=ms.device)
        else:
            crop_top, crop_left = estimator_window[2], estimator_window[3]
            out = torch.empty((batch, 4 * h - crop_top, 4 * w - crop_left), dtype=torch.float32, device=ms.device)
            if estimator_window[4]:
                confidence = torch.empty_like(out)
        token = None
        if training:
            ws, resident = torch.empty(max(int(nbytes), 256), dtype=torch.uint8, device=ms.device), False
        else:
            window = None if estimator_window is None else (estimator_window[0], estimator_window[1])
            ws, resident, token = module._workspace.get_resident(
                nbytes, ms.device, _lib.resident_key(module, module, (batch, d, h, w, window)))
        with torch.cuda.device(ms.device):
            if estimator_window is None:
                _lib.check(lib.pds_regularization_fwd(
                    ctypes.byref(params), _lib.ptr(ms), _lib.ptr(shortcut), _lib.ptr(out),
                    batch, d, h, w, _lib.ptr(ws), ws.numel(), int(resident), _lib.stream_handle(ms.device)),
                    'pds_regularization_fwd')
            elif estimator_window[5]:
                _lib.check(lib.pds_regularization_subpixel_map_mirrored_fwd(
                    ctypes.byref(params), _lib.ptr(ms), _lib.ptr(shortcut), _lib.ptr(out),
                    None if confidence is None else _lib.ptr(confidence),
                    batch, d, h, w, estimator_window[0], estimator_window[1], crop_top, crop_left,
                    _lib.ptr(ws), ws.numel(), int(resident), _lib.stream_handle(ms.device)),
                    'pds_regularization_subpixel_map_mirrored_fwd')
            elif confidence is not None:
                _lib.check(lib.pds_regularization_subpixel_map_confidence_fwd(
                    ctypes.byref(params), _lib.ptr(ms), _lib.ptr(shortcut), _lib.ptr(out), _lib.ptr(confidence),
                    batch, d, h, w, estimator_window[0], estimator_window[1], crop_top, crop_left,
                    _lib.ptr(ws), ws.numel(), int(resident), _lib.stream_handle(ms.device)),
                    'pds_regularization_subpixel_map_confidence_fwd')
            else:
                _lib.check(lib.pds_regularization_subpixel_map_fwd(
                    ctypes.byref(params), _lib.ptr(ms), _lib.ptr(shortcut), _lib.ptr(out),
                    batch, d, h, w, estimator_window[0], estimator_window[1], crop_top, crop_left,
                    _lib.ptr(ws), ws.numel(), int(resident), _lib.stream_handle(ms.device)),
                    'pds_regularization_subpixel_map_fwd')
        if token is not None:
            module._workspace.commit(token)
        if training:
            ctx.module = module
            ctx.forward_workspace = ws
            ctx.save_for_backward(ms, shortcut)
        else:
            ctx.module = None
        if confidence is not None:
            return out, confidence
        return out

    @staticmethod
    def backward(ctx, grad_out, *unused_grad_confidence):
        module = ctx.module
        if module is None:
            _lib.not_differentiable('Regularization fused with SubpixelMap (inference only, estimator.py:19)')
        lib = _lib.load()
        ms, shortcut = ctx.saved_tensors
        batch, _, d, h, w = ms.shape
        grad_out = grad_out.contiguous()
        params = module.native_params()
        grads, tensor_of = _lib.gradient_buffers(module)
        grad_params = module.native_params(tensor_of)
        grad_ms = torch.empty_like(ms)
        grad_shortcut = torch.empty_like(shortcut)
        nbytes = lib.pds_regularization_bwd_workspace_bytes(ctypes.byref(params), batch, d, h, w)
        ws = torch.empty(max(int(nbytes), 256), dtype=torch.uint8, device=ms.device)
        fws = _lib.saved_workspace(ctx, 'regularization')
        with torch.cuda.device(ms.device):
            _lib.check(lib.pds_regularization_bwd(
                ctypes.byref(params), ctypes.byref(grad_params), _lib.ptr(ms), _lib.ptr(shortcut),
                _lib.ptr(grad_out), _lib.ptr(grad_ms), _lib.ptr(grad_shortcut), batch, d, h, w,
                _lib.ptr(fws), fws.numel(), _lib.ptr(ws), ws.numel(), _lib.stream_handle(ms.device)),
                'pds_regularization_bwd')
        ctx.forward_workspace = None
        return (None, grad_ms, grad_shortcut, None) + tuple(grads[id(p)] for p in module.parameters())
```

Baseline: 433.1 pairs/s.

## Propagate a signature amax bound from matching into regularization's first conv

The final matching conv now writes per-block absolute-max records of the signatures, or a standalone amax kernel derives them. These records are attached to the signatures tensor and handed to new bounded regularization entry points, so the first 3D conv can take a bounded input and skip its own range pass over the large signature volume. The cost is a new cross-module certificate path with tensor-version tracking, plus an extra reduction kernel whenever no bound is attached.

After: 434.0 pairs/s (median of 2 runs). About the same (+0.2%).

```diff
diff --git a/include/pds_hip.h b/include/pds_hip.h
--- a/include/pds_hip.h
+++ b/include/pds_hip.h
@@ -60,6 +60,15 @@
                      void* workspace, size_t workspace_bytes, int weights_resident,
                      pds_stream_t stream);
 
+int pds_matching_signatures_bound_records(const PdsMatchingParams* params, int batch, int h, int w, int d_count);
+int pds_matching_bounded_fwd(const PdsMatchingParams* params,
+                             const float* left, const float* right, float* signatures,
+                             float* signatures_bound , int signatures_bound_records,
+                             int batch, int h, int w, int d_begin, int d_count,
+                             void* workspace, size_t workspace_bytes, int weights_resident,
+                             pds_stream_t stream);
+int pds_signatures_bound_fwd(const float* signatures, size_t count, float* bound, int records, pds_stream_t stream);
+
 size_t pds_matching_operation_workspace_bytes(const PdsMatchingParams* params, int n, int h, int w);
 int pds_matching_operation_fwd(const PdsMatchingParams* params,
                                const float* concatenated, float* signature,
@@ -83,6 +92,13 @@
                            void* workspace, size_t workspace_bytes, int weights_resident,
                            pds_stream_t stream);
 
+int pds_regularization_bounded_fwd(const PdsRegularizationParams* params,
+                                   const float* signatures, const float* signatures_bound ,
+                                   int signatures_bound_records, const float* left_shortcut, float* cost,
+                                   int batch, int d, int h, int w,
+                                   void* workspace, size_t workspace_bytes, int weights_resident,
+                                   pds_stream_t stream);
+
 int pds_regularization_subpixel_map_fwd(const PdsRegularizationParams* params,
                                         const float* signatures, const float* left_shortcut,
                                         float* disparities,
@@ -109,6 +125,16 @@
                                                  int crop_top, int crop_left,
                                                  void* workspace, size_t workspace_bytes,
                                                  int weights_resident, pds_stream_t stream);
+
+int pds_regularization_subpixel_map_bounded_fwd(const PdsRegularizationParams* params,
+                                                const float* signatures, const float* signatures_bound ,
+                                                int signatures_bound_records, const float* left_shortcut,
+                                                float* disparities, float* confidence ,
+                                                int batch, int d, int h, int w,
+                                                int half_support_window, int disparity_step,
+                                                int crop_top, int crop_left, int mirror,
+                                                void* workspace, size_t workspace_bytes,
+                                                int weights_resident, pds_stream_t stream);
 
 size_t pds_contraction_block_workspace_bytes(int batch, int c, int d, int h, int w);
 int pds_contraction_block_fwd(const PdsConvBlockParams* downsampling, const PdsConvBlockParams* smoothing,
@@ -131,6 +157,10 @@
                                const float* x_shift, int x_per_plane, const float* x_bound, float* raw, float* scale,
                                float* shift, int n, int cin, int cout, int d, int h, int w, int kd, int stride,
                                int per_plane, void* workspace, size_t workspace_bytes, pds_stream_t stream);
+int pds_conv_block_bounded_fwd(const PdsConvBlockParams* params, const float* x, const float* x_bound,
+                               int x_bound_records, float* raw, float* scale, float* shift, int n, int cin, int cout,
+                               int d, int h, int w, int kd, int stride, int per_plane, void* workspace,
+                               size_t workspace_bytes, pds_stream_t stream);
 
 size_t pds_regularization_bwd_workspace_bytes(const PdsRegularizationParams* params, int batch, int d, int h, int w);
 int pds_regularization_bwd(const PdsRegularizationParams* params, const PdsRegularizationParams* grads,
diff --git a/practicaldeepstereo_nips2018_amd/_lib.py b/practicaldeepstereo_nips2018_amd/_lib.py
--- a/practicaldeepstereo_nips2018_amd/_lib.py
+++ b/practicaldeepstereo_nips2018_amd/_lib.py
@@ -136,6 +136,10 @@
     'pds_matching_workspace_bytes': (_SZ, [ctypes.POINTER(MatchingParams), _I, _I, _I, _I]),
     'pds_matching_fwd': (_I, [ctypes.POINTER(MatchingParams), _VP, _VP, _VP, _I, _I, _I, _I, _I,
                               _VP, _SZ, _I, _VP]),
+    'pds_matching_signatures_bound_records': (_I, [ctypes.POINTER(MatchingParams), _I, _I, _I, _I]),
+    'pds_matching_bounded_fwd': (_I, [ctypes.POINTER(MatchingParams), _VP, _VP, _VP, _VP, _I, _I, _I, _I, _I, _I,
+                                      _VP, _SZ, _I, _VP]),
+    'pds_signatures_bound_fwd': (_I, [_VP, _SZ, _VP, _I, _VP]),
     'pds_matching_train_workspace_bytes': (_SZ, [ctypes.POINTER(MatchingParams), _I, _I, _I, _I]),
     'pds_matching_train_fwd': (_I, [ctypes.POINTER(MatchingParams), _VP, _VP, _VP, _I, _I, _I, _I, _I, _VP, _SZ, _VP]),
     'pds_matching_bwd_workspace_bytes': (_SZ, [ctypes.POINTER(MatchingParams), _I, _I, _I, _I]),
@@ -147,6 +151,11 @@
     'pds_regularization_workspace_bytes': (_SZ, [ctypes.POINTER(RegularizationParams), _I, _I, _I, _I]),
     'pds_regularization_fwd': (_I, [ctypes.POINTER(RegularizationParams), _VP, _VP, _VP,
                                     _I, _I, _I, _I, _VP, _SZ, _I, _VP]),
+    'pds_regularization_bounded_fwd': (_I, [ctypes.POINTER(RegularizationParams), _VP, _VP, _I, _VP, _VP,
+                                            _I, _I, _I, _I, _VP, _SZ, _I, _VP]),
+    'pds_regularization_subpixel_map_bounded_fwd': (_I, [ctypes.POINTER(RegularizationParams), _VP, _VP, _I, _VP, _VP,
+                                                         _VP, _I, _I, _I, _I, _I, _I, _I, _I, _I, _VP, _SZ, _I,
+                                                         _VP]),
     'pds_regularization_subpixel_map_fwd': (_I, [ctypes.POINTER(RegularizationParams), _VP, _VP, _VP,
                                                  _I, _I, _I, _I, _I, _I, _I, _I, _VP, _SZ, _I, _VP]),
     'pds_regularization_subpixel_map_confidence_fwd': (_I, [ctypes.POINTER(RegularizationParams), _VP, _VP, _VP,
@@ -159,6 +168,8 @@
     'pds_conv_block_fwd': (_I, [ctypes.POINTER(ConvBlockParams), _VP, _VP, _VP, _VP,
                                 _I, _I, _I, _I, _I, _I, _I, _I, _I, _VP, _SZ, _VP]),
     'pds_conv_block_chained_fwd': (_I, [ctypes.POINTER(ConvBlockParams), _VP, _VP, _VP, _I, _VP, _VP, _VP, _VP,
+                                        _I, _I, _I, _I, _I, _I, _I, _I, _I, _VP, _SZ, _VP]),
+    'pds_conv_block_bounded_fwd': (_I, [ctypes.POINTER(ConvBlockParams), _VP, _VP, _I, _VP, _VP, _VP,
                                         _I, _I, _I, _I, _I, _I, _I, _I, _I, _VP, _SZ, _VP]),
     'pds_regularization_bwd_workspace_bytes': (_SZ, [ctypes.POINTER(RegularizationParams), _I, _I, _I, _I]),
     'pds_regularization_bwd': (_I, [ctypes.POINTER(RegularizationParams), ctypes.POINTER(RegularizationParams),
@@ -263,6 +274,42 @@
     return ctypes.c_void_p(torch.cuda.current_stream(device).cuda_stream)
 
 
+_SIGNATURES_BOUND = '_pds_signatures_bound'
+SIGNATURES_BOUND_RECORDS = 512
+
+
+def _version_of(tensor):
+    try:
+        return tensor._version
+    except RuntimeError:
+        return None
+
+
+def attach_signatures_bound(signatures, records):
+    version = _version_of(signatures)
+    if version is not None:
+        setattr(signatures, _SIGNATURES_BOUND, (records, version))
+    return signatures
+
+
+def attached_signatures_bound(signatures):
+    held = getattr(signatures, _SIGNATURES_BOUND, None)
+    if held is None:
+        return None
+    records, version = held
+    if version != _version_of(signatures) or records.device != signatures.device:
+        return None
+    return records
+
+
+def derive_signatures_bound(signatures):
+    records = torch.empty(SIGNATURES_BOUND_RECORDS, dtype=torch.float32, device=signatures.device)
+    with torch.cuda.device(signatures.device):
+        check(load().pds_signatures_bound_fwd(ptr(signatures), signatures.numel(), ptr(records), records.numel(),
+                                              stream_handle(signatures.device)), 'pds_signatures_bound_fwd')
+    return records
+
+
 def conv_block_params(conv, norm=None, tensor_of=None):
     f = tensor_of if tensor_of is not None else (lambda t: t)
     p = ConvBlockParams()
diff --git a/practicaldeepstereo_nips2018_amd/csrc/api.hip b/practicaldeepstereo_nips2018_amd/csrc/api.hip
--- a/practicaldeepstereo_nips2018_amd/csrc/api.hip
+++ b/practicaldeepstereo_nips2018_amd/csrc/api.hip
@@ -169,6 +169,13 @@
     if (kind == 7) L.packed = c.get<float>(conv3d_ks_packed_floats(in.c, cout, 27));
     if (kind == 10) L.packed = c.get<float>(conv3d_nx_packed_floats(in.c, cout));
     if (kind == 9) L.packed = c.get<float>(conv2d_x3_packed_floats(in.c));
+    if (kind == 8 && extra && extra->amax_n > 0) {
+        L.amax = extra->amax;
+        L.amax_n = extra->amax_n;
+        o.bound = extra->amax;
+        o.bound_n = extra->amax_n;
+        o.bounded = true;
+    }
     if ((a.cb8 || b.cb8 || L.out_cb8) && !(kind == 9 && !b.p && conv2d_x3_cb8_ok(L, a.cb8 != 0, L.out_cb8 != 0))) {
         c.run(set_error(-1, "conv_block: a channel-blocked tensor reached a kernel that does not take it"));
         return o;
@@ -433,6 +440,36 @@
     return c.err;
 }
 
+int pds_conv_block_bounded_fwd(const PdsConvBlockParams* params, const float* x, const float* x_bound,
+                               int x_bound_records, float* raw, float* scale, float* shift, int n, int cin, int cout,
+                               int d, int h, int w, int kd, int stride, int per_plane, void* workspace,
+                               size_t workspace_bytes, pds_stream_t stream) {
+    PDS_REQUIRE(params && x && raw && workspace, "conv_block_bounded: null pointer");
+    PDS_REQUIRE(params->weight && params->bias, "conv_block_bounded: null weight/bias");
+    PDS_REQUIRE(n > 0 && cin > 0 && cout > 0 && d > 0 && h > 0 && w > 0, "conv_block_bounded: bad shape");
+    PDS_REQUIRE((kd == 1 || kd == 3) && (stride == 1 || stride == 2) && !(kd == 1 && stride == 2),
+                "conv_block_bounded: unsupported kd=%d stride=%d", kd, stride);
+    PDS_REQUIRE(!x_bound || x_bound_records > 0, "conv_block_bounded: a certificate needs at least one record");
+    if (params->gamma) PDS_REQUIRE(params->beta && scale && shift, "conv_block_bounded: null InstanceNorm outputs");
+    const size_t need = pds_conv_block_workspace_bytes(n, cin, cout, d, h, w, kd, stride, per_plane);
+    PDS_REQUIRE(workspace_bytes >= need, "conv_block_bounded: workspace too small (%zu < %zu)", workspace_bytes, need);
+    Ctx c{(char*)workspace, 0, false, (hipStream_t)stream};
+    Src src = plain_src(x);
+    if (x_bound) {
+        src.bound = x_bound;
+        src.bound_n = x_bound_records;
+        src.bounded = 1;
+    }
+    conv_block(c, src, no_src(), Geom{n, cin, d, h, w}, *params, cout, kd, stride, per_plane, raw, true, scale, shift);
+    return c.err;
+}
+
+int pds_signatures_bound_fwd(const float* signatures, size_t count, float* bound, int records, pds_stream_t stream) {
+    PDS_REQUIRE(signatures && bound, "signatures_bound: null pointer");
+    PDS_REQUIRE(count > 0 && records > 0 && records <= 65535, "signatures_bound: bad count");
+    return launch_tensor_amax(signatures, count, bound, records, (hipStream_t)stream);
+}
+
 int pds_conv_block_chained_fwd(const PdsConvBlockParams* params, const float* x, const float* x_scale,
                                const float* x_shift, int x_per_plane, const float* x_bound, float* raw, float* scale,
                                float* shift, int n, int cin, int cout, int d, int h, int w, int kd, int stride,
diff --git a/practicaldeepstereo_nips2018_amd/csrc/api_internal.hpp b/practicaldeepstereo_nips2018_amd/csrc/api_internal.hpp
--- a/practicaldeepstereo_nips2018_amd/csrc/api_internal.hpp
+++ b/practicaldeepstereo_nips2018_amd/csrc/api_internal.hpp
@@ -206,6 +206,8 @@
     const float* l1H = nullptr;
     unsigned l1_bstride = 0, l1_hstride = 0, l1_edge = 0;
     int l1_P = 0, l1_d0 = 0;
+    float* amax = nullptr;
+    int amax_n = 0;
     bool matching_extras() const { return l0A || side_out || plane_weight_sets > 0; }
 };
 
diff --git a/practicaldeepstereo_nips2018_amd/csrc/api_matching.hip b/practicaldeepstereo_nips2018_amd/csrc/api_matching.hip
--- a/practicaldeepstereo_nips2018_amd/csrc/api_matching.hip
+++ b/practicaldeepstereo_nips2018_amd/csrc/api_matching.hip
@@ -2,7 +2,25 @@
 
 namespace pds {
 
-static void operation_tail(Ctx& c, const PdsMatchingParams& P, const Src& x0, const Geom& g, float* signature) {
+struct SignatureBound {
+    float* records = nullptr;
+    int written = 0;
+};
+
+static void last_conv(Ctx& c, const Src& a, const Src& b, const Geom& g, const PdsMatchingParams& P, float* signatures,
+                      const ConvExtra* base, SignatureBound* sb) {
+    ConvExtra e = base ? *base : ConvExtra{};
+    if (sb) {
+        e.amax = sb->records;
+        e.amax_n = kConv2dT8Records;
+    }
+    const DT o = conv_block(c, a, b, g, P.last, P.signature_features, 1, 1, 1, signatures, true, nullptr, nullptr,
+                            (base || sb) ? &e : nullptr);
+    if (sb) sb->written = (o.bounded && o.bound_n == kConv2dT8Records) ? kConv2dT8Records : 0;
+}
+
+static void operation_tail(Ctx& c, const PdsMatchingParams& P, const Src& x0, const Geom& g, float* signature,
+                           SignatureBound* sb = nullptr) {
     const int F = P.features;
     Src cur = x0;
     DT t2;
@@ -20,9 +38,9 @@
         }
     }
     if (P.residual_blocks > 0)
-        conv_block(c, t2.src(), cur, g, P.last, P.signature_features, 1, 1, 1, signature);
+        last_conv(c, t2.src(), cur, g, P, signature, nullptr, sb);
     else
-        conv_block(c, cur, no_src(), g, P.last, P.signature_features, 1, 1, 1, signature);
+        last_conv(c, cur, no_src(), g, P, signature, nullptr, sb);
 }
 
 static bool fused_matching_supported(const PdsMatchingParams& P, int batch, int h, int w, int d_count) {
@@ -44,7 +62,7 @@
 
 static void matching_pipeline(Ctx& c, const PdsMatchingParams& P, const float* left, const float* right,
                               float* signatures, int batch, int h, int w, int d_begin, int d_count, bool train = false,
-                              MatchingL0* l0_out = nullptr) {
+                              MatchingL0* l0_out = nullptr, SignatureBound* sb = nullptr) {
     const int F = P.features;
     const size_t wn = (size_t)F * F * 9;
     float* w3 = c.get<float>(3 * wn);
@@ -136,7 +154,7 @@
             t.bounded = true;
             x0s.id = c.tape->add(t);
         }
-        operation_tail(c, P, x0s, g, signatures);
+        operation_tail(c, P, x0s, g, signatures, sb);
         return;
     }
     ConvExtra l0;
@@ -148,7 +166,7 @@
     l0.d_begin = d_begin;
     const Src none = no_src();
     if (P.residual_blocks == 0) {
-        conv_block(c, none, none, g, P.last, P.signature_features, 1, 1, 1, signatures, true, nullptr, nullptr, &l0);
+        last_conv(c, none, none, g, P, signatures, &l0, sb);
         return;
     }
     const int cb8_level = [&]() {
@@ -245,8 +263,7 @@
     DT t2 = on_the_fly ? conv_block(c, t1.src(), none, g, P.blocks[1], F, 1, 1, 1, nullptr, true, nullptr, nullptr, &fly)
                        : conv_block(c, t1.src(), none, g, P.blocks[1], F, 1, 1, 1);
     if (P.residual_blocks == 1) {
-        conv_block(c, t2.src(), none, g, P.last, P.signature_features, 1, 1, 1, signatures, true, nullptr, nullptr,
-                   &l0);
+        last_conv(c, t2.src(), none, g, P, signatures, &l0, sb);
         return;
     }
     DT cur;
@@ -272,7 +289,7 @@
             cur = nxt;
         }
     }
-    conv_block(c, t2.src(), cur.src(), g, P.last, P.signature_features, 1, 1, 1, signatures);
+    last_conv(c, t2.src(), cur.src(), g, P, signatures, nullptr, sb);
 }
 
 static void operation_pipeline(Ctx& c, const PdsMatchingParams& P, const float* concatenated, float* signature,
@@ -315,6 +332,38 @@
     PDS_REQUIRE(workspace_bytes >= need, "matching: workspace too small (%zu < %zu)", workspace_bytes, need);
     return run_with_batched_packing(workspace, (hipStream_t)stream, [&](Ctx& c) {
         matching_pipeline(c, *params, left, right, signatures, batch, h, w, d_begin, d_count);
+    }, weights_resident != 0);
+}
+
+int pds_matching_signatures_bound_records(const PdsMatchingParams* params, int batch, int h, int w, int d_count) {
+    if (check_matching_params(params)) return 0;
+    if (!(batch > 0 && h > 0 && w > 0 && d_count > 0)) return 0;
+    Ctx c{nullptr, 0, true, nullptr};
+    SignatureBound sb;
+    matching_pipeline(c, *params, nullptr, nullptr, nullptr, batch, h, w, 0, d_count, false, nullptr, &sb);
+    return c.err ? 0 : sb.written;
+}
+
+int pds_matching_bounded_fwd(const PdsMatchingParams* params, const float* left, const float* right, float* signatures,
+                             float* signatures_bound, int signatures_bound_records, int batch, int h, int w, int d_begin,
+                             int d_count, void* workspace, size_t workspace_bytes, int weights_resident,
+                             pds_stream_t stream) {
+    if (!signatures_bound)
+        return pds_matching_fwd(params, left, right, signatures, batch, h, w, d_begin, d_count, workspace, workspace_bytes,
+                                weights_resident, stream);
+    if (int rc = check_matching_params(params)) return rc;
+    PDS_REQUIRE(left && right && signatures && workspace, "matching_bounded: null pointer");
+    PDS_REQUIRE(batch > 0 && h > 0 && w > 0 && d_begin >= 0 && d_count > 0, "matching_bounded: bad shape");
+    const int records = pds_matching_signatures_bound_records(params, batch, h, w, d_count);
+    PDS_REQUIRE(records > 0, "matching_bounded: this path leaves no range certificate (pass signatures_bound = NULL)");
+    PDS_REQUIRE(signatures_bound_records == records, "matching_bounded: %d certificate records, need %d",
+                signatures_bound_records, records);
+    const size_t need = pds_matching_workspace_bytes(params, batch, h, w, d_count);
+    PDS_REQUIRE(workspace_bytes >= need, "matching_bounded: workspace too small (%zu < %zu)", workspace_bytes, need);
+    return run_with_batched_packing(workspace, (hipStream_t)stream, [&](Ctx& c) {
+        SignatureBound sb;
+        sb.records = signatures_bound;
+        matching_pipeline(c, *params, left, right, signatures, batch, h, w, d_begin, d_count, false, nullptr, &sb);
     }, weights_resident != 0);
 }
 
diff --git a/practicaldeepstereo_nips2018_amd/csrc/api_regularization.hip b/practicaldeepstereo_nips2018_amd/csrc/api_regularization.hip
--- a/practicaldeepstereo_nips2018_amd/csrc/api_regularization.hip
+++ b/practicaldeepstereo_nips2018_amd/csrc/api_regularization.hip
@@ -2,11 +2,25 @@
 
 namespace pds {
 
+struct SignatureCertificate {
+    const float* records = nullptr;
+    int count = 0;
+};
+static bool signature_bound_enabled() {
+    static const bool on = !debug_switch_off("PDS_SIGNATURE_BOUND");
+    return on;
+}
+
 static DT regularization_trunk(Ctx& c, const PdsRegularizationParams& P, const float* ms, const float* left,
-                               int batch, int d, int h, int w) {
+                               int batch, int d, int h, int w, const SignatureCertificate& cert = SignatureCertificate()) {
     const int F = P.features;
     const Geom g0{batch, F, d, h, w};
-    const Src ms_src = external_src(c, ms, g0);
+    Src ms_src = external_src(c, ms, g0);
+    if (cert.records && cert.count > 0 && signature_bound_enabled()) {
+        ms_src.bound = cert.records;
+        ms_src.bound_n = cert.count;
+        ms_src.bounded = 1;
+    }
     Src shortcut = external_src(c, left, g0, 1);
     KsChain chain;
     c.chain_sync = c.get<unsigned>(kKsChainStateWords);
@@ -37,8 +51,9 @@
                          float* cost, int batch, int cin, int d, int hi_, int wi, hipStream_t s);
 
 static void regularization_pipeline(Ctx& c, const PdsRegularizationParams& P, const float* ms, const float* left,
-                                    float* cost, int batch, int d, int h, int w) {
-    DT half = regularization_trunk(c, P, ms, left, batch, d, h, w);
+                                    float* cost, int batch, int d, int h, int w,
+                                    const SignatureCertificate& cert = SignatureCertificate()) {
+    DT half = regularization_trunk(c, P, ms, left, batch, d, h, w, cert);
     if (upsample_full_valu_supported(half.g.c)) {
         float* w_pairs = c.get<float>((size_t)half.g.c * 48);
         if (c.before_packing()) c.run(launch_upsample_weight_pairs(P.upsample_full.weight, w_pairs, half.g.c, c.s));
@@ -122,23 +137,34 @@
     return c.off;
 }
 
+int pds_regularization_bounded_fwd(const PdsRegularizationParams* params, const float* signatures,
+                                   const float* signatures_bound, int signatures_bound_records,
+                                   const float* left_shortcut, float* cost, int batch, int d, int h, int w,
+                                   void* workspace, size_t workspace_bytes, int weights_resident, pds_stream_t stream) {
+    if (int rc = check_regularization(params, batch, d, h, w)) return rc;
+    PDS_REQUIRE(signatures && left_shortcut && cost && workspace, "regularization: null pointer");
+    PDS_REQUIRE(!signatures_bound || signatures_bound_records > 0, "regularization: a certificate needs at least one record");
+    const size_t need = pds_regularization_workspace_bytes(params, batch, d, h, w);
+    PDS_REQUIRE(workspace_bytes >= need, "regularization: workspace too small (%zu < %zu)", workspace_bytes, need);
+    const SignatureCertificate cert{signatures_bound, signatures_bound ? signatures_bound_records : 0};
+    return run_with_batched_packing(workspace, (hipStream_t)stream, [&](Ctx& c) {
+        regularization_pipeline(c, *params, signatures, left_shortcut, cost, batch, d, h, w, cert);
+    }, weights_resident != 0);
+}
+
 int pds_regularization_fwd(const PdsRegularizationParams* params, const float* signatures,
                            const float* left_shortcut, float* cost, int batch, int d, int h, int w, void* workspace,
                            size_t workspace_bytes, int weights_resident, pds_stream_t stream) {
-    if (int rc = check_regularization(params, batch, d, h, w)) return rc;
-    PDS_REQUIRE(signatures && left_shortcut && cost && workspace, "regularization: null pointer");
-    const size_t need = pds_regularization_workspace_bytes(params, batch, d, h, w);
-    PDS_REQUIRE(workspace_bytes >= need, "regularization: workspace too small (%zu < %zu)", workspace_bytes, need);
-    return run_with_batched_packing(workspace, (hipStream_t)stream, [&](Ctx& c) {
-        regularization_pipeline(c, *params, signatures, left_shortcut, cost, batch, d, h, w);
-    }, weights_resident != 0);
+    return pds_regularization_bounded_fwd(params, signatures, nullptr, 0, left_shortcut, cost, batch, d, h, w, workspace,
+                                          workspace_bytes, weights_resident, stream);
 }
 
 static int regularization_estimator(const PdsRegularizationParams* params, const float* signatures,
                                     const float* left_shortcut, float* disparities, float* confidence, int batch, int d,
                                     int h, int w, int half_support_window, int disparity_step, int crop_top,
                                     int crop_left, void* workspace, size_t workspace_bytes, int weights_resident,
-                                    pds_stream_t stream, const char* what, bool mirror = false) {
+                                    pds_stream_t stream, const char* what, bool mirror = false,
+                                    const SignatureCertificate& cert = SignatureCertificate()) {
     if (int rc = check_regularization(params, batch, d, h, w)) return rc;
     PDS_REQUIRE(signatures && left_shortcut && disparities && workspace, "%s: null pointer", what);
     PDS_REQUIRE(disparity_step >= 1 && half_support_window >= 1 && half_support_window % disparity_step == 0,
@@ -154,7 +180,7 @@
         DT half;
         float* w_pairs = nullptr;
         if (int rc = run_with_batched_packing(workspace, (hipStream_t)stream, [&](Ctx& cc) {
-                half = regularization_trunk(cc, *params, signatures, left_shortcut, batch, d, h, w);
+                half = regularization_trunk(cc, *params, signatures, left_shortcut, batch, d, h, w, cert);
                 w_pairs = cc.get<float>((size_t)half.g.c * 48);
                 if (cc.before_packing())
                     cc.run(launch_upsample_weight_pairs(params->upsample_full.weight, w_pairs, half.g.c, cc.s));
@@ -170,7 +196,7 @@
     PDS_REQUIRE(!mirror, "%s: the mirror is only folded into the fused kernel (4 features, window <= 4 taps)", what);
     float* cost = c.get<float>((size_t)batch * 2 * d * 4 * h * 4 * w);
     if (int rc = run_with_batched_packing((char*)workspace + c.off, (hipStream_t)stream, [&](Ctx& cc) {
-            regularization_pipeline(cc, *params, signatures, left_shortcut, cost, batch, d, h, w);
+            regularization_pipeline(cc, *params, signatures, left_shortcut, cost, batch, d, h, w, cert);
         }, weights_resident != 0))
         return rc;
     if (confidence)
@@ -212,6 +238,21 @@
                                     true);
 }
 
+int pds_regularization_subpixel_map_bounded_fwd(const PdsRegularizationParams* params, const float* signatures,
+                                                const float* signatures_bound, int signatures_bound_records,
+                                                const float* left_shortcut, float* disparities, float* confidence,
+                                                int batch, int d, int h, int w, int half_support_window,
+                                                int disparity_step, int crop_top, int crop_left, int mirror,
+                                                void* workspace, size_t workspace_bytes, int weights_resident,
+                                                pds_stream_t stream) {
+    PDS_REQUIRE(!signatures_bound || signatures_bound_records > 0,
+                "regularization_subpixel_map_bounded: a certificate needs at least one record");
+    const SignatureCertificate cert{signatures_bound, signatures_bound ? signatures_bound_records : 0};
+    return regularization_estimator(params, signatures, left_shortcut, disparities, confidence, batch, d, h, w,
+                                    half_support_window, disparity_step, crop_top, crop_left, workspace,
+                                    workspace_bytes, weights_resident, stream, "regularization_subpixel_map_bounded",
+                                    mirror != 0, cert);
+}
 
 #define PDS_MARK reinterpret_cast<const float*>(8)
 static const PdsConvBlockParams kDummyBlocks[2] = {{PDS_MARK, PDS_MARK, PDS_MARK, PDS_MARK},
diff --git a/practicaldeepstereo_nips2018_amd/csrc/common.hpp b/practicaldeepstereo_nips2018_amd/csrc/common.hpp
--- a/practicaldeepstereo_nips2018_amd/csrc/common.hpp
+++ b/practicaldeepstereo_nips2018_amd/csrc/common.hpp
@@ -144,7 +144,10 @@
     const float* l1H = nullptr;
     unsigned l1_bstride = 0, l1_hstride = 0, l1_edge = 0;
     int l1_P = 0, l1_d0 = 0;
-};
+    float* amax = nullptr;
+    int amax_n = 0;
+};
+constexpr int kConv2dT8Records = 512;
 
 int launch_conv_direct(const ConvLayer& L, hipStream_t s);
 int conv_direct_tiles_for(const Geom& out_g, int stride);
@@ -238,6 +241,7 @@
 int launch_materialize_l0(const Src& a, const Geom& g, const float* A, const float* G, const float* G2,
                           size_t l0_cstride, int l0_rs, int d_begin, float* out, hipStream_t s, float* amax = nullptr);
 int materialize_l0_records(const Geom& g);
+int launch_tensor_amax(const float* x, size_t count, float* records, int n_records, hipStream_t s);
 
 int launch_left_right_check(const float* dl, const float* dr, unsigned char* lv, unsigned char* rv, float* lf,
                             float* rf, int rows, int w, float max_difference, hipStream_t s);
diff --git a/practicaldeepstereo_nips2018_amd/csrc/conv2d_t8.hip b/practicaldeepstereo_nips2018_amd/csrc/conv2d_t8.hip
--- a/practicaldeepstereo_nips2018_amd/csrc/conv2d_t8.hip
+++ b/practicaldeepstereo_nips2018_amd/csrc/conv2d_t8.hip
@@ -29,7 +29,19 @@
     int N, D, H, W;
     int lrelu;
     int tiles_x, tiles_y, tiles;
+    float* __restrict__ amax;
+    int amax_n;
 };
+
+__device__ __forceinline__ float c2_seen(float seen, float t, bool stored) {
+    return fmaxf(seen, stored ? (t == t ? fabsf(t) : __builtin_inff()) : 0.f);
+}
+__device__ __forceinline__ void c2_amax_record(const C2Args& A, float seen, float* red) {
+    if (!A.amax) return;
+    block_amax_record(seen, A.amax + blockIdx.x, red);
+    if (blockIdx.x == 0)
+        for (int i = (int)gridDim.x + (int)threadIdx.x; i < A.amax_n; i += (int)blockDim.x) A.amax[i] = 0.f;
+}
 
 __device__ __forceinline__ void c2_split(const float (&v)[4], f16x4& hi, f16x4& lo) {
     pds_u32x2 h, l;
@@ -251,6 +263,7 @@
     __syncthreads();
 
     f32x4 acc[C2_RP][C2_NB];
+    float seen = 0.f;
     TilePos Pcur = tile_pos(0);
     auto step = [&](int g, auto set_stash, auto set_fetch) {
         const int c = g % C2_CHUNKS;
@@ -318,6 +331,7 @@
                         const bool ok = y < A.H && Pcur.x0 + 16 * j + n16 < A.W;
                         __builtin_amdgcn_raw_buffer_store_b32(__builtin_bit_cast(int, t), ro,
                                                               ok ? out_lane + (h ? out_c1 : 0u) + 64u * j : ~0u, row_bytes, 0);
+                        seen = c2_seen(seen, t, ok);
                     }
                 }
         }
@@ -329,6 +343,7 @@
         step(g + 2, S3(), S2());
         step(g + 3, S0(), S3());
     }
+    c2_amax_record(A, seen, reinterpret_cast<float*>(ibuf));
 }
 
 constexpr int C2W_THREADS = 512;
@@ -519,6 +534,7 @@
     __syncthreads();
 
     f32x4 acc[NBH];
+    float seen = 0.f;
     TilePos Pcur = tile_pos(0);
 #ifdef PDS_C2W_TIMING
     long long tmw[5] = {0, 0, 0, 0, 0};
@@ -597,6 +613,7 @@
                     const bool ok = 2 * pair < C2W_TY && y < A.H && 16 * (half * NBH + j) + n16 < A.W;
                     __builtin_amdgcn_raw_buffer_store_b32(__builtin_bit_cast(int, t), ro,
                                                           ok ? out_lane + (h ? out_c1 : 0u) + 64u * j : ~0u, row_bytes, 0);
+                    seen = c2_seen(seen, t, ok);
                 }
             }
         }
@@ -616,6 +633,7 @@
         step(g, S1());
         step(g + 1, S0());
     }
+    c2_amax_record(A, seen, reinterpret_cast<float*>(ibuf));
 #ifdef PDS_C2W_TIMING
     if (lane == 0 && (blockIdx.x % 61) == 0 && (wave == 0 || wave == 5))
         printf("[t8w] wg %d wave %d: total %lld | stash(+wait) %lld fetch-issue %lld mfma %lld barrier %lld over %lld chunks (%d tiles)\n",
@@ -641,7 +659,7 @@
         (void)hipFuncSetAttribute(reinterpret_cast<const void*>(&conv2d_t8_kernel<TWO, NA, NB2>),
                                   hipFuncAttributeMaxDynamicSharedMemorySize, (int)(160 * 1024));
     }
-    int wgs = 512;
+    int wgs = kConv2dT8Records;
     if (wgs > A.tiles) wgs = (A.tiles + 7) / 8 * 8;
     hipLaunchKernelGGL((conv2d_t8_kernel<TWO, NA, NB2>), dim3(wgs), dim3(C2_THREADS), lds_bytes, s, A);
     return check_launch("conv2d_t8");
@@ -677,6 +695,7 @@
         cus[dev & 31] = n > 0 ? n : 256;
     }
     int wgs = cus[dev & 31] / 8 * 8;
+    if (wgs > kConv2dT8Records) wgs = kConv2dT8Records;
     if (wgs > A.tiles) wgs = (A.tiles + 7) / 8 * 8;
     const int probe = probe_before("conv2d_t8w", s);
     hipLaunchKernelGGL((conv2d_t8w_kernel<TWO, NBH, TY, ITEMS>), dim3(wgs), dim3(C2W_THREADS), lds_bytes, s, A);
@@ -720,6 +739,9 @@
     A.tiles_x = (A.W + C2_TX - 1) / C2_TX;
     A.tiles_y = (A.H + C2_TY - 1) / C2_TY;
     A.tiles = A.N * A.D * A.tiles_y * A.tiles_x;
+    A.amax = L.amax;
+    A.amax_n = L.amax ? L.amax_n : 0;
+    if (A.amax && A.amax_n < kConv2dT8Records) return set_error(-1, "conv2d_t8: %d certificate records, need %d", A.amax_n, kConv2dT8Records);
     if (!A.a.bound || A.a.bound_n <= 0 || (L.b.p && (!A.b.bound || A.b.bound_n <= 0)))
         return set_error(-1, "conv2d_t8: a source without a range bound");
     if (c2t8_wide(L)) {
diff --git a/practicaldeepstereo_nips2018_amd/csrc/conv3d_t8x.hip b/practicaldeepstereo_nips2018_amd/csrc/conv3d_t8x.hip
--- a/practicaldeepstereo_nips2018_amd/csrc/conv3d_t8x.hip
+++ b/practicaldeepstereo_nips2018_amd/csrc/conv3d_t8x.hip
@@ -280,8 +280,9 @@
     using C = TXCfg<NB, P>;
     constexpr size_t lds_bytes = (size_t)2 * C::BUF + 4 * T8_C * sizeof(float);
     static_assert(lds_bytes <= 160 * 1024, "LDS");
-    return launch_persistent<&conv3d_t8x_kernel<NB, P, SRC, EXACT>>(EXACT ? "conv3d_t8x<exact>" : "conv3d_t8x<guarded>",
-                                                                    "conv3d_t8x", A, A.records, batch, lds_bytes, s);
+    const char* name = P == 2 ? (EXACT ? "conv3d_t8x<fp16,exact>" : "conv3d_t8x<fp16,guarded>")
+                              : (EXACT ? "conv3d_t8x<bf16,exact>" : "conv3d_t8x<bf16,guarded>");
+    return launch_persistent<&conv3d_t8x_kernel<NB, P, SRC, EXACT>>(name, "conv3d_t8x", A, A.records, batch, lds_bytes, s);
 }
 
 }
diff --git a/practicaldeepstereo_nips2018_amd/csrc/misc.hip b/practicaldeepstereo_nips2018_amd/csrc/misc.hip
--- a/practicaldeepstereo_nips2018_amd/csrc/misc.hip
+++ b/practicaldeepstereo_nips2018_amd/csrc/misc.hip
@@ -759,4 +759,39 @@
     return check_launch("l1_combine");
 }
 
-}
+__global__ __launch_bounds__(256) void tensor_amax_kernel(const float* __restrict__ x, size_t count,
+                                                          float* __restrict__ records) {
+    __shared__ float red[16];
+    typedef float f32x4 __attribute__((ext_vector_type(4)));
+    float seen = 0.f, poison = 0.f;
+    const size_t head = (16 - (reinterpret_cast<uintptr_t>(x) & 15)) % 16 / sizeof(float);
+    const size_t first = head < count ? head : count;
+    const size_t quads = (count - first) / 4;
+    const f32x4* q = reinterpret_cast<const f32x4*>(x + first);
+    const size_t stride = (size_t)gridDim.x * 256;
+#pragma unroll 4
+    for (size_t i = (size_t)blockIdx.x * 256 + threadIdx.x; i < quads; i += stride) {
+        const f32x4 v = q[i];
+#pragma unroll
+        for (int e = 0; e < 4; ++e) {
+            seen = fmaxf(seen, fabsf(v[e]));
+            poison = fmaf(v[e], 0.f, poison);
+        }
+    }
+    if (blockIdx.x == 0) {
+        const size_t tail = first + 4 * quads;
+        for (size_t i = threadIdx.x; i < first + (count - tail); i += 256) {
+            const float v = x[i < first ? i : tail + (i - first)];
+            seen = fmaxf(seen, fabsf(v));
+            poison = fmaf(v, 0.f, poison);
+        }
+    }
+    block_amax_record(poison == poison ? seen : __builtin_inff(), records + blockIdx.x, red);
+}
+
+int launch_tensor_amax(const float* x, size_t count, float* records, int n_records, hipStream_t s) {
+    hipLaunchKernelGGL(tensor_amax_kernel, dim3(n_records), dim3(256), 0, s, x, count, records);
+    return check_launch("tensor_amax");
+}
+
+}
diff --git a/practicaldeepstereo_nips2018_amd/matching.py b/practicaldeepstereo_nips2018_amd/matching.py
--- a/practicaldeepstereo_nips2018_amd/matching.py
+++ b/practicaldeepstereo_nips2018_amd/matching.py
@@ -185,8 +185,11 @@
         if (isinstance(operation, MatchingOperation) and operation.supports_fused_matching()
                 and left.size(1) == operation.number_of_descriptor_features):
             if not needs_grad:
-                return _FusedMatchingFunction.apply(self, left, right, begin, count,
-                                                    *operation.parameters())
+                signatures, bound = _FusedMatchingFunction.apply(self, left, right, begin, count,
+                                                                 *operation.parameters())
+                if bound.numel() > 0:
+                    _lib.attach_signatures_bound(signatures, bound)
+                return signatures
             _lib.warn_eval_with_grad(self)
             if operation.supports_native_training():
                 return _TrainMatchingFunction.apply(self, left, right, begin, count, *operation.parameters())
@@ -258,16 +261,20 @@
         out = torch.empty((batch, operation.number_of_signature_features, count, h, w),
                           dtype=torch.float32, device=left.device)
         nbytes = lib.pds_matching_workspace_bytes(ctypes.byref(params), batch, h, w, count)
+        records = lib.pds_matching_signatures_bound_records(ctypes.byref(params), batch, h, w, count)
+        bound = torch.empty(max(int(records), 0), dtype=torch.float32, device=left.device)
         ws, resident, token = module._workspace.get_resident(
             nbytes, left.device, _lib.resident_key(module, operation, (batch, h, w, count)))
         with torch.cuda.device(left.device):
-            _lib.check(lib.pds_matching_fwd(
+            _lib.check(lib.pds_matching_bounded_fwd(
                 ctypes.byref(params), _lib.ptr(left), _lib.ptr(right), _lib.ptr(out),
+                _lib.ptr(bound) if bound.numel() > 0 else None, bound.numel(),
                 batch, h, w, begin, count, _lib.ptr(ws), ws.numel(), int(resident),
-                _lib.stream_handle(left.device)), 'pds_matching_fwd')
+                _lib.stream_handle(left.device)), 'pds_matching_bounded_fwd')
         module._workspace.commit(token)
         del keep
-        return out
+        ctx.mark_non_differentiable(bound)
+        return out, bound
 
     @staticmethod
     def backward(ctx, *grads):
diff --git a/practicaldeepstereo_nips2018_amd/regularization.py b/practicaldeepstereo_nips2018_amd/regularization.py
--- a/practicaldeepstereo_nips2018_amd/regularization.py
+++ b/practicaldeepstereo_nips2018_amd/regularization.py
@@ -200,17 +200,32 @@
                              (tuple(shortcut.shape), tuple(ms.shape)))
         return ms, shortcut
 
-    def forward(self, matching_signatures, shortcut_from_left_image):
+    def _signatures_bound(self, ms, signatures_bound):
+        if signatures_bound is None or signatures_bound is False:
+            return None
+        if signatures_bound is True:
+            held = _lib.attached_signatures_bound(ms)
+            return held if held is not None else _lib.derive_signatures_bound(ms)
+        records = _lib.require_gpu_tensor(signatures_bound, 'signatures_bound', 1)
+        if records.device != ms.device or records.numel() < 1:
+            raise ValueError('signatures_bound must hold at least one record on the device of the signatures')
+        return records
+
+    def forward(self, matching_signatures, shortcut_from_left_image, signatures_bound=True):
         ms, shortcut = self._check_inputs(matching_signatures, shortcut_from_left_image)
-        return _RegularizationFunction.apply(self, ms, shortcut, None, *self.parameters())
+        needs_grad = torch.is_grad_enabled() and (
+            ms.requires_grad or shortcut.requires_grad or any(p.requires_grad for p in self.parameters()))
+        bound = None if needs_grad else self._signatures_bound(ms, signatures_bound)
+        return _RegularizationFunction.apply(self, ms, shortcut, None, bound, *self.parameters())
 
     def forward_with_estimator(self, matching_signatures, shortcut_from_left_image, estimator, crop=(0, 0),
-                               with_confidence=False, mirror=False):
+                               with_confidence=False, mirror=False, signatures_bound=True):
         ms, shortcut = self._check_inputs(matching_signatures, shortcut_from_left_image)
         fold_mirror = bool(mirror) and self.can_fold_crop(estimator)
         window = (estimator._half_support_window, estimator._disparity_step, int(crop[0]), int(crop[1]),
                   bool(with_confidence), fold_mirror)
-        out = _RegularizationFunction.apply(self, ms, shortcut, window, *self.parameters())
+        bound = self._signatures_bound(ms, signatures_bound)
+        out = _RegularizationFunction.apply(self, ms, shortcut, window, bound, *self.parameters())
         if mirror and not fold_mirror:
             out = tuple(torch.flip(o, [-1]) for o in out) if with_confidence else torch.flip(out, [-1])
         return tuple(out) if with_confidence else out
@@ -219,7 +234,7 @@
 class _RegularizationFunction(torch.autograd.Function):
 
     @staticmethod
-    def forward(ctx, module, ms, shortcut, estimator_window, *unused_parameters):
+    def forward(ctx, module, ms, shortcut, estimator_window, bound, *unused_parameters):
         lib = _lib.load()
         batch, _, d, h, w = ms.shape
         params = module.native_params()
@@ -242,8 +257,22 @@
             window = None if estimator_window is None else (estimator_window[0], estimator_window[1])
             ws, resident, token = module._workspace.get_resident(
                 nbytes, ms.device, _lib.resident_key(module, module, (batch, d, h, w, window)))
+        if training:
+            bound = None
         with torch.cuda.device(ms.device):
-            if estimator_window is None:
+            if bound is not None and estimator_window is None:
+                _lib.check(lib.pds_regularization_bounded_fwd(
+                    ctypes.byref(params), _lib.ptr(ms), _lib.ptr(bound), bound.numel(), _lib.ptr(shortcut),
+                    _lib.ptr(out), batch, d, h, w, _lib.ptr(ws), ws.numel(), int(resident),
+                    _lib.stream_handle(ms.device)), 'pds_regularization_bounded_fwd')
+            elif bound is not None:
+                _lib.check(lib.pds_regularization_subpixel_map_bounded_fwd(
+                    ctypes.byref(params), _lib.ptr(ms), _lib.ptr(bound), bound.numel(), _lib.ptr(shortcut),
+                    _lib.ptr(out), None if confidence is None else _lib.ptr(confidence),
+                    batch, d, h, w, estimator_window[0], estimator_window[1], crop_top, crop_left,
+                    int(estimator_window[5]), _lib.ptr(ws), ws.numel(), int(resident),
+                    _lib.stream_handle(ms.device)), 'pds_regularization_subpixel_map_bounded_fwd')
+            elif estimator_window is None:
                 _lib.check(lib.pds_regularization_fwd(
                     ctypes.byref(params), _lib.ptr(ms), _lib.ptr(shortcut), _lib.ptr(out),
                     batch, d, h, w, _lib.ptr(ws), ws.numel(), int(resident), _lib.stream_handle(ms.device)),
@@ -303,4 +332,4 @@
                 _lib.ptr(fws), fws.numel(), _lib.ptr(ws), ws.numel(), _lib.stream_handle(ms.device)),
                 'pds_regularization_bwd')
         ctx.forward_workspace = None
-        return (None, grad_ms, grad_shortcut, None) + tuple(grads[id(p)] for p in module.parameters())
+        return (None, grad_ms, grad_shortcut, None, None) + tuple(grads[id(p)] for p in module.parameters())
```
